# mmp/pbrt-v3

Hardware: NVIDIA H100
Metric: Msamples/sec (higher is better)
Workload: dtype f32

## Files before the change

### include/pb2.h

```cpp
#ifndef PB2_H
#define PB2_H

#include <stddef.h>
#include <stdint.h>

#ifdef __cplusplus
extern "C" {
#endif

#define PB2_ABI_VERSION 10

typedef enum pb2_status {
    PB2_OK = 0,
    PB2_ERR_NO_DEVICE = 1,
    PB2_ERR_CUDA = 2,
    PB2_ERR_INVALID = 3,
    PB2_ERR_UNSUPPORTED = 4,
    PB2_ERR_NCCL = 5
} pb2_status;


typedef struct pb2_bvh_node {
    float bmin[3];
    float bmax[3];
    int32_t offset;
    uint16_t n_prims;
    uint8_t axis;
    uint8_t pad;
} pb2_bvh_node;

enum { PB2_PRIM_TRIANGLE = 0, PB2_PRIM_SPHERE = 1, PB2_PRIM_INSTANCE = 2 };
enum { PB2_MAT_NONE = 0, PB2_MAT_MATTE = 1, PB2_MAT_PLASTIC = 2, PB2_MAT_MIRROR = 3, PB2_MAT_GLASS = 4, PB2_MAT_SUBSTRATE = 5, PB2_MAT_METAL = 6,
       PB2_MAT_UBER = 7 };
enum { PB2_LIGHTDIST_UNIFORM = 0, PB2_LIGHTDIST_POWER = 1, PB2_LIGHTDIST_SPATIAL = 2 };
enum { PB2_FILTER_BOX = 0, PB2_FILTER_GAUSSIAN = 1, PB2_FILTER_MITCHELL = 2, PB2_FILTER_SINC = 3, PB2_FILTER_TRIANGLE = 4 };

typedef struct pb2_mesh {
    int32_t first_tri, n_tris;
    int32_t first_vertex, n_vertices;
    int32_t has_n, has_uv, has_s;
    int32_t reverse_orientation;
    int32_t transform_swaps_handedness;
    int32_t alpha_tex, shadow_alpha_tex;
    int32_t pad;
} pb2_mesh;

enum { PB2_WRAP_REPEAT = 0, PB2_WRAP_BLACK = 1, PB2_WRAP_CLAMP = 2 };
typedef struct pb2_texture {
    int32_t channels;
    int32_t width, height;
    int32_t wrap;
    int32_t do_trilinear;
    float max_anisotropy;
    float su, sv, du, dv;
    int32_t kind;
    int32_t pad;
    const float *texels;
    int32_t child[3];
    float value[3];
} pb2_texture;
enum { PB2_TEXKIND_IMAGE = 0, PB2_TEXKIND_CONSTANT = 1, PB2_TEXKIND_SCALE = 2, PB2_TEXKIND_MIX = 3, PB2_TEXKIND_CHECKERBOARD = 4,
       PB2_TEXKIND_UV = 5 };

enum { PB2_TEX_KD = 0, PB2_TEX_KS = 1, PB2_TEX_KR = 2, PB2_TEX_KT = 3, PB2_TEX_OPACITY = 4, PB2_TEX_SIGMA = 5, PB2_TEX_ROUGHNESS = 6,
       PB2_TEX_UROUGHNESS = 7, PB2_TEX_VROUGHNESS = 8, PB2_TEX_ETA = 9, PB2_TEX_METAL_ETA = 10, PB2_TEX_METAL_K = 11,
       PB2_TEX_BUMP = 12, PB2_TEX_SLOTS = 13 };

typedef struct pb2_sphere {
    float object_to_world[16];
    float world_to_object[16];
    float radius, z_min, z_max, theta_min, theta_max, phi_max;
    int32_t reverse_orientation;
    int32_t transform_swaps_handedness;
} pb2_sphere;

typedef struct pb2_material {
    int32_t type;
    float kd[3];
    float sigma;
    float ks[3];
    float roughness;
    int32_t remap_roughness;
    int32_t pad[2];
    float kr[3];
    float kt[3];
    float eta;
    float uroughness, vroughness;
    float opacity[3];
    float metal_eta[3];
    float metal_k[3];
    int32_t pad3[2];
    int32_t tex[16];
} pb2_material;

enum { PB2_LIGHT_AREA = 0, PB2_LIGHT_POINT = 1, PB2_LIGHT_SPOT = 2, PB2_LIGHT_DISTANT = 3, PB2_LIGHT_INFINITE = 4 };
typedef struct pb2_light {
    int32_t prim;
    float L[3];
    int32_t two_sided;
    float area;
    int32_t type;
    int32_t pad;
} pb2_light;

typedef struct pb2_delta_light {
    float p[3];
    float total_width_deg;
    float falloff_start_deg;
    float world_radius;
    float world_to_light[9];
    float pad;
    float light_to_world[9];
    int32_t env_tex;
    float pad2[2];
} pb2_delta_light;

typedef struct pb2_bvh {
    int64_t node_offset, n_nodes;
    int64_t prim_offset, n_prims;
} pb2_bvh;

typedef struct pb2_instance {
    float instance_to_world[16];
    float world_to_instance[16];
    int32_t bvh;
    int32_t lone_prim;
    int32_t pad[2];
} pb2_instance;

typedef struct pb2_scene_desc {
    int64_t n_vertices;
    const float *P;
    const float *N;
    const float *UV;
    const float *S;
    int64_t n_tris;
    const int32_t *tri_index;
    const int32_t *tri_mesh;
    int32_t n_meshes;
    const pb2_mesh *meshes;
    int32_t n_spheres;
    const pb2_sphere *spheres;

    int64_t n_prims;
    const uint8_t *prim_type;
    const int32_t *prim_index;
    const int32_t *prim_material;
    const int32_t *prim_light;

    int64_t n_nodes;
    const pb2_bvh_node *nodes;
    const int32_t *bvh_prims;

    int32_t n_materials;
    const pb2_material *materials;
    int32_t n_lights;
    const pb2_light *lights;

    int32_t light_strategy;
    int32_t spatial_max_voxels;

    int32_t n_instances;
    int32_t n_bvhs;
    const pb2_instance *instances;
    const pb2_bvh *bvhs;
    int64_t n_bvh_prims;
    const pb2_delta_light *delta_lights;
    int32_t n_textures;
    int32_t pad_textures;
    const pb2_texture *textures;
} pb2_scene_desc;

typedef struct pb2_camera {
    float camera_to_world[16];
    float world_to_camera[16];
    float screen_window[4];
    float fov;
    float lens_radius, focal_distance;
    float shutter_open, shutter_close;
    float raster_to_camera[16];
    float dx_camera[3], dy_camera[3];
} pb2_camera;

typedef struct pb2_film_desc {
    int32_t full_resolution[2];
    int32_t cropped_pixel_bounds[4];
    float filter_radius[2];
    float max_sample_luminance;
    float scale;
    int32_t filter_type;
    float filter_param[2];
    int32_t pad;
} pb2_film_desc;

typedef struct pb2_path_params {
    int32_t samples_per_pixel;
    int32_t sample_at_pixel_center;
    int32_t max_depth;
    float rr_threshold;
    int32_t pixel_bounds[4];
    int32_t tile_rank, tile_count;
    int32_t flags;
    int32_t sampler;
} pb2_path_params;

enum { PB2_SAMPLER_HALTON = 0, PB2_SAMPLER_SOBOL = 1 };

#define PB2_FLAG_COUNT_TRAVERSAL 1
#define PB2_FLAG_LINEAR_NODES 2
#define PB2_FLAG_WIDE4 4
#define PB2_FLAG_PLAIN_TRACE 8
#define PB2_FLAG_SMALL_STACK 16
#define PB2_FLAG_LD128 32
#define PB2_FLAG_LEAF_TMA 64
#define PB2_FLAG_POOL 128
#define PB2_FLAG_CHAIN 256

typedef struct pb2_ray {
    float o[3];
    float d[3];
    float t_max;
} pb2_ray;

typedef struct pb2_hit {
    int32_t prim;
    float t;
    float b[3];
    float p[3];
    float p_error[3];
    float n[3];
    float ns[3];
    float dpdu[3];
    float uv[2];
} pb2_hit;

typedef struct pb2_stats {
    uint64_t camera_rays;
    uint64_t regular_rays;
    uint64_t shadow_rays;
    uint64_t node_visits;
    uint64_t prim_tests;
    uint64_t kernel_launches;
    double render_ms;
    double h2d_ms, d2h_ms;
    double trace_ms;
} pb2_stats;

typedef struct pb2_scene pb2_scene;


int pb2_abi_version(void);
const char *pb2_last_error(void);

int pb2_init(int device_id);
int pb2_init_devices(int n_devices, const int *device_ids);
int pb2_device_count(void);
int pb2_shutdown(void);

#define PB2_DIST_ID_BYTES 128
int pb2_dist_unique_id(void *id);
int pb2_dist_init(int rank, int world, const void *id);
int pb2_dist_info(int *rank, int *world);
int pb2_dist_shutdown(void);

int pb2_work_items(const pb2_film_desc *film, const pb2_path_params *params, int64_t first, int64_t n, int32_t *out,
                   int64_t *n_items);

int pb2_host_alloc(size_t bytes, void **out);
int pb2_host_free(void *p);

int pb2_scene_create(const pb2_scene_desc *desc, pb2_scene **out);
int pb2_scene_destroy(pb2_scene *scene);
int pb2_shade_class(const pb2_scene_desc *desc, int32_t *out);

int pb2_intersect(pb2_scene *scene, const pb2_ray *rays, int64_t n, pb2_hit *hits);
int pb2_intersect_p(pb2_scene *scene, const pb2_ray *rays, int64_t n, uint8_t *occluded);

int pb2_render_path(pb2_scene *scene, const pb2_camera *camera, const pb2_film_desc *film,
                    const pb2_path_params *params, float *film_rgbw, pb2_stats *stats);

int pb2_render_path_device(pb2_scene *scene, const pb2_camera *camera, const pb2_film_desc *film,
                           const pb2_path_params *params, float *film_rgbw_device, int clear,
                           void *stream, pb2_stats *stats);

typedef struct pb2_wf_hit {
    int32_t found;
    int32_t leaf;
    int32_t prim;
    float t;
    float b[3];
    int32_t listed;
} pb2_wf_hit;
int pb2_trace_wavefront(pb2_scene *scene, const pb2_ray *rays, const uint8_t *any_hit, int64_t n, int32_t flags,
                        pb2_wf_hit *out);

int pb2_li_samples(pb2_scene *scene, const pb2_camera *camera, const pb2_film_desc *film,
                   const pb2_path_params *params, const int32_t *pixel_xy, const int64_t *sample_num,
                   int64_t n, float *out_rgb, float *out_pfilm);

int pb2_halton_samples(const pb2_film_desc *film, const pb2_path_params *params,
                       const int32_t *pixel_xy, const int64_t *sample_num, const int32_t *dim,
                       int64_t n, float *out);

int pb2_sobol_samples_host(const pb2_film_desc *film, const pb2_path_params *params, const int32_t *pixel_xy,
                           const int64_t *sample_num, const int32_t *dim, int64_t n, float *out, uint64_t *tables);

int pb2_light_distribution(pb2_scene *scene, const float *points_xyz, int64_t n, float *out);

int pb2_texture_pyramid(const pb2_texture *texture, int32_t level, int32_t *n_levels, int32_t *w, int32_t *h, float *out);

int pb2_texture_eval_host(const pb2_texture *textures, int32_t n_textures, int32_t id, int64_t n, const float *uv, const float *duv,
                          float *out);

int pb2_bsdf_eval_host(const pb2_material *material, int64_t n, const float *in, float *out);

int pb2_camera_differentials_host(const pb2_camera *camera, const pb2_film_desc *film, const pb2_path_params *params, int64_t n,
                                  const float *in, float *out);
int pb2_uv_differentials_host(int64_t n, const float *in, float *out);

int pb2_env_distribution(const pb2_texture *texture, int32_t *nu, int32_t *nv, float *out);

int pb2_texture_lookup(const pb2_texture *texture, int64_t n, const float *st, const float *dst, float *out);

typedef struct pb2_build_node {
    float bmin[3], bmax[3];
    int32_t child[2];
    int32_t split_axis;
    int32_t first_prim_offset;
    int32_t n_primitives;
} pb2_build_node;
int pb2_hlbvh_treelets(const float *prim_bounds, int64_t n, int32_t max_prims_in_node, pb2_build_node *pool,
                       int32_t *ordered_prims, int32_t *treelet_roots, int32_t *n_treelets, double *device_ms);

int pb2_hlbvh_build(const float *prim_bounds, int64_t n, int32_t max_prims_in_node, pb2_bvh_node *nodes, int64_t *n_nodes,
                    int32_t *ordered_prims, double *device_ms);

#ifdef __cplusplus
}
#endif
#endif
```

### pbrt_v3_b200/__init__.py

```python
import ctypes as C
import os

import numpy as np

_HERE = os.path.dirname(os.path.abspath(__file__))
LIB_PATH = os.environ.get("PB2_LIB") or os.path.join(_HERE, "lib", "libpb2.so")

c_float_p = C.POINTER(C.c_float)
c_int32_p = C.POINTER(C.c_int32)
c_int64_p = C.POINTER(C.c_int64)
c_uint8_p = C.POINTER(C.c_uint8)

PB2_OK, PB2_ERR_NO_DEVICE, PB2_ERR_CUDA, PB2_ERR_INVALID, PB2_ERR_UNSUPPORTED, PB2_ERR_NCCL = range(6)
PB2_PRIM_TRIANGLE, PB2_PRIM_SPHERE, PB2_PRIM_INSTANCE = 0, 1, 2
PB2_FILTER_BOX, PB2_FILTER_GAUSSIAN, PB2_FILTER_MITCHELL, PB2_FILTER_SINC, PB2_FILTER_TRIANGLE = 0, 1, 2, 3, 4
PB2_MAT_NONE, PB2_MAT_MATTE, PB2_MAT_PLASTIC, PB2_MAT_MIRROR, PB2_MAT_GLASS, PB2_MAT_SUBSTRATE, PB2_MAT_METAL, PB2_MAT_UBER = range(8)
PB2_ABI_VERSION = 10
PB2_LIGHTDIST_UNIFORM, PB2_LIGHTDIST_POWER, PB2_LIGHTDIST_SPATIAL = 0, 1, 2
PB2_LIGHT_AREA, PB2_LIGHT_POINT, PB2_LIGHT_SPOT, PB2_LIGHT_DISTANT, PB2_LIGHT_INFINITE = 0, 1, 2, 3, 4


class BvhNode(C.Structure):
    _fields_ = [("bmin", C.c_float * 3), ("bmax", C.c_float * 3), ("offset", C.c_int32),
                ("n_prims", C.c_uint16), ("axis", C.c_uint8), ("pad", C.c_uint8)]


class Mesh(C.Structure):
    _fields_ = [("first_tri", C.c_int32), ("n_tris", C.c_int32), ("first_vertex", C.c_int32),
                ("n_vertices", C.c_int32), ("has_n", C.c_int32), ("has_uv", C.c_int32), ("has_s", C.c_int32),
                ("reverse_orientation", C.c_int32), ("transform_swaps_handedness", C.c_int32),
                ("alpha_tex", C.c_int32), ("shadow_alpha_tex", C.c_int32), ("pad", C.c_int32)]


class Sphere(C.Structure):
    _fields_ = [("object_to_world", C.c_float * 16), ("world_to_object", C.c_float * 16),
                ("radius", C.c_float), ("z_min", C.c_float), ("z_max", C.c_float), ("theta_min", C.c_float),
                ("theta_max", C.c_float), ("phi_max", C.c_float), ("reverse_orientation", C.c_int32),
                ("transform_swaps_handedness", C.c_int32)]


class Material(C.Structure):
    _fields_ = [("type", C.c_int32), ("kd", C.c_float * 3), ("sigma", C.c_float), ("ks", C.c_float * 3),
                ("roughness", C.c_float), ("remap_roughness", C.c_int32), ("pad", C.c_int32 * 2),
                ("kr", C.c_float * 3), ("kt", C.c_float * 3), ("eta", C.c_float), ("uroughness", C.c_float),
                ("vroughness", C.c_float), ("opacity", C.c_float * 3), ("metal_eta", C.c_float * 3),
                ("metal_k", C.c_float * 3), ("pad3", C.c_int32 * 2), ("tex", C.c_int32 * 16)]


PB2_WRAP_REPEAT, PB2_WRAP_BLACK, PB2_WRAP_CLAMP = 0, 1, 2
PB2_SAMPLER_HALTON, PB2_SAMPLER_SOBOL = 0, 1
(PB2_TEX_KD, PB2_TEX_KS, PB2_TEX_KR, PB2_TEX_KT, PB2_TEX_OPACITY, PB2_TEX_SIGMA, PB2_TEX_ROUGHNESS, PB2_TEX_UROUGHNESS,
 PB2_TEX_VROUGHNESS, PB2_TEX_ETA, PB2_TEX_METAL_ETA, PB2_TEX_METAL_K, PB2_TEX_BUMP) = range(13)


class Texture(C.Structure):
    _fields_ = [("channels", C.c_int32), ("width", C.c_int32), ("height", C.c_int32), ("wrap", C.c_int32),
                ("do_trilinear", C.c_int32), ("max_anisotropy", C.c_float), ("su", C.c_float), ("sv", C.c_float),
                ("du", C.c_float), ("dv", C.c_float), ("kind", C.c_int32), ("pad", C.c_int32), ("texels", c_float_p),
                ("child", C.c_int32 * 3), ("value", C.c_float * 3)]


PB2_TEXKIND_IMAGE, PB2_TEXKIND_CONSTANT, PB2_TEXKIND_SCALE, PB2_TEXKIND_MIX, PB2_TEXKIND_CHECKERBOARD, PB2_TEXKIND_UV = 0, 1, 2, 3, 4, 5


class Light(C.Structure):
    _fields_ = [("prim", C.c_int32), ("L", C.c_float * 3), ("two_sided", C.c_int32), ("area", C.c_float),
                ("type", C.c_int32), ("pad", C.c_int32)]


class DeltaLight(C.Structure):
    _fields_ = [("p", C.c_float * 3), ("total_width_deg", C.c_float), ("falloff_start_deg", C.c_float),
                ("world_radius", C.c_float), ("world_to_light", C.c_float * 9), ("pad", C.c_float),
                ("light_to_world", C.c_float * 9), ("env_tex", C.c_int32), ("pad2", C.c_float * 2)]


class Bvh(C.Structure):
    _fields_ = [("node_offset", C.c_int64), ("n_nodes", C.c_int64), ("prim_offset", C.c_int64), ("n_prims", C.c_int64)]


class Instance(C.Structure):
    _fields_ = [("instance_to_world", C.c_float * 16), ("world_to_instance", C.c_float * 16), ("bvh", C.c_int32),
                ("lone_prim", C.c_int32), ("pad", C.c_int32 * 2)]


class SceneDesc(C.Structure):
    _fields_ = [("n_vertices", C.c_int64), ("P", c_float_p), ("N", c_float_p), ("UV", c_float_p), ("S", c_float_p),
                ("n_tris", C.c_int64), ("tri_index", c_int32_p), ("tri_mesh", c_int32_p),
                ("n_meshes", C.c_int32), ("meshes", C.POINTER(Mesh)),
                ("n_spheres", C.c_int32), ("spheres", C.POINTER(Sphere)),
                ("n_prims", C.c_int64), ("prim_type", c_uint8_p), ("prim_index", c_int32_p),
                ("prim_material", c_int32_p), ("prim_light", c_int32_p),
                ("n_nodes", C.c_int64), ("nodes", C.POINTER(BvhNode)), ("bvh_prims", c_int32_p),
                ("n_materials", C.c_int32), ("materials", C.POINTER(Material)),
                ("n_lights", C.c_int32), ("lights", C.POINTER(Light)),
                ("light_strategy", C.c_int32), ("spatial_max_voxels", C.c_int32),
                ("n_instances", C.c_int32), ("n_bvhs", C.c_int32), ("instances", C.POINTER(Instance)),
                ("bvhs", C.POINTER(Bvh)), ("n_bvh_prims", C.c_int64), ("delta_lights", C.POINTER(DeltaLight)),
                ("n_textures", C.c_int32), ("pad_textures", C.c_int32), ("textures", C.POINTER(Texture))]


class Camera(C.Structure):
    _fields_ = [("camera_to_world", C.c_float * 16), ("world_to_camera", C.c_float * 16),
                ("screen_window", C.c_float * 4), ("fov", C.c_float), ("lens_radius", C.c_float),
                ("focal_distance", C.c_float), ("shutter_open", C.c_float), ("shutter_close", C.c_float),
                ("raster_to_camera", C.c_float * 16), ("dx_camera", C.c_float * 3), ("dy_camera", C.c_float * 3)]


class FilmDesc(C.Structure):
    _fields_ = [("full_resolution", C.c_int32 * 2), ("cropped_pixel_bounds", C.c_int32 * 4),
                ("filter_radius", C.c_float * 2), ("max_sample_luminance", C.c_float), ("scale", C.c_float),
                ("filter_type", C.c_int32), ("filter_param", C.c_float * 2), ("pad", C.c_int32)]


class PathParams(C.Structure):
    _fields_ = [("samples_per_pixel", C.c_int32), ("sample_at_pixel_center", C.c_int32), ("max_depth", C.c_int32),
                ("rr_threshold", C.c_float), ("pixel_bounds", C.c_int32 * 4), ("tile_rank", C.c_int32),
                ("tile_count", C.c_int32), ("flags", C.c_int32), ("sampler", C.c_int32)]


class Ray(C.Structure):
    _fields_ = [("o", C.c_float * 3), ("d", C.c_float * 3), ("t_max", C.c_float)]


class Hit(C.Structure):
    _fields_ = [("prim", C.c_int32), ("t", C.c_float), ("b", C.c_float * 3), ("p", C.c_float * 3),
                ("p_error", C.c_float * 3), ("n", C.c_float * 3), ("ns", C.c_float * 3), ("dpdu", C.c_float * 3),
                ("uv", C.c_float * 2)]


class WfHit(C.Structure):
    _fields_ = [("found", C.c_int32), ("leaf", C.c_int32), ("prim", C.c_int32), ("t", C.c_float), ("b", C.c_float * 3),
                ("listed", C.c_int32)]


class Stats(C.Structure):
    _fields_ = [("camera_rays", C.c_uint64), ("regular_rays", C.c_uint64), ("shadow_rays", C.c_uint64),
                ("node_visits", C.c_uint64), ("prim_tests", C.c_uint64), ("kernel_launches", C.c_uint64),
                ("render_ms", C.c_double), ("h2d_ms", C.c_double), ("d2h_ms", C.c_double), ("trace_ms", C.c_double)]


RAY_DTYPE = np.dtype([("o", np.float32, 3), ("d", np.float32, 3), ("t_max", np.float32)])
HIT_DTYPE = np.dtype([("prim", np.int32), ("t", np.float32), ("b", np.float32, 3), ("p", np.float32, 3),
                      ("p_error", np.float32, 3), ("n", np.float32, 3), ("ns", np.float32, 3),
                      ("dpdu", np.float32, 3), ("uv", np.float32, 2)])
WFHIT_DTYPE = np.dtype([("found", np.int32), ("leaf", np.int32), ("prim", np.int32), ("t", np.float32), ("b", np.float32, 3),
                        ("listed", np.int32)])
PB2_FLAG_COUNT_TRAVERSAL, PB2_FLAG_LINEAR_NODES, PB2_FLAG_WIDE4, PB2_FLAG_PLAIN_TRACE, PB2_FLAG_SMALL_STACK, PB2_FLAG_LD128, PB2_FLAG_LEAF_TMA, PB2_FLAG_POOL = 1, 2, 4, 8, 16, 32, 64, 128
PB2_FLAG_CHAIN = 256
NODE_DTYPE = np.dtype([("bmin", np.float32, 3), ("bmax", np.float32, 3), ("offset", np.int32),
                       ("n_prims", np.uint16), ("axis", np.uint8), ("pad", np.uint8)])
assert WFHIT_DTYPE.itemsize == C.sizeof(WfHit)
assert RAY_DTYPE.itemsize == C.sizeof(Ray) and HIT_DTYPE.itemsize == C.sizeof(Hit) and NODE_DTYPE.itemsize == 32


class Pb2Error(RuntimeError):
    def __init__(self, code, message):
        super().__init__("pb2 status %d: %s" % (code, message))
        self.code = code


_lib = None


def lib():
    global _lib
    if _lib is not None:
        return _lib
    if not os.path.exists(LIB_PATH):
        raise ImportError("%s is missing: run `python -c 'import __graft_entry__ as g; g.build()'` "
                          "(the CUDA extension is required; there is no fallback)" % LIB_PATH)
    L = C.CDLL(LIB_PATH)
    vp = C.c_void_p
    L.pb2_last_error.restype = C.c_char_p
    L.pb2_scene_create.argtypes = [C.POINTER(SceneDesc), C.POINTER(vp)]
    L.pb2_scene_destroy.argtypes = [vp]
    L.pb2_intersect.argtypes = [vp, vp, C.c_int64, vp]
    L.pb2_intersect_p.argtypes = [vp, vp, C.c_int64, vp]
    L.pb2_trace_wavefront.argtypes = [vp, vp, vp, C.c_int64, C.c_int32, vp]
    L.pb2_work_items.argtypes = [C.POINTER(FilmDesc), C.POINTER(PathParams), C.c_int64, C.c_int64, vp, C.POINTER(C.c_int64)]
    L.pb2_init_devices.argtypes = [C.c_int, C.POINTER(C.c_int)]
    L.pb2_dist_unique_id.argtypes = [vp]
    L.pb2_dist_init.argtypes = [C.c_int, C.c_int, vp]
    L.pb2_dist_info.argtypes = [C.POINTER(C.c_int), C.POINTER(C.c_int)]
    L.pb2_host_alloc.argtypes = [C.c_size_t, C.POINTER(vp)]
    L.pb2_host_free.argtypes = [vp]
    L.pb2_render_path.argtypes = [vp, C.POINTER(Camera), C.POINTER(FilmDesc), C.POINTER(PathParams), vp, C.POINTER(Stats)]
    L.pb2_render_path_device.argtypes = [vp, C.POINTER(Camera), C.POINTER(FilmDesc), C.POINTER(PathParams), vp,
                                         C.c_int, vp, C.POINTER(Stats)]
    L.pb2_li_samples.argtypes = [vp, C.POINTER(Camera), C.POINTER(FilmDesc), C.POINTER(PathParams), vp, vp, C.c_int64, vp, vp]
    L.pb2_halton_samples.argtypes = [C.POINTER(FilmDesc), C.POINTER(PathParams), vp, vp, vp, C.c_int64, vp]
    L.pb2_light_distribution.argtypes = [vp, vp, C.c_int64, vp]
    L.pb2_sobol_samples_host.argtypes = [C.POINTER(FilmDesc), C.POINTER(PathParams), vp, vp, vp, C.c_int64, vp, vp]
    L.pb2_texture_pyramid.argtypes = [C.POINTER(Texture), C.c_int32, C.POINTER(C.c_int32), C.POINTER(C.c_int32), C.POINTER(C.c_int32), vp]
    L.pb2_texture_lookup.argtypes = [C.POINTER(Texture), C.c_int64, vp, vp, vp]
    L.pb2_env_distribution.argtypes = [C.POINTER(Texture), C.POINTER(C.c_int32), C.POINTER(C.c_int32), vp]
    L.pb2_texture_eval_host.argtypes = [C.POINTER(Texture), C.c_int32, C.c_int32, C.c_int64, vp, vp, vp]
    L.pb2_bsdf_eval_host.argtypes = [C.POINTER(Material), C.c_int64, vp, vp]
    L.pb2_camera_differentials_host.argtypes = [C.POINTER(Camera), C.POINTER(FilmDesc), C.POINTER(PathParams), C.c_int64, vp, vp]
    L.pb2_uv_differentials_host.argtypes = [C.c_int64, vp, vp]
    L.pb2h_parse_file.argtypes = [C.c_char_p, C.c_char_p]
    L.pb2h_parse_string.argtypes = [C.c_char_p]
    L.pb2h_synth_soup.argtypes = [C.c_int64, C.c_uint64, C.c_float, C.c_int, C.c_int, C.c_int, C.c_int, C.c_char_p]
    L.pb2h_synth_instanced.argtypes = [C.c_int64, C.c_int, C.c_uint64, C.c_uint64, C.c_float, C.c_int, C.c_int, C.c_int, C.c_int]
    L.pb2h_scene_desc.restype = C.POINTER(SceneDesc)
    L.pb2h_camera.restype = C.POINTER(Camera)
    L.pb2h_film.restype = C.POINTER(FilmDesc)
    L.pb2h_path_params.restype = C.POINTER(PathParams)
    L.pb2h_render.argtypes = [C.c_int, C.POINTER(Stats)]
    L.pb2h_image.restype = c_float_p
    L.pb2h_image.argtypes = [C.POINTER(C.c_int), C.POINTER(C.c_int)]
    L.pb2h_resolve_film.argtypes = [vp, vp]
    L.pb2h_device_scene.restype = vp
    L.pb2h_write_pfm.argtypes = [C.c_char_p, vp, C.c_int, C.c_int]
    L.pb2h_write_image.argtypes = [C.c_char_p, vp] + [C.c_int] * 6
    L.pb2h_read_image.argtypes = [C.c_char_p, vp, C.POINTER(C.c_int), C.POINTER(C.c_int)]
    L.pb2h_loop_subdivide.argtypes = [C.c_int, C.c_int, vp, C.c_int, vp, C.POINTER(C.c_int), C.POINTER(C.c_int), vp, vp, vp]
    L.pb2h_set_light_strategy.argtypes = [C.c_int]
    L.pb2h_scene_intersect.argtypes = [vp, vp, vp]
    _lib = L
    return L


def check(code):
    if code != PB2_OK:
        raise Pb2Error(code, lib().pb2_last_error().decode("utf-8", "replace"))


def ptr(a):
    return a.ctypes.data_as(C.c_void_p) if a is not None else None


_initialised_device = None


def init(device=None):
    global _initialised_device
    if device is None:
        device = int(os.environ.get("LOCAL_RANK", os.environ.get("PB2_DEVICE", "0")))
    if _initialised_device == device:
        return
    check(lib().pb2_init(device))
    _initialised_device = device


def sobol_samples_host(film, params, pixel_xy, sample_num, dim, tables=False):
    pixel_xy = np.ascontiguousarray(pixel_xy, np.int32)
    sample_num = np.ascontiguousarray(sample_num, np.int64)
    dim = np.ascontiguousarray(dim, np.int32)
    out = np.zeros(len(dim), np.float32)
    tab = np.zeros(104, np.uint64)
    check(lib().pb2_sobol_samples_host(film, params, ptr(pixel_xy), ptr(sample_num), ptr(dim), len(dim), ptr(out), ptr(tab)))
    return (out, tab) if tables else out


def texture_pyramid(texture, fn=None):
    fn = fn or lib().pb2_texture_pyramid
    nl, w, h = C.c_int32(), C.c_int32(), C.c_int32()
    check(fn(C.byref(texture), 0, C.byref(nl), C.byref(w), C.byref(h), None))
    levels = []
    for lv in range(nl.value):
        check(fn(C.byref(texture), lv, C.byref(nl), C.byref(w), C.byref(h), None))
        a = np.zeros((h.value, w.value, texture.channels), np.float32)
        check(fn(C.byref(texture), lv, C.byref(nl), C.byref(w), C.byref(h), ptr(a)))
        levels.append(a)
    return levels


def bsdf_eval_host(material, frames, fn=None):
    fn = fn or lib().pb2_bsdf_eval_host
    frames = np.ascontiguousarray(frames, np.float32)
    out = np.zeros((len(frames), 19), np.float32)
    check(fn(C.byref(material), len(frames), ptr(frames), ptr(out)))
    return out


def texture_eval_host(textures, n_textures, tex_id, uv, duv, fn=None):
    fn = fn or lib().pb2_texture_eval_host
    uv = np.ascontiguousarray(uv, np.float32)
    duv = np.ascontiguousarray(duv, np.float32)
    out = np.zeros((len(uv), 3), np.float32)
    check(fn(textures, n_textures, tex_id, len(uv), ptr(uv), ptr(duv), ptr(out)))
    return out


def env_distribution(texture, fn=None):
    fn = fn or lib().pb2_env_distribution
    nu, nv = C.c_int32(), C.c_int32()
    check(fn(C.byref(texture), C.byref(nu), C.byref(nv), None))
    table = np.zeros(nv.value * (2 * nu.value + 2) + 2 * nv.value + 2, np.float32)
    check(fn(C.byref(texture), C.byref(nu), C.byref(nv), ptr(table)))
    return nu.value, nv.value, table


def read_image(path):
    w, h = C.c_int(), C.c_int()
    if lib().pb2h_read_image(path.encode(), None, C.byref(w), C.byref(h)) != 0:
        raise RuntimeError("cannot read %s" % path)
    out = np.zeros((h.value, w.value, 3), np.float32)
    lib().pb2h_read_image(path.encode(), ptr(out), C.byref(w), C.byref(h))
    return out


def texture_lookup(texture, st, dst):
    init()
    st = np.ascontiguousarray(st, np.float32)
    dst = np.ascontiguousarray(dst, np.float32)
    out = np.zeros((len(st), 3), np.float32)
    check(lib().pb2_texture_lookup(C.byref(texture), len(st), ptr(st), ptr(dst), ptr(out)))
    return out


class HostScene:

    _generation = 0

    def __init__(self):
        self.L = lib()
        HostScene._generation += 1
        self._gen = HostScene._generation

    def _current(self):
        if self._gen != HostScene._generation:
            raise RuntimeError("this HostScene was replaced by a later HostScene (the host front end holds one scene at a time)")

    @classmethod
    def from_file(cls, path, outfile=None):
        s = cls()
        if s.L.pb2h_parse_file(path.encode(), outfile.encode() if outfile else None) != 0:
            raise RuntimeError("could not parse %s" % path)
        return s

# ... 176 lines not shown
```

### pbrt_v3_b200/csrc/pb2_cuda.cu

```cuda
#include <cuda_runtime.h>
#include <cub/device/device_radix_sort.cuh>
#include <dlfcn.h>
#include <nccl.h>

#include <algorithm>
#include <mutex>
#include <chrono>
#include <cstddef>
#include <cstdio>
#include <cstdlib>
#include <cstring>
#include <string>
#include <thread>
#include <vector>

#include "device/pb2_path.cuh"
#include "device/pb2_wide4.cuh"
#include "host/core.h"
#include "pb2.h"

using namespace pb2;

static thread_local std::string g_lastError;
static int setError(int code, const std::string &msg) {
// ... 425 lines not shown
        out.prim = it.prim;
        out.b[0] = h.b0; out.b[1] = h.b1; out.b[2] = h.b2;
        out.p[0] = it.p.x; out.p[1] = it.p.y; out.p[2] = it.p.z;
        out.p_error[0] = it.pError.x; out.p_error[1] = it.pError.y; out.p_error[2] = it.pError.z;
        out.n[0] = it.n.x; out.n[1] = it.n.y; out.n[2] = it.n.z;
        out.ns[0] = it.ns.x; out.ns[1] = it.ns.y; out.ns[2] = it.ns.z;
        out.dpdu[0] = it.dpdus.x; out.dpdu[1] = it.dpdus.y; out.dpdu[2] = it.dpdus.z;
        out.uv[0] = it.uv.x; out.uv[1] = it.uv.y;
    }
    hits[i] = out;
}

__global__ void k_intersect_p(DScene sc, const pb2_ray *rays, int64_t n, uint8_t *occluded) {
    int64_t i = blockIdx.x * (int64_t)blockDim.x + threadIdx.x;
    if (i >= n) return;
    DRay r;
    r.o = mk3(rays[i].o[0], rays[i].o[1], rays[i].o[2]);
    r.d = mk3(rays[i].d[0], rays[i].d[1], rays[i].d[2]);
    r.tMax = rays[i].t_max;
    DHit h;
    h.leaf = -1;
    h.inst = -1;
    float tMax = r.tMax;
    occluded[i] = traverse<true>(sc, r, &tMax, &h, nullptr) ? 1 : 0;
}

struct DRenderParams {
    DCamera cam;
    DHalton halton;
    DPathParams path;
    int sbx0, sby0, sbx1, sby1;
    int pbx0, pby0, pbx1, pby1;
    int cx0, cy0, cx1, cy1;
    float filterRadiusX, filterRadiusY;
    float invFilterRadiusX, invFilterRadiusY;
    const float *filterTable;
    float maxSampleLuminance;
    int nTilesX, nTilesY;
    int tileRank, tileCount;
    long long nOwnedTiles;
    long long nWorkItems;
    int spp;
    float diffScale;
};

enum { CTR_WORK = 0, CTR_CAMERA = 1, CTR_REGULAR = 2, CTR_SHADOW = 3, CTR_NODES = 4, CTR_PRIMS = 5, CTR_COUNT = 8 };

PB2_HD int compact1by1(unsigned x) {
    x &= 0x55555555u;
    x = (x ^ (x >> 1)) & 0x33333333u;
    x = (x ^ (x >> 2)) & 0x0f0f0f0fu;
    x = (x ^ (x >> 4)) & 0x00ff00ffu;
    return (int)x;
}

PB2_HD bool decodeWork(const DRenderParams &rp, long long item, int *px, int *py, int *sample) {
    long long perTile = 256LL * rp.spp;
    long long owned = item / perTile;
    int r = (int)(item - owned * perTile);
    long long tile = (long long)rp.tileRank + owned * rp.tileCount;
    int ty = (int)(tile / rp.nTilesX), tx = (int)(tile - (long long)ty * rp.nTilesX);
    int s = r >> 8, m = r & 255;
    int x = rp.sbx0 + tx * 16 + compact1by1((unsigned)m);
    int y = rp.sby0 + ty * 16 + compact1by1((unsigned)m >> 1);
    *px = x;
    *py = y;
    *sample = s;
    if (x >= rp.sbx1 || y >= rp.sby1) return false;
    return x >= rp.pbx0 && x < rp.pbx1 && y >= rp.pby0 && y < rp.pby1;
}

__device__ __noinline__ void addSampleFiltered(const DRenderParams &rp, float4 *film, V2 pFilm, V3 L) {
    float dx = pFilm.x - 0.5f, dy = pFilm.y - 0.5f;
    int p0x = (int)ceilf(dx - rp.filterRadiusX), p0y = (int)ceilf(dy - rp.filterRadiusY);
    int p1x = (int)floorf(dx + rp.filterRadiusX) + 1, p1y = (int)floorf(dy + rp.filterRadiusY) + 1;
    p0x = max(p0x, rp.cx0);
    p0y = max(p0y, rp.cy0);
    p1x = min(p1x, rp.cx1);
    p1y = min(p1y, rp.cy1);
    int width = rp.cx1 - rp.cx0;
    for (int yy = p0y; yy < p1y; ++yy) {
        float fy = fabsf(((float)yy - dy) * rp.invFilterRadiusY * 16.f);
        int ify = min((int)floorf(fy), 15);
        for (int xx = p0x; xx < p1x; ++xx) {
            float fx = fabsf(((float)xx - dx) * rp.invFilterRadiusX * 16.f);
            int ifx = min((int)floorf(fx), 15);
            float w = rp.filterTable[ify * 16 + ifx];
            float4 *px = film + ((size_t)(yy - rp.cy0) * width + (xx - rp.cx0));
            atomicAdd(px, make_float4(L.x * w, L.y * w, L.z * w, w));
        }
    }
}

__device__ __forceinline__ void addSample(const DRenderParams &rp, float4 *film, V2 pFilm, V3 L) {
    float y = luminance(L);
    if (y > rp.maxSampleLuminance) L = L * (rp.maxSampleLuminance / y);
    if (rp.filterTable) {
        addSampleFiltered(rp, film, pFilm, L);
        return;
    }
    float dx = pFilm.x - 0.5f, dy = pFilm.y - 0.5f;
    int p0x = (int)ceilf(dx - rp.filterRadiusX), p0y = (int)ceilf(dy - rp.filterRadiusY);
    int p1x = (int)floorf(dx + rp.filterRadiusX) + 1, p1y = (int)floorf(dy + rp.filterRadiusY) + 1;
    p0x = max(p0x, rp.cx0);
    p0y = max(p0y, rp.cy0);
    p1x = min(p1x, rp.cx1);
    p1y = min(p1y, rp.cy1);
    int width = rp.cx1 - rp.cx0;
    for (int yy = p0y; yy < p1y; ++yy)
        for (int xx = p0x; xx < p1x; ++xx) {
            float4 *px = film + ((size_t)(yy - rp.cy0) * width + (xx - rp.cx0));
            atomicAdd(px, make_float4(L.x, L.y, L.z, 1.f));
        }
}

#include "pb2_wavefront.cuh"

__global__ void k_li_samples(DScene sc, DRenderParams rp, const int32_t *pixelXY, const int64_t *sampleNum, int64_t n,
                             float *outRGB, float *outPFilm, int *deferred) {
    int64_t i = blockIdx.x * (int64_t)blockDim.x + threadIdx.x;
    if (i >= n) return;
    int px = pixelXY[2 * i], py = pixelXY[2 * i + 1];
    DSampler smp;
    smp.index = sampleIndex<true>(rp.halton, px, py, sampleNum[i]);
    smp.dim = 0;
    V2 pFilm;
    DRay ray = generateCameraRay<true>(rp.cam, rp.halton, smp, px, py, &pFilm);
    DLane ln;
    laneStartPath(ln, ray, smp);
    while (ln.state != LS_IDLE) {
        DHit hit;
        float tMax;
        bool found = traceLane(sc, ln, &tMax, &hit, nullptr);
        DTexCtx tc;
        tc.cam = &rp.cam;
        tc.pFilm = pFilm;
        tc.diffScale = rp.diffScale;
        laneAdvance<SHADE_FULL>(sc, rp.halton, rp.path, ln, found, hit, tMax, &tc);
        if (ln.state == LS_DEFER) {
            atomicAdd(deferred, 1);
            return;
        }
    }
    V3 L = guardRadiance(ln.L);
    outRGB[3 * i] = L.x;
    outRGB[3 * i + 1] = L.y;
    outRGB[3 * i + 2] = L.z;
    if (outPFilm) {
        outPFilm[2 * i] = pFilm.x;
        outPFilm[2 * i + 1] = pFilm.y;
    }
}

__global__ void k_wf_debug_fill(WfPool pool, const pb2_ray *rays, const uint8_t *anyHit, int n) {
    int i = blockIdx.x * blockDim.x + threadIdx.x;
    if (i == 0) {
        for (int q = 0; q < WQ_COUNT; ++q) pool.counts[q] = 0;
        pool.counts[WQ_TRACE0] = (unsigned)n;
    }
    if (i >= n) return;
    WfCtx &cx = pool.ctx[i];
    cx.ln.state = (anyHit && anyHit[i]) ? LS_SHADOW : LS_PATH;
    cx.ln.ray.o = mk3(rays[i].o[0], rays[i].o[1], rays[i].o[2]);
    cx.ln.ray.d = mk3(rays[i].d[0], rays[i].d[1], rays[i].d[2]);
    cx.ln.ray.tMax = rays[i].t_max;
    cx.hit = make_float4(__int_as_float(-1), 0.f, 0.f, 0.f);
    cx.tHit = 0.f;
    cx.found = -1;
    pool.queue[WQ_TRACE0][i] = i;
}
__global__ void k_wf_debug_read(DScene sc, WfPool pool, int n, pb2_wf_hit *out) {
    int i = blockIdx.x * blockDim.x + threadIdx.x;
    if (i >= n) return;
    const WfCtx &cx = pool.ctx[i];
    pb2_wf_hit h;
    h.found = cx.found;
    h.t = cx.tHit;
    h.leaf = __float_as_int(cx.hit.x);
    h.b[0] = cx.hit.y; h.b[1] = cx.hit.z; h.b[2] = cx.hit.w;
    h.prim = (cx.found > 0 && h.leaf >= 0) ? asInt(ldg4(&sc.leafPrims[3 * (size_t)h.leaf]).w) : -1;
    h.listed = 0;
    out[i] = h;
}
__global__ void k_wf_debug_lists(WfPool pool, pb2_wf_hit *out) {
    unsigned ns = pool.counts[WQ_SHADE], nl = pool.counts[WQ_LIGHT];
    for (unsigned i = blockIdx.x * blockDim.x + threadIdx.x; i < ns + nl; i += gridDim.x * blockDim.x) {
        int c = i < ns ? pool.queue[WQ_SHADE][i] : pool.queue[WQ_LIGHT][i - ns];
        atomicAdd(&out[c].listed, i < ns ? 1 : 2);
    }
}

__global__ void k_halton_samples(DHalton h, const int32_t *pixelXY, const int64_t *sampleNum, const int32_t *dim, int64_t n,
                                 float *out) {
    int64_t i = blockIdx.x * (int64_t)blockDim.x + threadIdx.x;
    if (i >= n) return;
    const int px = pixelXY[2 * i], py = pixelXY[2 * i + 1];
    int64_t index = sampleIndex<true>(h, px, py, sampleNum[i]);
    if (h.sobol && dim[i] < 2) out[i] = sobolPixelSample(h, index, dim[i], dim[i] == 0 ? px : py);
    else out[i] = sampleDimension<true>(h, index, dim[i]);
}

__global__ void k_halton_batch(DHalton h, const int32_t *pixelXY, const int64_t *sampleNum, const int32_t *dim0, int64_t n, float *out) {
    int64_t i = blockIdx.x * (int64_t)blockDim.x + threadIdx.x;
    if (i >= n) return;
    const int64_t index = sampleIndex<true>(h, pixelXY[2 * i], pixelXY[2 * i + 1], sampleNum[i]);
    float u[kSampleBatch];
    haltonSampleBatch<true>(h, index, dim0[i], kSampleBatch, u);
#pragma unroll
    for (int k = 0; k < kSampleBatch; ++k) out[kSampleBatch * i + k] = u[k];
}

__global__ void k_light_distribution(DScene sc, const float *points, int64_t n, float *out) {
    int64_t i = blockIdx.x * (int64_t)blockDim.x + threadIdx.x;
    if (i >= n) return;
    const float *rec = lightDistLookup(sc.lightDist, mk3(points[3 * i], points[3 * i + 1], points[3 * i + 2]));
    if (!rec) return;
    int stride = 2 * sc.nLights + 1;
    for (int k = 0; k < stride; ++k) out[i * stride + k] = rec[k];
}

static DHalton haltonTablesOnly() {
    DHalton h;
    memset(&h, 0, sizeof(h));
    h.primes = cur().primes;
    h.primeSums = cur().primeSums;
    h.perms = cur().perms;
    h.dimRecs = cur().dimRecs;
    h.dimTabs = cur().dimTabs;
    h.digitTab = cur().digitTab;
    return h;
}

static void launchLightDistBuild(const pb2_scene *scene, cudaStream_t stream) {
    k_lightdist_build<<<g_numSMs * 4, 128, 0, stream>>>(scene->d, haltonTablesOnly());
    k_lightdist_done<<<1, 32, 0, stream>>>(scene->d);
}
static int lightDistOverflowed(pb2_scene *scene, cudaStream_t stream, bool *overflowed) {
    *overflowed = false;
    if (!scene->lazyLightDist) return PB2_OK;
    CUDA_TRY(cudaMemcpyAsync(scene->ldHostCounters, scene->d.lightDist.counters, 4 * sizeof(int), cudaMemcpyDeviceToHost, stream));
    CUDA_TRY(cudaStreamSynchronize(stream));
    *overflowed = scene->ldHostCounters[2] != 0;
    return PB2_OK;
}
static int lightDistOverflowError() {
    return setError(PB2_ERR_UNSUPPORTED, "the on-demand pool of spatial light distributions is exhausted (very many lights x very many voxels touched): "
                                         "raise PB2_LIGHTDIST_POOL_MB or use lightsamplestrategy \"power\" / \"uniform\"");
}

static int requireDevice() {
    if (!g_initialised) return setError(PB2_ERR_NO_DEVICE, "pb2_init() has not succeeded: no CUDA device is bound (there is no CPU fallback)");
    return PB2_OK;
}

static bool computeFilterTable(const pb2_film_desc *f, float table[256]) {
    const float rx = f->filter_radius[0], ry = f->filter_radius[1];
    const float p0 = f->filter_param[0], p1 = f->filter_param[1];
    auto eval = [&](float x, float y) -> float {
        switch (f->filter_type) {
        case PB2_FILTER_GAUSSIAN: {
            const float alpha = p0, expX = std::exp(-alpha * rx * rx), expY = std::exp(-alpha * ry * ry);
            auto g = [&](float d, float expv) { return std::max((float)0, float(std::exp(-alpha * d * d) - expv)); };
            return g(x, expX) * g(y, expY);
        }
        case PB2_FILTER_MITCHELL: {
            const float B = p0, C = p1;
            auto m1 = [&](float v) {
                v = std::abs(2 * v);
                if (v > 1)
                    return ((-B - 6 * C) * v * v * v + (6 * B + 30 * C) * v * v + (-12 * B - 48 * C) * v + (8 * B + 24 * C)) * (1.f / 6.f);
                return ((12 - 9 * B - 6 * C) * v * v * v + (-18 + 12 * B + 6 * C) * v * v + (6 - 2 * B)) * (1.f / 6.f);
            };
            const float invRx = 1 / rx, invRy = 1 / ry;
            return m1(x * invRx) * m1(y * invRy);
        }
        case PB2_FILTER_SINC: {
            const float tau = p0, Pi = 3.14159265358979323846f;
            auto sinc = [&](float v) -> float {
                v = std::abs(v);
                if (v < 1e-5) return 1;
                return std::sin(Pi * v) / (Pi * v);
            };
            auto ws = [&](float v, float radius) -> float {
                v = std::abs(v);
                if (v > radius) return 0;
                float lanczos = sinc(v / tau);
                return sinc(v) * lanczos;
            };
            return ws(x, rx) * ws(y, ry);
        }
        case PB2_FILTER_TRIANGLE:
            return std::max((float)0, rx - std::abs(x)) * std::max((float)0, ry - std::abs(y));
        default:
            return 1.f;
        }
    };
    int offset = 0;
    for (int y = 0; y < 16; ++y)
        for (int x = 0; x < 16; ++x, ++offset) table[offset] = eval((x + 0.5f) * rx / 16, (y + 0.5f) * ry / 16);
    return f->filter_type != PB2_FILTER_BOX;
}

static DRenderParams makeRenderParams(const pb2_camera *cam, const pb2_film_desc *film, const pb2_path_params *pp) {
    DRenderParams rp;
    memset(&rp, 0, sizeof(rp));
    memcpy(rp.cam.rasterToCamera.m, cam->raster_to_camera, sizeof(float) * 16);
    memcpy(rp.cam.cameraToWorld.m, cam->camera_to_world, sizeof(float) * 16);
    rp.cam.lensRadius = cam->lens_radius;
    rp.cam.focalDistance = cam->focal_distance;
    rp.cam.dxCamera = mk3(cam->dx_camera[0], cam->dx_camera[1], cam->dx_camera[2]);
    rp.cam.dyCamera = mk3(cam->dy_camera[0], cam->dy_camera[1], cam->dy_camera[2]);
    rp.diffScale = 1 / std::sqrt((float)pp->samples_per_pixel);
    rp.halton = makeHalton(film, pp);
    rp.path.maxDepth = pp->max_depth;
    rp.path.rrThreshold = pp->rr_threshold;
    SampleBounds sb = filmSampleBounds(film);
    rp.sbx0 = sb.x0; rp.sby0 = sb.y0; rp.sbx1 = sb.x1; rp.sby1 = sb.y1;
    rp.pbx0 = pp->pixel_bounds[0]; rp.pby0 = pp->pixel_bounds[1]; rp.pbx1 = pp->pixel_bounds[2]; rp.pby1 = pp->pixel_bounds[3];
    rp.cx0 = film->cropped_pixel_bounds[0]; rp.cy0 = film->cropped_pixel_bounds[1];
    rp.cx1 = film->cropped_pixel_bounds[2]; rp.cy1 = film->cropped_pixel_bounds[3];
    rp.filterRadiusX = film->filter_radius[0];
    rp.filterRadiusY = film->filter_radius[1];
    rp.invFilterRadiusX = 1.f / film->filter_radius[0];
    rp.invFilterRadiusY = 1.f / film->filter_radius[1];
    rp.filterTable = nullptr;
    rp.maxSampleLuminance = film->max_sample_luminance;
    rp.nTilesX = (sb.x1 - sb.x0 + 15) / 16;
    rp.nTilesY = (sb.y1 - sb.y0 + 15) / 16;
    rp.tileCount = std::max(1, pp->tile_count);
    rp.tileRank = pp->tile_rank;
    long long nTiles = (long long)std::max(0, rp.nTilesX) * std::max(0, rp.nTilesY);
    rp.nOwnedTiles = nTiles > rp.tileRank ? (nTiles - rp.tileRank + rp.tileCount - 1) / rp.tileCount : 0;
    rp.spp = pp->samples_per_pixel;
    rp.nWorkItems = rp.nOwnedTiles * 256LL * rp.spp;
    return rp;
}

static int validateRenderArgs(const pb2_scene *scene, const pb2_camera *cam, const pb2_film_desc *film, const pb2_path_params *pp) {
    if (!scene || !cam || !film || !pp) return setError(PB2_ERR_INVALID, "null argument");
    if (pp->samples_per_pixel <= 0 || pp->max_depth < 0) return setError(PB2_ERR_INVALID, "bad samples_per_pixel / max_depth");
    if (5 + 8 * ((long long)pp->max_depth + 1) > kMaxHaltonDims)
        return setError(PB2_ERR_UNSUPPORTED, "maxdepth above 123: HaltonSampler can only sample 1000 dimensions");
    if (pp->tile_count < 0 || pp->tile_rank < 0 || (pp->tile_count > 0 && pp->tile_rank >= pp->tile_count))
        return setError(PB2_ERR_INVALID, "bad tile_rank / tile_count");
    if (pp->sampler != PB2_SAMPLER_HALTON && pp->sampler != PB2_SAMPLER_SOBOL) return setError(PB2_ERR_INVALID, "unknown sampler");
    if (pp->sampler == PB2_SAMPLER_SOBOL && (pp->samples_per_pixel & (pp->samples_per_pixel - 1)))
        return setError(PB2_ERR_INVALID, "SobolSampler: samples_per_pixel must be the power of two its constructor rounds up to (sobol.h:52)");
    if (film->cropped_pixel_bounds[2] < film->cropped_pixel_bounds[0] || film->cropped_pixel_bounds[3] < film->cropped_pixel_bounds[1])
        return setError(PB2_ERR_INVALID, "bad cropped pixel bounds");
    if (!(film->filter_radius[0] > 0) || !(film->filter_radius[1] > 0)) return setError(PB2_ERR_INVALID, "bad filter radius");
    if (film->filter_type < PB2_FILTER_BOX || film->filter_type > PB2_FILTER_TRIANGLE) return setError(PB2_ERR_INVALID, "unknown filter type");
    return PB2_OK;
}

enum { kMaxPipes = 4 };
typedef void (*TraceKernel)(DScene, WfPool, int, WfChain);
typedef void (*AdvanceKernel)(const DScene *, const DRenderParams *, WfPool, int, int, int, float4 *, unsigned long long *);

struct TraceLaunch {
    TraceKernel fn = nullptr;
    int block = 128;
    size_t smem = 0;
    int grid = 0;
    bool chain = false;
    const char *name = "";
};

enum TraceKernelForm { TK_COUNT, TK_PLAIN, TK_POOL, TK_WIDE2, TK_WIDE4, TK_LINEAR };
struct TraceKernelEntry {
    TraceKernelForm form;
    int features;
    TraceKernel fn;
    const char *name;
    size_t smem;
};
template <int WIDTH, int T>
static TraceKernelEntry wideTrace() {
    const char *name = WIDTH == 4              ? "k_wf_trace_w<4>"
                       : (T & TRACE_ALPHA) ? "k_wf_trace_w<2,alpha>"
                       : (T & TRACE_CHAIN) ? "k_wf_trace_w<2,chain>"
                                           : "k_wf_trace_w<2>";
    return {WIDTH == 4 ? TK_WIDE4 : TK_WIDE2, T, k_wf_trace_w<WIDTH, T>, name, 0};
}
template <int T>
static TraceKernelEntry linearTrace() { return {TK_LINEAR, T, k_wf_trace<T>, "k_wf_trace", 0}; }

struct TraceKey {
    TraceKernelForm form;
    int features;
};
static TraceKey chooseTraceKernel(const pb2_scene *scene, int flags, bool render) {
    const bool instanced = scene->d.instances != nullptr;
    const bool records = scene->d.wide4 != nullptr && !(flags & PB2_FLAG_LINEAR_NODES);
    const bool linearFits = !instanced || scene->bvhDepth + 3 + scene->instDepth <= 64;
    int sceneBits = scene->d.spheres ? TRACE_SPHERES : 0;
    if (instanced) sceneBits |= TRACE_SPHERES | TRACE_INST;
    if (flags & PB2_FLAG_COUNT_TRAVERSAL) return {TK_COUNT, 0};
    if ((flags & PB2_FLAG_PLAIN_TRACE) || (!records && !linearFits)) return {TK_PLAIN, 0};
    if (scene->d.hasAlpha) return records ? TraceKey{TK_WIDE2, sceneBits | TRACE_ALPHA} : TraceKey{TK_PLAIN, 0};
    if (!records) return {TK_LINEAR, sceneBits | (sceneBits || scene->bvhDepth > 32 ? TRACE_DEEP : 0)};
    if ((flags & PB2_FLAG_POOL) && !sceneBits) return {TK_POOL, 0};
    const bool ld128 = (flags & PB2_FLAG_LD128) != 0;
    int features = sceneBits | (ld128 ? TRACE_LD128 : 0) | ((flags & PB2_FLAG_SMALL_STACK) ? TRACE_SMALL_STACK : 0);
    if (flags & PB2_FLAG_WIDE4) return {TK_WIDE4, features};
    if (!ld128 && (flags & PB2_FLAG_LEAF_TMA) && !sceneBits) features = TRACE_LEAF_TMA;
    if (!ld128 && render && (flags & PB2_FLAG_CHAIN) && !(flags & (PB2_FLAG_SMALL_STACK | PB2_FLAG_LEAF_TMA))) features |= TRACE_CHAIN;
    return {TK_WIDE2, features};
}

static int selectTraceKernel(pb2_scene *scene, int flags, TraceLaunch *out, bool render = false, const char *steps = "") {
    static const TraceKernelEntry kernels[] = {
        {TK_COUNT, 0, k_wf_trace_plain<true>, "k_wf_trace_plain<count>", 0},
        {TK_PLAIN, 0, k_wf_trace_plain<false>, "k_wf_trace_plain", 0},
        {TK_POOL, 0, k_wf_trace_pool, "k_wf_trace_pool", 4 * sizeof(PoolWarp)},
        wideTrace<2, 0>(), wideTrace<2, TRACE_SMALL_STACK>(),
        wideTrace<2, TRACE_LD128>(), wideTrace<2, TRACE_LD128 | TRACE_SMALL_STACK>(),
        wideTrace<2, TRACE_SPHERES>(), wideTrace<2, TRACE_SPHERES | TRACE_SMALL_STACK>(),
        wideTrace<2, TRACE_SPHERES | TRACE_LD128>(), wideTrace<2, TRACE_SPHERES | TRACE_LD128 | TRACE_SMALL_STACK>(),
        wideTrace<2, TRACE_SPHERES | TRACE_INST>(), wideTrace<2, TRACE_SPHERES | TRACE_INST | TRACE_SMALL_STACK>(),
        wideTrace<2, TRACE_SPHERES | TRACE_INST | TRACE_LD128>(), wideTrace<2, TRACE_SPHERES | TRACE_INST | TRACE_LD128 | TRACE_SMALL_STACK>(),
        wideTrace<2, TRACE_LEAF_TMA>(),
        wideTrace<2, TRACE_CHAIN>(), wideTrace<2, TRACE_SPHERES | TRACE_CHAIN>(), wideTrace<2, TRACE_SPHERES | TRACE_INST | TRACE_CHAIN>(),
        wideTrace<2, TRACE_ALPHA>(), wideTrace<2, TRACE_SPHERES | TRACE_ALPHA>(), wideTrace<2, TRACE_SPHERES | TRACE_INST | TRACE_ALPHA>(),
        wideTrace<4, 0>(), wideTrace<4, TRACE_SMALL_STACK>(),
        wideTrace<4, TRACE_LD128>(), wideTrace<4, TRACE_LD128 | TRACE_SMALL_STACK>(),
        wideTrace<4, TRACE_SPHERES>(), wideTrace<4, TRACE_SPHERES | TRACE_SMALL_STACK>(),
        wideTrace<4, TRACE_SPHERES | TRACE_LD128>(), wideTrace<4, TRACE_SPHERES | TRACE_LD128 | TRACE_SMALL_STACK>(),
        wideTrace<4, TRACE_SPHERES | TRACE_INST>(), wideTrace<4, TRACE_SPHERES | TRACE_INST | TRACE_SMALL_STACK>(),
        wideTrace<4, TRACE_SPHERES | TRACE_INST | TRACE_LD128>(), wideTrace<4, TRACE_SPHERES | TRACE_INST | TRACE_LD128 | TRACE_SMALL_STACK>(),
        linearTrace<0>(), linearTrace<TRACE_DEEP>(),
        linearTrace<TRACE_SPHERES | TRACE_DEEP>(), linearTrace<TRACE_SPHERES | TRACE_INST | TRACE_DEEP>(),
    };
    const TraceKey want = chooseTraceKernel(scene, flags, render);
    const TraceKernelEntry *k = nullptr;
    for (const TraceKernelEntry &e : kernels)
        if (e.form == want.form && e.features == want.features) k = &e;
    if (!k)
        return setError(PB2_ERR_CUDA, "no trace kernel of form " + std::to_string(want.form) + " is compiled for the trace features " +
                                          std::to_string(want.features));
    TraceLaunch t;
    t.fn = k->fn;
    t.smem = k->smem;
    t.chain = (k->features & TRACE_CHAIN) != 0;
    t.name = k->name;
    if (k->form == TK_POOL && !scene->wfSpill)
        CUDA_TRY(cudaMalloc((void **)&scene->wfSpill, (size_t)kMaxPipes * g_numSMs * 8 * 4 * PL_R * PL_SPILL * sizeof(int2)));
    if (t.smem) CUDA_TRY(cudaFuncSetAttribute(t.fn, cudaFuncAttributeMaxDynamicSharedMemorySize, (int)t.smem));
    int blocksPerSM = 1;
    CUDA_TRY(cudaOccupancyMaxActiveBlocksPerMultiprocessor(&blocksPerSM, t.fn, t.block, t.smem));
    blocksPerSM = std::max(1, std::min(blocksPerSM, 8));
    cudaFuncAttributes fa;
    CUDA_TRY(cudaFuncGetAttributes(&fa, t.fn));
    size_t need = (size_t)blocksPerSM * (fa.sharedSizeBytes + t.smem + 1024);
    int pct = (int)std::min<size_t>(100, (need * 100 + 233471) / 233472);
    CUDA_TRY(cudaFuncSetAttribute(t.fn, cudaFuncAttributePreferredSharedMemoryCarveout, pct));
    static const int verbose = envInt("PB2_VERBOSE", 0);
    if (verbose)
        fprintf(stderr, "pb2: trace kernel %s: %d regs, %zu B smem, %d blocks/SM, carve-out %d %%, BVH depth %d%s\n", t.name, fa.numRegs,
                fa.sharedSizeBytes + t.smem, blocksPerSM, pct, scene->bvhDepth, steps);
    t.grid = g_numSMs * blocksPerSM;
    *out = t;
    return PB2_OK;
}

static int ensurePool(pb2_scene *scene, int capacity) {
    if (scene->wfCapacity < capacity) {
        if (scene->wfCtx) cudaFree(scene->wfCtx);
        if (scene->wfQueues) cudaFree(scene->wfQueues);
        scene->wfCtx = nullptr;
        scene->wfQueues = nullptr;
        scene->wfCapacity = 0;
        CUDA_TRY(cudaMalloc(&scene->wfCtx, (size_t)capacity * sizeof(WfCtx)));
        CUDA_TRY(cudaMalloc((void **)&scene->wfQueues, (size_t)capacity * WQ_COUNT * sizeof(int)));
        scene->wfCapacity = capacity;
    }
    if (!scene->wfCounts) CUDA_TRY(cudaMalloc((void **)&scene->wfCounts, kMaxPipes * WQ_COUNT * sizeof(unsigned)));
    if (!scene->wfHostCounts) CUDA_TRY(cudaMallocHost((void **)&scene->wfHostCounts, (kMaxPipes * WQ_COUNT + 2) * sizeof(unsigned long long)));
    return PB2_OK;
}

static WfPool poolOf(const pb2_scene *scene, int capacity, int pipe = 0, int nPipes = 1) {
    WfPool pool;
    const int cap = capacity / nPipes;
    pool.capacity = cap;
    pool.ctx = (WfCtx *)scene->wfCtx + (size_t)pipe * cap;
    for (int q = 0; q < WQ_COUNT; ++q) pool.queue[q] = scene->wfQueues + ((size_t)pipe * WQ_COUNT + q) * cap;
    pool.counts = scene->wfCounts + (size_t)pipe * WQ_COUNT;
    pool.ctr = scene->counters;
    pool.spill = scene->wfSpill ? scene->wfSpill + (size_t)pipe * g_numSMs * 8 * 4 * PL_R * PL_SPILL : nullptr;
    return pool;
}

constexpr int kShadeLambertAreaMinBlocks = 4;

typedef void (*GenKernel)(const DRenderParams *, WfPool, int, int);
typedef void (*FinishKernel)(const DScene *, const DRenderParams *, WfPool, int, unsigned, float4 *);

template <typename K>
struct StepKernel {
    int features;
    K fn;
};
template <bool SHADE, int MINB, int F>
static StepKernel<AdvanceKernel> advanceStep() { return {F, k_wf_advance<SHADE, MINB, F>}; }

template <typename K, size_t N>
static const StepKernel<K> &stepKernel(const StepKernel<K> (&table)[N], int frame) {
    int reads = 0;
    for (const StepKernel<K> &k : table) reads |= k.features;
    const StepKernel<K> *best = nullptr;
    for (const StepKernel<K> &k : table)
        if (!(frame & reads & ~k.features) && (!best || __builtin_popcount(k.features) < __builtin_popcount(best->features))) best = &k;
    return *best;
}

static int frameShadeFeatures(const pb2_scene *scene, const DRenderParams &rp) {
    int f = scene->shadeFeatures;
    if (scene->d.spheres) f |= SHADE_SPHERES;
    if (scene->lazyLightDist) f |= SHADE_LAZY;
    if (scene->d.nTextures > 0) f |= SHADE_TEXTURES;
    if (rp.halton.sobol) f |= SHADE_SOBOL;
    return f;
}

static int renderWavefront(pb2_scene *scene, const DRenderParams &rp, float4 *film, cudaStream_t stream, int flags,
                           bool timeTrace, unsigned long long *launches, double *traceMs) {
    const bool lazyLights = scene->lazyLightDist;
    static const int maxCapacity = envInt("PB2_POOL", 1 << 22);
    long long want = std::min<long long>(maxCapacity, std::max<long long>(rp.nWorkItems, 1024));
    int capacity = (int)((want + 255) / 256 * 256);
    int rc = ensurePool(scene, capacity);
    if (rc) return rc;
    static const StepKernel<GenKernel> genSteps[] = {{0, k_wf_gen<0>}, {SHADE_SOBOL, k_wf_gen<SHADE_SOBOL>}};
    static const StepKernel<AdvanceKernel> lightSteps[] = {
        advanceStep<false, 7, SHADE_LAMBERT_AREA>(),
        advanceStep<false, 7, SHADE_GENERAL>(),
        advanceStep<false, 7, SHADE_GENERAL | SHADE_SPHERES>(),
    };
    static const StepKernel<AdvanceKernel> shadeSteps[] = {
        advanceStep<true, kShadeLambertAreaMinBlocks, SHADE_LAMBERT_AREA>(),
        advanceStep<true, 4, SHADE_GENERAL>(),
        advanceStep<true, 4, SHADE_GENERAL | SHADE_SPHERES>(),
        advanceStep<true, 4, SHADE_GENERAL | SHADE_SPECULAR>(),
        advanceStep<true, 4, SHADE_GENERAL | SHADE_SPHERES | SHADE_SPECULAR>(),
        advanceStep<true, 4, SHADE_GENERAL | SHADE_LAZY>(),
        advanceStep<true, 4, SHADE_GENERAL | SHADE_SPHERES | SHADE_LAZY>(),
        advanceStep<true, 4, SHADE_GENERAL | SHADE_SPECULAR | SHADE_LAZY>(),
        advanceStep<true, 4, SHADE_GENERAL | SHADE_SPHERES | SHADE_SPECULAR | SHADE_LAZY>(),
        advanceStep<true, 3, SHADE_FULL>(),
    };
    static const StepKernel<FinishKernel> finishSteps[] = {
        {SHADE_LAMBERT_AREA, k_wf_finish<SHADE_LAMBERT_AREA>},
        {SHADE_GENERAL, k_wf_finish<SHADE_GENERAL>},
        {SHADE_GENERAL | SHADE_SPHERES, k_wf_finish<SHADE_GENERAL | SHADE_SPHERES>},
        {SHADE_GENERAL | SHADE_SPECULAR, k_wf_finish<SHADE_GENERAL | SHADE_SPECULAR>},
        {SHADE_GENERAL | SHADE_SPHERES | SHADE_SPECULAR, k_wf_finish<SHADE_GENERAL | SHADE_SPHERES | SHADE_SPECULAR>},
    };
    const int features = frameShadeFeatures(scene, rp);
    const StepKernel<GenKernel> &gen = stepKernel(genSteps, features);
    const StepKernel<AdvanceKernel> &advLight = stepKernel(lightSteps, features), &advShade = stepKernel(shadeSteps, features);
    const StepKernel<FinishKernel> &finish = stepKernel(finishSteps, features);
    char steps[96];
    snprintf(steps, sizeof(steps), "; shade features %d: gen %d, light %d, shade %d, tail %d", features, gen.features,
             advLight.features, advShade.features, finish.features);
    TraceLaunch trace;
    if ((rc = selectTraceKernel(scene, flags, &trace, true, steps))) return rc;
    if (!scene->paramBuf) CUDA_TRY(cudaMalloc(&scene->paramBuf, sizeof(DScene) + sizeof(DRenderParams)));
    const DScene *dSc = reinterpret_cast<const DScene *>(scene->paramBuf);
    const DRenderParams *dRp = reinterpret_cast<const DRenderParams *>((char *)scene->paramBuf + sizeof(DScene));
    CUDA_TRY(cudaMemcpyAsync((void *)dSc, &scene->d, sizeof(DScene), cudaMemcpyHostToDevice, stream));
    CUDA_TRY(cudaMemcpyAsync((void *)dRp, &rp, sizeof(DRenderParams), cudaMemcpyHostToDevice, stream));
    WfChain chain;
    memset(&chain, 0, sizeof(chain));
    if (trace.chain) {
        chain.sc = dSc;
        chain.rp = dRp;
        chain.film = film;
    }
    static const int finishPerSM = envInt("PB2_FINISH", 256);
    const bool textured = (features & (SHADE_TEXTURES | SHADE_SOBOL)) != 0;
    const unsigned finishThreshold = ((flags & PB2_FLAG_COUNT_TRAVERSAL) || lazyLights || textured) ? 0u : (unsigned)(g_numSMs * std::max(0, finishPerSM));
    const int finishBlocks = std::max(1, (int)((finishThreshold + 127) / 128));
    static const int syncEvery = std::max(1, envInt("PB2_SYNC_EVERY", 8));
    static const int pipesEnv = envInt("PB2_PIPES", 0);
    const int pipesWanted = std::min((int)kMaxPipes, pipesEnv > 0 ? pipesEnv : 2);
    const int nPipes = (lazyLights || capacity < 65536) ? 1 : pipesWanted;
    cudaStream_t streams[kMaxPipes] = {stream, stream, stream, stream};
    if (nPipes > 1) {
        if (!scene->forkEvent) CUDA_TRY(cudaEventCreateWithFlags(&scene->forkEvent, cudaEventDisableTiming));
        CUDA_TRY(cudaEventRecord(scene->forkEvent, stream));
        for (int p = 1; p < nPipes; ++p) {
            if (!scene->pipeStreams[p]) CUDA_TRY(cudaStreamCreateWithFlags(&scene->pipeStreams[p], cudaStreamNonBlocking));
            if (!scene->joinEvents[p]) CUDA_TRY(cudaEventCreateWithFlags(&scene->joinEvents[p], cudaEventDisableTiming));
            streams[p] = scene->pipeStreams[p];
            CUDA_TRY(cudaStreamWaitEvent(streams[p], scene->forkEvent, 0));
        }
    }
    WfPool pools[kMaxPipes];
    for (int p = 0; p < nPipes; ++p) pools[p] = poolOf(scene, capacity / nPipes * nPipes, p, nPipes);
    const int capP = pools[0].capacity;
    const int blocks128 = std::min((capP + 127) / 128, g_numSMs * 32);
    for (int p = 0; p < nPipes; ++p) k_wf_init<<<(capP + 255) / 256, 256, 0, streams[p]>>>(pools[p]);
    unsigned long long nLaunch = nPipes;
    size_t nEvents = 0;
    int cur = 0;
    volatile unsigned *hc = scene->wfHostCounts;
    unsigned long long *hWork = reinterpret_cast<unsigned long long *>(scene->wfHostCounts + kMaxPipes * WQ_COUNT);
    for (long long round = 0;; ++round) {
        int next = 1 - cur;
        for (int p = 0; p < nPipes; ++p) {
            const WfPool &pool = pools[p];
            cudaStream_t st = streams[p];
            gen.fn<<<blocks128, 128, 0, st>>>(dRp, pool, WQ_FREE0 + cur, WQ_TRACE0 + cur);
            if (timeTrace) {
                if (scene->traceEvents.size() < nEvents + 2) {
                    cudaEvent_t e0, e1;
                    CUDA_TRY(cudaEventCreate(&e0));
                    CUDA_TRY(cudaEventCreate(&e1));
                    scene->traceEvents.push_back(e0);
                    scene->traceEvents.push_back(e1);
                }
                CUDA_TRY(cudaEventRecord(scene->traceEvents[nEvents], st));
            }
            chain.freeQ = WQ_FREE0 + next;
            trace.fn<<<trace.grid, trace.block, trace.smem, st>>>(scene->d, pool, WQ_TRACE0 + cur, chain);
            if (timeTrace) {
                CUDA_TRY(cudaEventRecord(scene->traceEvents[nEvents + 1], st));
                nEvents += 2;
            }
            if (!trace.chain) advLight.fn<<<blocks128, 128, 0, st>>>(dSc, dRp, pool, WQ_LIGHT, WQ_TRACE0 + next, WQ_FREE0 + next, film, scene->counters);
            else --nLaunch;
            advShade.fn<<<blocks128, 128, 0, st>>>(dSc, dRp, pool, WQ_SHADE, WQ_TRACE0 + next, WQ_FREE0 + next, film, scene->counters);
            if (lazyLights) {
                launchLightDistBuild(scene, st);
                advShade.fn<<<blocks128, 128, 0, st>>>(dSc, dRp, pool, WQ_RETRY, WQ_TRACE0 + next, WQ_FREE0 + next, film, scene->counters);
                nLaunch += 3;
            }
            if (finishThreshold) finish.fn<<<finishBlocks, 128, 0, st>>>(dSc, dRp, pool, WQ_TRACE0 + next, finishThreshold, film);
            k_wf_reset<<<1, 32, 0, st>>>(pool, WQ_FREE0 + cur, WQ_TRACE0 + cur, WQ_TRACE0 + next, finishThreshold);
            nLaunch += finishThreshold ? 6 : 5;
        }
        cur = next;
        if ((round + 1) % syncEvery != 0) continue;
        for (int p = 0; p < nPipes; ++p)
            CUDA_TRY(cudaMemcpyAsync((void *)(scene->wfHostCounts + p * WQ_COUNT), pools[p].counts, WQ_COUNT * sizeof(unsigned), cudaMemcpyDeviceToHost, streams[p]));
        for (int p = 1; p < nPipes; ++p) CUDA_TRY(cudaStreamSynchronize(streams[p]));
        CUDA_TRY(cudaMemcpyAsync(hWork, &scene->counters[CTR_WORK], sizeof(unsigned long long), cudaMemcpyDeviceToHost, stream));
        CUDA_TRY(cudaStreamSynchronize(stream));
        bool overflowed = false;
        if ((rc = lightDistOverflowed(scene, stream, &overflowed))) return rc;
        if (overflowed) return lightDistOverflowError();
        const bool workLeft = (long long)*hWork < rp.nWorkItems;
        bool done = true;
        for (int p = 0; p < nPipes; ++p) {
            const unsigned traceNext = hc[p * WQ_COUNT + WQ_TRACE0 + cur], freeNext = hc[p * WQ_COUNT + WQ_FREE0 + cur];
            if (!(traceNext == 0 && !(workLeft && freeNext > 0))) done = false;
        }
        if (done) break;
        if (round > 100000000LL) return setError(PB2_ERR_CUDA, "wavefront did not terminate");
    }
    if (nPipes > 1) {
        for (int p = 1; p < nPipes; ++p) {
            CUDA_TRY(cudaEventRecord(scene->joinEvents[p], streams[p]));
            CUDA_TRY(cudaStreamWaitEvent(stream, scene->joinEvents[p], 0));
        }
    }
    CUDA_TRY(cudaGetLastError());
    *launches = nLaunch;
    *traceMs = 0;
    for (size_t e = 0; e + 1 < nEvents; e += 2) {
        float ms = 0;
        CUDA_TRY(cudaEventElapsedTime(&ms, scene->traceEvents[e], scene->traceEvents[e + 1]));
        *traceMs += ms;
    }
    return PB2_OK;
}

extern "C" {

int pb2_abi_version(void) { return PB2_ABI_VERSION; }
const char *pb2_last_error(void) { return g_lastError.c_str(); }

static void freeDeviceTables() {
    for (DeviceState &d : g_devs) {
        cudaSetDevice(d.id);
        cudaFree(d.primes);
        cudaFree(d.primeSums);
        cudaFree(d.perms);
        cudaFree(d.dimRecs);
        cudaFree(d.dimTabs);
        cudaFree(d.digitTab);
        cudaFree(d.sobol);
        cudaFree(d.sobolVdc);
    }
    g_devs.clear();
    g_initialised = false;
}

int pb2_init_devices(int n, const int *device_ids) {
    int count = 0;
    cudaError_t e = cudaGetDeviceCount(&count);
    if (e != cudaSuccess || count == 0) {
        cudaGetLastError();
        return setError(PB2_ERR_NO_DEVICE, std::string("no CUDA device available (") +
                                               (e != cudaSuccess ? cudaGetErrorString(e) : "device count is 0") +
                                               "); the path-tracing hot path has no CPU fallback");
    }
    std::vector<int> ids;
    if (n <= 0) for (int i = 0; i < count; ++i) ids.push_back(i);
    else {
        if (!device_ids) return setError(PB2_ERR_INVALID, "null device list");
        ids.assign(device_ids, device_ids + n);
    }
    for (size_t i = 0; i < ids.size(); ++i) {
        if (ids[i] < 0 || ids[i] >= count) return setError(PB2_ERR_INVALID, "device id out of range");
        for (size_t j = 0; j < i; ++j)
            if (ids[j] == ids[i]) return setError(PB2_ERR_INVALID, "device listed twice");
    }
    if (g_initialised && g_devs.size() == ids.size()) {
        bool same = true;
        for (size_t i = 0; i < ids.size(); ++i) same &= g_devs[i].id == ids[i];
        if (same) return PB2_OK;
    }
    if (g_dist.comm) return setError(PB2_ERR_INVALID, "pb2_init: shut the communicator down (pb2_dist_shutdown) before rebinding devices");
    freeDeviceTables();
    buildHaltonHostTables();
    t_dev = 0;
    for (int id : ids) {
        CUDA_TRY(cudaSetDevice(id));
        cudaDeviceProp prop;
        CUDA_TRY(cudaGetDeviceProperties(&prop, id));
        if (prop.major != 9 || prop.minor != 0) {
            freeDeviceTables();
            return setError(PB2_ERR_NO_DEVICE, std::string("device \"") + prop.name + "\" is not sm_90 (Hopper); this library is built for sm_90a only");
        }
        g_devs.emplace_back();
        DeviceState &d = g_devs.back();
        d.id = id;
        d.numSMs = prop.multiProcessorCount;
        CUDA_TRY(cudaMalloc((void **)&d.primes, g_halton.hPrimes.size() * sizeof(int32_t)));
        CUDA_TRY(cudaMalloc((void **)&d.primeSums, g_halton.hPrimeSums.size() * sizeof(int32_t)));
        CUDA_TRY(cudaMalloc((void **)&d.perms, g_halton.hPerms.size() * sizeof(uint16_t)));
        CUDA_TRY(cudaMalloc((void **)&d.dimRecs, g_halton.hDimRecs.size() * sizeof(ulonglong2)));
        CUDA_TRY(cudaMemcpy(d.dimRecs, g_halton.hDimRecs.data(), g_halton.hDimRecs.size() * sizeof(ulonglong2), cudaMemcpyHostToDevice));
        CUDA_TRY(cudaMemcpy(d.primes, g_halton.hPrimes.data(), g_halton.hPrimes.size() * sizeof(int32_t), cudaMemcpyHostToDevice));
        CUDA_TRY(cudaMemcpy(d.primeSums, g_halton.hPrimeSums.data(), g_halton.hPrimeSums.size() * sizeof(int32_t), cudaMemcpyHostToDevice));
        CUDA_TRY(cudaMemcpy(d.perms, g_halton.hPerms.data(), g_halton.hPerms.size() * sizeof(uint16_t), cudaMemcpyHostToDevice));
        CUDA_TRY(cudaMalloc((void **)&d.dimTabs, g_halton.hDimTabs.size() * sizeof(HaltonDimTab)));
        CUDA_TRY(cudaMalloc((void **)&d.digitTab, g_halton.hDigitTab.size() * sizeof(uint16_t)));
        CUDA_TRY(cudaMemcpy(d.dimTabs, g_halton.hDimTabs.data(), g_halton.hDimTabs.size() * sizeof(HaltonDimTab), cudaMemcpyHostToDevice));
        CUDA_TRY(cudaMemcpy(d.digitTab, g_halton.hDigitTab.data(), g_halton.hDigitTab.size() * sizeof(uint16_t), cudaMemcpyHostToDevice));
    }
    CUDA_TRY(cudaSetDevice(g_devs[0].id));
    for (size_t i = 1; i < g_devs.size(); ++i) {
        int can = 0;
        if (cudaDeviceCanAccessPeer(&can, g_devs[0].id, g_devs[i].id) == cudaSuccess && can) {
            cudaError_t pe = cudaDeviceEnablePeerAccess(g_devs[i].id, 0);
            g_devs[i].peerOfPrimary = pe == cudaSuccess || pe == cudaErrorPeerAccessAlreadyEnabled;
        }
        cudaGetLastError();
    }
    g_initialised = true;
    return PB2_OK;
}

int pb2_init(int device_id) { return pb2_init_devices(1, &device_id); }

int pb2_device_count(void) { return g_initialised ? (int)g_devs.size() : 0; }

int pb2_shutdown(void) {
    if (!g_initialised) return PB2_OK;
    pb2_dist_shutdown();
    freeDeviceTables();
    return PB2_OK;
}

int pb2_debug_radical_inverse_tables(const uint32_t *index, const int32_t *dim, int64_t n, float *out_loop, float *out_tab) {
    if (!index || !dim || !out_loop || !out_tab) return setError(PB2_ERR_INVALID, "null argument");
    buildHaltonHostTables();
    for (int64_t i = 0; i < n; ++i) {
        if (dim[i] < 2 || dim[i] >= kMaxHaltonDims) return setError(PB2_ERR_INVALID, "dimension out of range");
        const uint32_t base = (uint32_t)g_halton.hPrimes[dim[i]];
        const uint16_t *perm = g_halton.hPerms.data() + g_halton.hPrimeSums[dim[i]];
        const uint64_t magic = g_halton.hDimRecs[dim[i]].x;
        out_loop[i] = scrambledRadicalInverse32(base, magic, index[i], perm);
        out_tab[i] = scrambledRadicalInverseTab(g_halton.hDimTabs[dim[i]], g_halton.hDigitTab.data(), base, magic, index[i], perm);
    }
    return PB2_OK;
}

int pb2_debug_halton_batch(const pb2_film_desc *film, const pb2_path_params *pp, const uint32_t *index, const int32_t *dim0, int64_t n,
                           float *out_batch, float *out_tab) {
    if (!film || !pp || !index || !dim0 || !out_batch || !out_tab) return setError(PB2_ERR_INVALID, "null argument");
    buildHaltonHostTables();
    DHalton h = makeHalton(film, pp);
    h.perms = g_halton.hPerms.data();
    h.primes = g_halton.hPrimes.data();
    h.primeSums = g_halton.hPrimeSums.data();
    h.dimRecs = g_halton.hDimRecs.data();
    h.dimTabs = g_halton.hDimTabs.data();
    h.digitTab = g_halton.hDigitTab.data();
    for (int64_t i = 0; i < n; ++i) {
        if (dim0[i] < 2 || dim0[i] + kSampleBatch > kMaxHaltonDims) return setError(PB2_ERR_INVALID, "dimension out of range");
        haltonSampleBatch(h, (int64_t)index[i], dim0[i], kSampleBatch, out_batch + kSampleBatch * i);
        for (int k = 0; k < kSampleBatch; ++k) {
            const int d = dim0[i] + k;
            const uint32_t base = (uint32_t)g_halton.hPrimes[d];
            const uint16_t *perm = g_halton.hPerms.data() + g_halton.hPrimeSums[d];
// ... 796 lines not shown
        std::vector<int32_t> lightPrims(d->n_lights);
        for (int i = 0; i < d->n_lights; ++i) {
            if (d->lights[i].type != PB2_LIGHT_AREA) {
                lightPrims[i] = 0;
                continue;
            }
            if (d->lights[i].prim < 0 || d->lights[i].prim >= d->n_prims) return setError(PB2_ERR_INVALID, "light primitive out of range");
            lightPrims[i] = d->lights[i].prim;
        }
        const int32_t *dLightPrims;
        if ((rc = upload(s, lightPrims.data(), lightPrims.size(), &dLightPrims))) return rc;
        float4 *lrec;
        if ((rc = allocate(s, 3 * (size_t)d->n_lights, &lrec))) return rc;
        k_build_leaf_records<<<(unsigned)((d->n_lights + 255) / 256), 256>>>(sc, dLightPrims, d->n_lights, lrec);
        CUDA_TRY(cudaGetLastError());
        sc.lightRecs = lrec;
    }

    DLightDist &ld = sc.lightDist;
    memset(&ld, 0, sizeof(ld));
    int nl = d->n_lights;
    ld.stride = 2 * nl + 2;
    ld.strategy = (nl <= 1) ? PB2_LIGHTDIST_UNIFORM : d->light_strategy;
    ld.boundsMin = mk3(d->nodes[0].bmin[0], d->nodes[0].bmin[1], d->nodes[0].bmin[2]);
    ld.boundsMax = mk3(d->nodes[0].bmax[0], d->nodes[0].bmax[1], d->nodes[0].bmax[2]);
    if (nl > 0 && ld.strategy != PB2_LIGHTDIST_SPATIAL) {
        std::vector<float> rec(ld.stride);
        for (int i = 0; i < nl; ++i) {
            if (ld.strategy == PB2_LIGHTDIST_UNIFORM)
                rec[i] = 1.f;
            else {
                const pb2_light &l = d->lights[i];
                const float Pi = 3.14159265358979323846f;
                float s2 = l.two_sided ? 2.f : 1.f;
                float p[3];
                for (int c = 0; c < 3; ++c) {
                    if (l.type == PB2_LIGHT_POINT)
                        p[c] = l.L[c] * (4 * Pi);
                    else if (l.type == PB2_LIGHT_SPOT)
                        p[c] = ((l.L[c] * 2) * Pi) * (1 - .5f * (deltaLights[i].cosFalloffStart + deltaLights[i].cosTotalWidth));
                    else if (l.type == PB2_LIGHT_DISTANT)
                        p[c] = ((l.L[c] * Pi) * deltaLights[i].worldRadius) * deltaLights[i].worldRadius;
                    else if (l.type == PB2_LIGHT_INFINITE)
                        p[c] = ((Pi * deltaLights[i].worldRadius) * deltaLights[i].worldRadius) * (deltaLights[i].envTex ? deltaLights[i].dist[c] : l.L[c]);
                    else
                        p[c] = ((s2 * l.L[c]) * l.area) * Pi;
                }
                rec[i] = 0.212671f * p[0] + 0.715160f * p[1] + 0.072169f * p[2];
            }
        }
        float *cdf = rec.data() + nl;
        cdf[0] = 0;
        for (int i = 1; i < nl + 1; ++i) cdf[i] = cdf[i - 1] + rec[i - 1] / nl;
        float funcInt = cdf[nl];
        if (funcInt == 0) {
            for (int i = 1; i < nl + 1; ++i) cdf[i] = float(i) / float(nl);
        } else {
            for (int i = 1; i < nl + 1; ++i) cdf[i] /= funcInt;
        }
        rec[2 * nl + 1] = funcInt;
        if ((rc = upload(s, rec.data(), rec.size(), &ld.table))) return rc;
    } else if (nl > 0) {
        float diag[3] = {ld.boundsMax.x - ld.boundsMin.x, ld.boundsMax.y - ld.boundsMin.y, ld.boundsMax.z - ld.boundsMin.z};
        int maxExtent = (diag[0] > diag[1] && diag[0] > diag[2]) ? 0 : (diag[1] > diag[2] ? 1 : 2);
        float bmax = diag[maxExtent];
        int maxVoxels = d->spatial_max_voxels > 0 ? d->spatial_max_voxels : 64;
        for (int i = 0; i < 3; ++i) ld.nVoxels[i] = std::max(1, int(std::round(diag[i] / bmax * maxVoxels)));
        size_t nVox = (size_t)ld.nVoxels[0] * ld.nVoxels[1] * ld.nVoxels[2];
        const size_t recordBytes = (size_t)ld.stride * sizeof(float);
        const size_t eagerLimit = (size_t)std::max(1, envInt("PB2_LIGHTDIST_EAGER_MB", 256)) << 20;
        const bool lazy = envInt("PB2_LIGHTDIST_LAZY", 0) != 0 || nVox * recordBytes > eagerLimit;
        if (!lazy) {
            float *table;
            if ((rc = allocate(s, nVox * ld.stride, &table))) return rc;
            ld.table = table;
            int threads = 128;
            k_spatial_light_dist<<<(unsigned)((nVox + threads - 1) / threads), threads>>>(sc, haltonTablesOnly(), table);
            CUDA_TRY(cudaGetLastError());
        } else {
            const size_t poolLimit = (size_t)std::max(1, envInt("PB2_LIGHTDIST_POOL_MB", 2048)) << 20;
            const size_t records = std::max<size_t>(1, std::min(nVox, poolLimit / recordBytes));
            float *table;
            if ((rc = allocate(s, records * ld.stride, &table))) return rc;
            ld.table = table;
            ld.poolRecords = (int)records;
            if ((rc = allocate(s, nVox, &ld.slots))) return rc;
            if ((rc = allocate(s, nVox, &ld.requests))) return rc;
            if ((rc = allocate(s, (size_t)4, &ld.counters))) return rc;
            CUDA_TRY(cudaMemset(ld.slots, 0xff, nVox * sizeof(int)));
            CUDA_TRY(cudaMemset(ld.counters, 0, 4 * sizeof(int)));
            CUDA_TRY(cudaMallocHost((void **)&s->ldHostCounters, 4 * sizeof(int)));
            s->lazyLightDist = true;
        }
    }
    if ((rc = allocate(s, (size_t)CTR_COUNT, &s->counters))) return rc;
    CUDA_TRY(cudaDeviceSynchronize());
    guard.s = nullptr;
    *out = s;
    return PB2_OK;
}

int pb2_intersect(pb2_scene *scene, const pb2_ray *rays, int64_t n, pb2_hit *hits) {
    int rc = requireDevice();
    if (rc) return rc;
    if (!scene || (n > 0 && (!rays || !hits))) return setError(PB2_ERR_INVALID, "null argument");
    if (n <= 0) return PB2_OK;
    pb2_ray *dRays = nullptr;
    pb2_hit *dHits = nullptr;
    CUDA_TRY(cudaMalloc((void **)&dRays, n * sizeof(pb2_ray)));
    cudaError_t e = cudaMalloc((void **)&dHits, n * sizeof(pb2_hit));
    if (e != cudaSuccess) { cudaFree(dRays); return setError(PB2_ERR_CUDA, cudaGetErrorString(e)); }
    e = cudaMemcpy(dRays, rays, n * sizeof(pb2_ray), cudaMemcpyHostToDevice);
    if (e == cudaSuccess) {
        k_intersect<<<(unsigned)((n + 127) / 128), 128>>>(scene->d, dRays, n, dHits);
        e = cudaGetLastError();
    }
    if (e == cudaSuccess) e = cudaMemcpy(hits, dHits, n * sizeof(pb2_hit), cudaMemcpyDeviceToHost);
    cudaFree(dRays);
    cudaFree(dHits);
    if (e != cudaSuccess) return setError(PB2_ERR_CUDA, std::string("pb2_intersect: ") + cudaGetErrorString(e));
    return PB2_OK;
}

int pb2_intersect_p(pb2_scene *scene, const pb2_ray *rays, int64_t n, uint8_t *occluded) {
    int rc = requireDevice();
    if (rc) return rc;
    if (!scene || (n > 0 && (!rays || !occluded))) return setError(PB2_ERR_INVALID, "null argument");
    if (n <= 0) return PB2_OK;
    pb2_ray *dRays = nullptr;
    uint8_t *dOcc = nullptr;
    CUDA_TRY(cudaMalloc((void **)&dRays, n * sizeof(pb2_ray)));
    cudaError_t e = cudaMalloc((void **)&dOcc, n);
    if (e != cudaSuccess) { cudaFree(dRays); return setError(PB2_ERR_CUDA, cudaGetErrorString(e)); }
    e = cudaMemcpy(dRays, rays, n * sizeof(pb2_ray), cudaMemcpyHostToDevice);
    if (e == cudaSuccess) {
        k_intersect_p<<<(unsigned)((n + 127) / 128), 128>>>(scene->d, dRays, n, dOcc);
        e = cudaGetLastError();
    }
    if (e == cudaSuccess) e = cudaMemcpy(occluded, dOcc, n, cudaMemcpyDeviceToHost);
    cudaFree(dRays);
    cudaFree(dOcc);
    if (e != cudaSuccess) return setError(PB2_ERR_CUDA, std::string("pb2_intersect_p: ") + cudaGetErrorString(e));
    return PB2_OK;
}

int pb2_trace_wavefront(pb2_scene *scene, const pb2_ray *rays, const uint8_t *any_hit, int64_t n, int32_t flags, pb2_wf_hit *out) {
    int rc = requireDevice();
    if (rc) return rc;
    if (!scene || (n > 0 && (!rays || !out))) return setError(PB2_ERR_INVALID, "null argument");
    if (n <= 0) return PB2_OK;
    if (n > (1 << 24)) return setError(PB2_ERR_INVALID, "at most 2^24 rays per call");
    const int N = (int)n;
    if ((rc = ensurePool(scene, (N + 255) / 256 * 256))) return rc;
    TraceLaunch trace;
    if ((rc = selectTraceKernel(scene, flags, &trace))) return rc;
    WfPool pool = poolOf(scene, scene->wfCapacity);
    pb2_ray *dRays = nullptr;
    uint8_t *dAny = nullptr;
    pb2_wf_hit *dOut = nullptr;
    cudaError_t e = cudaMalloc((void **)&dRays, n * sizeof(pb2_ray));
    if (e == cudaSuccess) e = cudaMalloc((void **)&dOut, n * sizeof(pb2_wf_hit));
    if (e == cudaSuccess && any_hit) e = cudaMalloc((void **)&dAny, n);
    if (e == cudaSuccess) e = cudaMemcpy(dRays, rays, n * sizeof(pb2_ray), cudaMemcpyHostToDevice);
    if (e == cudaSuccess && any_hit) e = cudaMemcpy(dAny, any_hit, n, cudaMemcpyHostToDevice);
    if (e == cudaSuccess) {
        const int blocks = (N + 127) / 128;
        k_wf_debug_fill<<<blocks, 128>>>(pool, dRays, dAny, N);
        WfChain noChain;
        memset(&noChain, 0, sizeof(noChain));
        trace.fn<<<trace.grid, trace.block, trace.smem>>>(scene->d, pool, WQ_TRACE0, noChain);
        k_wf_debug_read<<<blocks, 128>>>(scene->d, pool, N, dOut);
        k_wf_debug_lists<<<std::min(blocks, g_numSMs * 8), 128>>>(pool, dOut);
        e = cudaGetLastError();
    }
    if (e == cudaSuccess) e = cudaMemcpy(out, dOut, n * sizeof(pb2_wf_hit), cudaMemcpyDeviceToHost);
    cudaFree(dRays);
    cudaFree(dAny);
    cudaFree(dOut);
    if (e != cudaSuccess) return setError(PB2_ERR_CUDA, std::string("pb2_trace_wavefront: ") + cudaGetErrorString(e));
    return PB2_OK;
}

__global__ void k_film_sum_peers(float4 *film, const float4 *p0, const float4 *p1, const float4 *p2, const float4 *p3, const float4 *p4,
                                 const float4 *p5, const float4 *p6, int nPeers, size_t nPixels) {
    const float4 *peers[7] = {p0, p1, p2, p3, p4, p5, p6};
    for (size_t i = blockIdx.x * (size_t)blockDim.x + threadIdx.x; i < nPixels; i += (size_t)gridDim.x * blockDim.x) {
        float4 a = film[i];
        for (int k = 0; k < nPeers; ++k) {
            const float4 b = peers[k][i];
            a.x += b.x; a.y += b.y; a.z += b.z; a.w += b.w;
        }
        film[i] = a;
    }
}

static int ensureFilm(pb2_scene *scene, size_t nFloats) {
    if (scene->filmFloats < nFloats) {
        if (scene->film) cudaFree(scene->film);
        scene->film = nullptr;
        scene->filmFloats = 0;
        CUDA_TRY(cudaMalloc((void **)&scene->film, nFloats * sizeof(float)));
        scene->filmFloats = nFloats;
    }
    return PB2_OK;
}

static int renderPathDeviceOne(pb2_scene *scene, const pb2_camera *cam, const pb2_film_desc *film, const pb2_path_params *pp,
                               float *film_rgbw_device, int clear, void *stream_, pb2_stats *stats);

static int renderPathDeviceGroup(pb2_scene *scene, const pb2_camera *cam, const pb2_film_desc *film, const pb2_path_params *pp,
                                 float *film_rgbw_device, int clear, cudaStream_t stream, pb2_stats *stats) {
    const int n = (int)g_devs.size();
    if (n > 8) return setError(PB2_ERR_UNSUPPORTED, "at most 8 local devices");
    if ((int)scene->replicas.size() != n - 1) return setError(PB2_ERR_INVALID, "the scene was created before pb2_init_devices bound this device group");
    const size_t nPixels = (size_t)(film->cropped_pixel_bounds[2] - film->cropped_pixel_bounds[0]) *
                           (size_t)(film->cropped_pixel_bounds[3] - film->cropped_pixel_bounds[1]);
    std::vector<int> rcs((size_t)n, PB2_OK);
    std::vector<std::string> errs((size_t)n);
    std::vector<pb2_stats> sts((size_t)n);
    std::vector<std::thread> workers;
    CUDA_TRY(cudaStreamSynchronize(stream));
    for (int i = 0; i < n; ++i)
        workers.emplace_back([&, i] {
            t_dev = i;
            pb2_scene *rep = i == 0 ? scene : scene->replicas[(size_t)i - 1];
            int rc = cudaSetDevice(g_devs[(size_t)i].id) == cudaSuccess ? PB2_OK : setError(PB2_ERR_CUDA, "cudaSetDevice failed");
            float *target = film_rgbw_device;
            if (rc == PB2_OK && i > 0) {
                rc = ensureFilm(rep, nPixels * 4);
                target = rep->film;
            }
            pb2_path_params p = *pp;
            p.tile_rank = i;
            p.tile_count = n;
            memset(&sts[(size_t)i], 0, sizeof(pb2_stats));
            if (rc == PB2_OK) rc = renderPathDeviceOne(rep, cam, film, &p, target, i == 0 ? clear : 1, nullptr, &sts[(size_t)i]);
            if (rc == PB2_OK && cudaDeviceSynchronize() != cudaSuccess) rc = setError(PB2_ERR_CUDA, "device synchronisation failed after the render");
            rcs[(size_t)i] = rc;
            errs[(size_t)i] = g_lastError;
        });
    for (std::thread &w : workers) w.join();
    t_dev = 0;
    CUDA_TRY(cudaSetDevice(g_devs[0].id));
    for (int i = 0; i < n; ++i)
        if (rcs[(size_t)i]) return setError(rcs[(size_t)i], "device " + std::to_string(g_devs[(size_t)i].id) + ": " + errs[(size_t)i]);
    const float4 *peers[7] = {nullptr, nullptr, nullptr, nullptr, nullptr, nullptr, nullptr};
    std::vector<float *> staged;
    for (int i = 1; i < n; ++i) {
        pb2_scene *rep = scene->replicas[(size_t)i - 1];
        if (g_devs[(size_t)i].peerOfPrimary) peers[i - 1] = reinterpret_cast<const float4 *>(rep->film);
        else {
            float *tmp = nullptr;
            CUDA_TRY(cudaMalloc((void **)&tmp, nPixels * 16));
            staged.push_back(tmp);
            CUDA_TRY(cudaMemcpyPeerAsync(tmp, g_devs[0].id, rep->film, g_devs[(size_t)i].id, nPixels * 16, stream));
            peers[i - 1] = reinterpret_cast<const float4 *>(tmp);
        }
    }
    const int blocks = (int)std::min<size_t>((nPixels + 255) / 256, (size_t)g_numSMs * 8);
    k_film_sum_peers<<<blocks, 256, 0, stream>>>(reinterpret_cast<float4 *>(film_rgbw_device), peers[0], peers[1], peers[2], peers[3], peers[4],
                                                 peers[5], peers[6], n - 1, nPixels);
    CUDA_TRY(cudaGetLastError());
    CUDA_TRY(cudaStreamSynchronize(stream));
    for (float *t : staged) cudaFree(t);
    if (stats) {
        memset(stats, 0, sizeof(*stats));
        for (const pb2_stats &st : sts) {
            stats->camera_rays += st.camera_rays;
            stats->regular_rays += st.regular_rays;
            stats->shadow_rays += st.shadow_rays;
            stats->node_visits += st.node_visits;
            stats->prim_tests += st.prim_tests;
            stats->kernel_launches += st.kernel_launches;
            stats->render_ms = std::max(stats->render_ms, st.render_ms);
            stats->trace_ms = std::max(stats->trace_ms, st.trace_ms);
        }
        stats->kernel_launches += 1;
    }
    return PB2_OK;
}

int pb2_render_path_device(pb2_scene *scene, const pb2_camera *cam, const pb2_film_desc *film, const pb2_path_params *pp,
                           float *film_rgbw_device, int clear, void *stream_, pb2_stats *stats) {
    int rc = requireDevice();
    if (rc) return rc;
    if ((rc = validateRenderArgs(scene, cam, film, pp))) return rc;
    if (!film_rgbw_device) return setError(PB2_ERR_INVALID, "null film pointer");
    if (pp->tile_count == 0 && g_devs.size() > 1) return renderPathDeviceGroup(scene, cam, film, pp, film_rgbw_device, clear, (cudaStream_t)stream_, stats);
    return renderPathDeviceOne(scene, cam, film, pp, film_rgbw_device, clear, stream_, stats);
}

static int renderPathDeviceOne(pb2_scene *scene, const pb2_camera *cam, const pb2_film_desc *film, const pb2_path_params *pp,
                               float *film_rgbw_device, int clear, void *stream_, pb2_stats *stats) {
    int rc = PB2_OK;
    cudaStream_t stream = (cudaStream_t)stream_;
    const bool distributed = pp->tile_count == 0 && g_dist.world > 1;
    pb2_path_params ppLocal = *pp;
    if (distributed) {
        ppLocal.tile_rank = g_dist.rank;
        ppLocal.tile_count = g_dist.world;
        pp = &ppLocal;
    }
    DRenderParams rp = makeRenderParams(cam, film, pp);
    if (pp->sampler == PB2_SAMPLER_SOBOL && (rc = attachSobol(&rp.halton, film))) return rc;
    {
        float table[256];
        if (computeFilterTable(film, table)) {
            if (!scene->filterTable) CUDA_TRY(cudaMalloc((void **)&scene->filterTable, sizeof(table)));
            CUDA_TRY(cudaMemcpyAsync(scene->filterTable, table, sizeof(table), cudaMemcpyHostToDevice, stream));
            CUDA_TRY(cudaStreamSynchronize(stream));
            rp.filterTable = scene->filterTable;
        }
    }
    size_t nPixels = (size_t)(rp.cx1 - rp.cx0) * (size_t)(rp.cy1 - rp.cy0);
    if (clear) CUDA_TRY(cudaMemsetAsync(film_rgbw_device, 0, nPixels * 4 * sizeof(float), stream));
    CUDA_TRY(cudaMemsetAsync(scene->counters, 0, CTR_COUNT * sizeof(unsigned long long), stream));
    cudaEvent_t e0 = nullptr, e1 = nullptr;
    if (stats) {
        CUDA_TRY(cudaEventCreate(&e0));
        CUDA_TRY(cudaEventCreate(&e1));
        CUDA_TRY(cudaEventRecord(e0, stream));
    }
    unsigned long long launches = 0;
    double traceMs = 0;
    if (rp.nWorkItems > 0) {
        rc = renderWavefront(scene, rp, (float4 *)film_rgbw_device, stream, pp->flags, stats != nullptr, &launches, &traceMs);
        if (rc) {
            if (e0) cudaEventDestroy(e0);
            if (e1) cudaEventDestroy(e1);
            return rc;
        }
    }
// ... 796 lines not shown
```

### pbrt_v3_b200/csrc/pb2_wavefront.cuh

```cuda
#ifndef PB2_WAVEFRONT_CUH
#define PB2_WAVEFRONT_CUH

struct alignas(32) WfCtx {
    DLane ln;
    alignas(16) float4 hit;
    float tHit;
    int found;
    V2 pFilm;
};
static_assert(offsetof(WfCtx, ln) == 0 && offsetof(DLane, state) == 0 && offsetof(DLane, ray) == 4 && sizeof(DRay) == 28,
              "the trace kernels read the first 32 bytes of a context as {state, o, d, tMax}");
static_assert(offsetof(WfCtx, tHit) % 8 == 0 && offsetof(WfCtx, found) == offsetof(WfCtx, tHit) + 4, "tHit/found are stored as one float2");
static_assert(sizeof(DLane) == 192 && offsetof(WfCtx, hit) == 192 && offsetof(WfCtx, tHit) == 208 && offsetof(WfCtx, pFilm) == 216 &&
                  sizeof(WfCtx) == 224 && sizeof(WfCtx) % 32 == 0,
              "a context is seven whole 32-byte sectors: the lane (six), then hit, tHit / found and pFilm (one)");

struct WfSlot {
    DLane ln;
    float hit[4];
    float tHit;
    int found;
    V2 pFilm;
    int pad[2];
};
static_assert(offsetof(WfSlot, hit) == offsetof(WfCtx, hit) && offsetof(WfSlot, tHit) == offsetof(WfCtx, tHit) &&
                  offsetof(WfSlot, found) == offsetof(WfCtx, found) && offsetof(WfSlot, pFilm) == offsetof(WfCtx, pFilm) &&
                  sizeof(WfSlot) == 232 && alignof(WfSlot) == 8,
              "a slot holds a context's bytes at the context's offsets, 8-byte aligned, 58 words apart");

enum { WF_OUT_START = 96, WF_OUT_LIGHT = 128, WF_OUT_SHADE = (int)sizeof(DLane) };
static_assert(offsetof(DLane, lightNum) == 88 && offsetof(DLane, pick) == 92 && offsetof(DLane, ldSum) == 96 && offsetof(DLane, ldLight) == 108 &&
                  offsetof(DLane, bounces) < 96 && offsetof(DLane, misTerm) == 120,
              "the written-back prefixes above cover the fields their kernels change");

__device__ __forceinline__ int wfLaneId() {
    int lane;
    asm volatile("mov.u32 %0, %%laneid;" : "=r"(lane));
    return lane;
}

enum { WF_IN_ALL = 0x7f, WF_IN_SHADE = 0x47 };
static_assert(offsetof(DLane, etaScale) + sizeof(float) <= 96 && offsetof(DLane, smp) + sizeof(DSampler) <= 96 &&
                  offsetof(DLane, ldSum) == 96 && offsetof(DLane, betaNext) + sizeof(V3) <= 192 && offsetof(WfCtx, hit) == 192 &&
                  offsetof(WfCtx, pFilm) + sizeof(V2) <= 224,
              "WF_IN_SHADE: the fields shadeVertex reads on entry lie in sectors 0-2 and 6, the dead ones in sectors 3-5");

template <unsigned SECTORS>
__device__ __forceinline__ int wfStagedChunk(int kk) {
    if (SECTORS == WF_IN_ALL) return kk;
    const int n = kk >> 1;
    int s = 0, seen = 0;
#pragma unroll
    for (int t = 0; t < 7; ++t)
        if ((SECTORS >> t) & 1u) {
            s = n == seen ? t : s;
            ++seen;
        }
    return 2 * s + (kk & 1);
}

template <unsigned SECTORS = WF_IN_ALL>
__device__ __forceinline__ void wfStageIn(const WfCtx *ctx, WfSlot *warpSlots, int c) {
    constexpr int NSECT = ((SECTORS >> 0) & 1) + ((SECTORS >> 1) & 1) + ((SECTORS >> 2) & 1) + ((SECTORS >> 3) & 1) +
                          ((SECTORS >> 4) & 1) + ((SECTORS >> 5) & 1) + ((SECTORS >> 6) & 1);
    static_assert(SECTORS <= WF_IN_ALL && NSECT > 0, "sectors of a 224-byte context");
    constexpr int CHUNKS = 2 * NSECT, BATCH = NSECT;
    const int lane = wfLaneId();
    __syncwarp();
#pragma unroll
    for (int b = 0; b < 2; ++b) {
        uint4 v[BATCH];
        int cs[BATCH];
#pragma unroll
        for (int it = 0; it < BATCH; ++it) {
            const int q = (b * BATCH + it) * 32 + lane, j = q / CHUNKS, kk = q % CHUNKS;
            const int k = wfStagedChunk<SECTORS>(kk);
            cs[it] = __shfl_sync(0xffffffffu, c, j);
            if (cs[it] >= 0) v[it] = __ldcs(reinterpret_cast<const uint4 *>(ctx + cs[it]) + k);
        }
#pragma unroll
        for (int it = 0; it < BATCH; ++it) {
            const int q = (b * BATCH + it) * 32 + lane, j = q / CHUNKS, kk = q % CHUNKS;
            const int k = wfStagedChunk<SECTORS>(kk);
            if (cs[it] >= 0) {
                uint2 *s = reinterpret_cast<uint2 *>(reinterpret_cast<char *>(&warpSlots[j]) + 16 * k);
                s[0] = make_uint2(v[it].x, v[it].y);
                s[1] = make_uint2(v[it].z, v[it].w);
            }
        }
    }
    __syncwarp();
}

template <int BYTES>
__device__ __forceinline__ void wfStageOut(WfCtx *ctx, const WfSlot *warpSlots, int c) {
    static_assert(BYTES % 32 == 0 && BYTES <= (int)sizeof(DLane), "whole sectors of the lane");
    constexpr int CHUNKS = BYTES / 16;
    const int lane = wfLaneId();
    __syncwarp();
#pragma unroll
    for (int it = 0; it < CHUNKS; ++it) {
        const int q = it * 32 + lane, j = q / CHUNKS, k = q % CHUNKS;
        const int cj = __shfl_sync(0xffffffffu, c, j);
        if (cj >= 0) {
            const uint2 *s = reinterpret_cast<const uint2 *>(reinterpret_cast<const char *>(&warpSlots[j]) + 16 * k);
            const uint2 lo = s[0], hi = s[1];
            __stcs(reinterpret_cast<uint4 *>(ctx + cj) + k, make_uint4(lo.x, lo.y, hi.x, hi.y));
        }
    }
    __syncwarp();
}

enum { WQ_TRACE0 = 0, WQ_TRACE1 = 1, WQ_SHADE = 2, WQ_LIGHT = 3, WQ_FREE0 = 4, WQ_FREE1 = 5, WQ_CURSOR = 6, WQ_RETRY = 7, WQ_COUNT = 8 };
enum { WQ_FINISH = WQ_RETRY, WF_FINISH_WAIT = 1, WF_FINISH_GO = 2 };

struct WfPool {
    int capacity;
    WfCtx *ctx;
    int *queue[WQ_COUNT];
    unsigned *counts;
    unsigned long long *ctr;
    int2 *spill;
};

__device__ __forceinline__ int *wfQueue(const WfPool &pool, int q) {
    int *list = pool.queue[0];
#pragma unroll
    for (int k = 1; k < WQ_COUNT; ++k) {
        int *entry = pool.queue[k];
        asm("" : "+l"(entry));
        list = q == k ? entry : list;
    }
    return list;
}

__device__ __forceinline__ void wfPush(int *queue, unsigned *counter, int value, bool participate) {
    unsigned mask = __ballot_sync(0xffffffffu, participate);
    if (!mask) return;
    int lane = threadIdx.x & 31;
    int leader = __ffs(mask) - 1;
    unsigned base = 0;
    if (lane == leader) base = atomicAdd(counter, (unsigned)__popc(mask));
    base = __shfl_sync(0xffffffffu, base, leader);
    if (participate) queue[base + __popc(mask & ((1u << lane) - 1u))] = value;
}

__device__ __forceinline__ void wfCountRays(unsigned long long *counters, unsigned regular, unsigned shadow) {
    for (int o = 16; o > 0; o >>= 1) {
        regular += __shfl_down_sync(0xffffffffu, regular, o);
        shadow += __shfl_down_sync(0xffffffffu, shadow, o);
    }
    if ((threadIdx.x & 31) == 0) {
        if (regular) atomicAdd(&counters[CTR_REGULAR], (unsigned long long)regular);
        if (shadow) atomicAdd(&counters[CTR_SHADOW], (unsigned long long)shadow);
    }
}

struct WfChain {
    const DScene *sc;
    const DRenderParams *rp;
    float4 *film;
    int freeQ;
    int pad;
};

template <int F>
__device__ __noinline__ int wfChainLight(const WfChain &ch, WfCtx *cx, bool found) {
    DLane &ln = cx->ln;
    const float4 h4 = cx->hit;
    const int foundCode = cx->found;
    DHit hit;
    hit.leaf = __float_as_int(h4.x);
    hit.b0 = h4.y;
    hit.b1 = h4.z;
    hit.b2 = h4.w;
    hit.inst = foundCode >= 2 ? foundCode - 2 : -1;
    lightAdvance<F>(*ch.sc, ln, found, hit, cx->tHit);
    if (ln.state == LS_IDLE) addSample(*ch.rp, ch.film, cx->pFilm, guardRadiance(ln.L));
    return ln.state;
}

template <bool GENERAL>
__device__ __forceinline__ bool wfStartSample(const DRenderParams &rp, const WfPool &pool, WfSlot &slot, bool want, unsigned *cameraRays) {
    bool started = false;
    while (__any_sync(0xffffffffu, want && !started)) {
        const bool draw = want && !started;
        const unsigned mask = __ballot_sync(0xffffffffu, draw);
        const int lane = threadIdx.x & 31, leader = __ffs(mask) - 1;
        unsigned long long w0 = 0;
        if (lane == leader) w0 = atomicAdd(&pool.ctr[CTR_WORK], (unsigned long long)__popc(mask));
        w0 = __shfl_sync(0xffffffffu, w0, leader);
        if (draw) {
            const long long item = (long long)w0 + __popc(mask & ((1u << lane) - 1u));
            if (item >= rp.nWorkItems) {
                want = false;
            } else {
                int px, py, sample;
                if (decodeWork(rp, item, &px, &py, &sample)) {
                    DSampler smp;
                    smp.index = sampleIndex<GENERAL>(rp.halton, px, py, sample);
                    smp.dim = 0;
                    V2 pFilm;
                    DRay ray = generateCameraRay<GENERAL>(rp.cam, rp.halton, smp, px, py, &pFilm);
                    laneStartPath(slot.ln, ray, smp);
                    slot.pFilm = pFilm;
                    ++*cameraRays;
                    started = true;
                }
            }
        }
    }
    return started;
}

template <int F>
__global__ void __launch_bounds__(128) k_wf_gen(const DRenderParams *__restrict__ rpp, WfPool pool, int freeQ, int traceQ) {
    __shared__ WfSlot stage[128];
    WfSlot &slot = stage[threadIdx.x];
    WfSlot *warpSlots = stage + (threadIdx.x & ~31u);
    const DRenderParams &rp = *rpp;
    const int *freeList = wfQueue(pool, freeQ);
    int *traceList = wfQueue(pool, traceQ);
    const unsigned n = pool.counts[freeQ];
    unsigned stride = gridDim.x * blockDim.x;
    unsigned cameraRays = 0;
    for (unsigned base = blockIdx.x * blockDim.x; base < n; base += stride) {
        unsigned i = base + threadIdx.x;
        const bool have = i < n;
        const int c = have ? freeList[i] : -1;
        const bool started = wfStartSample<(F & SHADE_SOBOL) != 0>(rp, pool, slot, have, &cameraRays);
        if (started) {
            slot.ln.lightNum = 0;
            slot.ln.pick = 0;
            __stcs(reinterpret_cast<float2 *>(&pool.ctx[c].pFilm), make_float2(slot.pFilm.x, slot.pFilm.y));
        }
        wfStageOut<WF_OUT_START>(pool.ctx, warpSlots, started ? c : -1);
        wfPush(traceList, &pool.counts[traceQ], c, started);
    }
    for (int o = 16; o > 0; o >>= 1) cameraRays += __shfl_down_sync(0xffffffffu, cameraRays, o);
    if ((threadIdx.x & 31) == 0 && cameraRays) {
        atomicAdd(&pool.ctr[CTR_CAMERA], (unsigned long long)cameraRays);
        atomicAdd(&pool.ctr[CTR_REGULAR], (unsigned long long)cameraRays);
    }
}

enum {
    TRACE_SPHERES = 1,
    TRACE_INST = 2,
    TRACE_ALPHA = 4,
    TRACE_LD128 = 8,
    TRACE_SMALL_STACK = 16,
    TRACE_LEAF_TMA = 32,
    TRACE_CHAIN = 64,
    TRACE_DEEP = 128,
};

template <bool COUNT>
__global__ void __launch_bounds__(128) k_wf_trace_plain(DScene sc, WfPool pool, int traceQ, WfChain) {
    unsigned long long *counters = pool.ctr;
    unsigned n = pool.counts[traceQ];
    unsigned stride = gridDim.x * blockDim.x;
    DCounters ctr;
    ctr.nodes = ctr.prims = 0;
    for (unsigned base = blockIdx.x * blockDim.x; base < n; base += stride) {
        unsigned i = base + threadIdx.x;
        bool have = i < n;
        int c = have ? pool.queue[traceQ][i] : 0;
        int state = LS_IDLE;
        if (have) {
            const float4 *p = reinterpret_cast<const float4 *>(&pool.ctx[c]);
            float4 a = p[0], b = p[1];
            state = __float_as_int(a.x);
            DRay ray;
            ray.o = mk3(a.y, a.z, a.w);
            ray.d = mk3(b.x, b.y, b.z);
            ray.tMax = b.w;
            float tMax = ray.tMax;
            DHit hit;
            hit.leaf = -1;
            hit.b0 = hit.b1 = hit.b2 = 0;
            hit.inst = -1;
            bool found = traverseAnyOrClosest(sc, ray, state == LS_SHADOW, &tMax, &hit, COUNT ? &ctr : nullptr);
            WfCtx &cx = pool.ctx[c];
            cx.hit = make_float4(__int_as_float(hit.leaf), hit.b0, hit.b1, hit.b2);
            cx.tHit = tMax;
            cx.found = found ? (state != LS_SHADOW && hit.inst >= 0 ? 2 + hit.inst : 1) : 0;
        }
        wfPush(pool.queue[WQ_SHADE], &pool.counts[WQ_SHADE], c, have && state == LS_PATH);
        wfPush(pool.queue[WQ_LIGHT], &pool.counts[WQ_LIGHT], c, have && state != LS_PATH);
    }
    if (COUNT) {
        unsigned long long n0 = ctr.nodes, n1 = ctr.prims;
        for (int o = 16; o > 0; o >>= 1) {
            n0 += __shfl_down_sync(0xffffffffu, n0, o);
            n1 += __shfl_down_sync(0xffffffffu, n1, o);
        }
        if ((threadIdx.x & 31) == 0) {
            atomicAdd(&counters[CTR_NODES], n0);
            atomicAdd(&counters[CTR_PRIMS], n1);
        }
    }
}

template <int T>
__global__ void __launch_bounds__(128, (T & TRACE_SPHERES) ? 6 : 8) k_wf_trace(DScene sc, WfPool pool, int traceQ, WfChain) {
    static constexpr bool SPHERES = (T & TRACE_SPHERES) != 0, INST = (T & TRACE_INST) != 0, DEEP = (T & TRACE_DEEP) != 0;
    static constexpr int LEAF_T = SPHERES ? 8 : 12, FETCH_T = 8, NSUB = SPHERES ? 2 : 4, SDEPTH = 32;
    __shared__ int sstack[SDEPTH][128];
    int lstack[DEEP ? 64 - SDEPTH : 1];
    const unsigned FULL = 0xffffffffu;
    const int tid = threadIdx.x;
    const int lane = tid & 31;
    const unsigned n = pool.counts[traceQ];
    enum { M_FETCH = 0, M_NODE = 1, M_LEAF = 2 };
    enum { F_ANY = 1, F_FOUND = 2, F_EXHAUSTED = 4, F_EXIT = 8, F_HITIN = 16 };
    int inst = -1, hitInst = -1, instBase = 0;
    int mode = M_FETCH;
    int c = -1;
    int flags = 0;
    DRaySetup rs;
    rs.o = rs.invDir = mk3(0, 0, 0);
    rs.neg0 = rs.neg1 = rs.neg2 = 0;
    rs.kx = rs.ky = rs.kz = 0;
    rs.Sx = rs.Sy = rs.Sz = 0;
    float tMax = 0;
    int cur = 0, sp = 0, leafFirst = 0, leafN = 0;
    auto stackGet = [&](int slot) -> int { return (!DEEP || slot < SDEPTH) ? sstack[slot][tid] : lstack[DEEP ? slot - SDEPTH : 0]; };
    auto stackPut = [&](int slot, int v) {
        if (!DEEP || slot < SDEPTH) sstack[slot][tid] = v;
        else lstack[DEEP ? slot - SDEPTH : 0] = v;
    };
    while (true) {
        unsigned mNode = __ballot_sync(FULL, mode == M_NODE);
        unsigned mLeaf = __ballot_sync(FULL, mode == M_LEAF);
        unsigned mFetch = __ballot_sync(FULL, mode == M_FETCH && !((flags & F_EXHAUSTED) && c < 0));
        int nNode = __popc(mNode), nLeaf = __popc(mLeaf), nFetch = __popc(mFetch);
        int step;
        if (nFetch >= FETCH_T || (nFetch > 0 && nNode == 0 && nLeaf == 0)) step = M_FETCH;
        else if (nLeaf >= LEAF_T || (nLeaf > 0 && nNode == 0)) step = M_LEAF;
        else if (nNode > 0) step = M_NODE;
        else break;

        if (step == M_NODE) {
#pragma unroll
            for (int sub = 0; sub < NSUB; ++sub) {
                if (mode == M_NODE) {
                    float4 n0 = ldg4(&sc.nodes[2 * (size_t)cur]);
                    float4 n1 = ldg4(&sc.nodes[2 * (size_t)cur + 1]);
                    bool pass = slabTest(n0, n1, rs, tMax);
                    uint32_t meta = floatBits(n1.w);
                    int nPrims = (int)(meta & 0xffffu);
                    int axis = (int)((meta >> 16) & 0xffu);
                    int isNeg = axis == 0 ? rs.neg0 : (axis == 1 ? rs.neg1 : rs.neg2);
                    int second = asInt(n1.z);
                    bool interior = pass && nPrims == 0;
                    bool leaf = pass && nPrims > 0;
                    int far = isNeg ? cur + 1 : second;
                    int near = isNeg ? second : cur + 1;
                    int slot = interior ? sp : (sp > 0 ? sp - 1 : 0);
                    int top = stackGet(slot);
                    if (interior) stackPut(slot, far);
                    if (interior) {
                        cur = near;
                        ++sp;
                    } else if (leaf) {
                        leafFirst = second;
                        leafN = nPrims;
                        mode = M_LEAF;
                    } else if (sp == instBase) {
                        if (INST && inst >= 0) {
                            mode = M_LEAF;
                            flags |= F_EXIT;
                            leafN = 0;
                        } else
                            mode = M_FETCH;
                    } else {
                        cur = top;
                        --sp;
                    }
                }
            }
        } else if (step == M_LEAF) {
            if (mode == M_LEAF) {
                if (INST && (flags & F_EXIT)) {
                    flags &= ~F_EXIT;
                    sp -= 3;
                    float saved = __int_as_float(stackGet(sp));
                    leafFirst = stackGet(sp + 1);
                    leafN = stackGet(sp + 2);
                    if (!(flags & F_HITIN)) tMax = saved;
                    const float4 *p = reinterpret_cast<const float4 *>(&pool.ctx[c]);
                    float4 ra = p[0], rb = p[1];
                    rs = setupRay(mk3(ra.y, ra.z, ra.w), mk3(rb.x, rb.y, rb.z));
                    inst = -1;
                    instBase = 0;
                }
                bool finished = false, entered = false;
                const bool any = (flags & F_ANY) != 0;
                while (leafN > 0) {
                    const int idx = leafFirst;
                    ++leafFirst;
                    --leafN;
                    const float4 *rec = &sc.leafPrims[3 * (size_t)idx];
                    float4 a = ldg4(rec), b = ldg4(rec + 1), c4 = ldg4(rec + 2);
                    uint32_t pf = floatBits(b.w);
                    if (INST && (pf & LEAF_INSTANCE)) {
                        const int id = asInt(c4.w);
                        const DInstance &in = sc.instances[id];
                        const float4 *p = reinterpret_cast<const float4 *>(&pool.ctx[c]);
                        float4 ra = p[0], rb = p[1];
                        DRay ray;
                        ray.o = mk3(ra.y, ra.z, ra.w);
                        ray.d = mk3(rb.x, rb.y, rb.z);
                        ray.tMax = rb.w;
                        DRay r2 = xfRay(in.w2i, ray, tMax);
                        stackPut(sp, __float_as_int(tMax));
                        stackPut(sp + 1, leafFirst);
                        stackPut(sp + 2, leafN);
                        sp += 3;
                        instBase = sp;
                        inst = id;
                        flags &= ~F_HITIN;
                        rs = setupRay(r2.o, r2.d);
                        tMax = r2.tMax;
                        if (in.root >= 0) {
                            cur = in.root;
                            mode = M_NODE;
                            leafN = 0;
                            entered = true;
                            break;
                        }
                        leafFirst = in.lone;
                        leafN = 1;
                        continue;
                    }
                    if (SPHERES && (pf & LEAF_SPHERE)) {
                        const float4 *p = reinterpret_cast<const float4 *>(&pool.ctx[c]);
                        float4 ra = p[0], rb = p[1];
                        DRay ray;
                        ray.o = mk3(ra.y, ra.z, ra.w);
                        ray.d = mk3(rb.x, rb.y, rb.z);
                        ray.tMax = rb.w;
                        if (INST && inst >= 0) ray = xfRay(sc.instances[inst].w2i, ray, tMax);
                        float t, phi;
                        if (sphereLeafTest(sc, asInt(c4.w), ray, tMax, &t, &phi)) {
                            flags |= F_FOUND;
                            if (any) { finished = true; break; }
                            tMax = t;
                            if (INST) {
                                hitInst = inst;
                                if (inst >= 0) flags |= F_HITIN;
                            }
                            __stcs(reinterpret_cast<float4 *>(&pool.ctx[c].hit), make_float4(__int_as_float(idx), phi, 0.f, 0.f));
                        }
                        continue;
                    }
                    float t, b0, b1, b2;
                    if (triangleTest(mk3(a.x, a.y, a.z), mk3(b.x, b.y, b.z), mk3(c4.x, c4.y, c4.z), rs, tMax, &t, &b0, &b1, &b2)) {
                        if (any) { flags |= F_FOUND; finished = true; break; }
                        if (pf & LEAF_DEGENERATE) continue;
                        flags |= F_FOUND;
                        tMax = t;
                        if (INST) {
                            hitInst = inst;
                            if (inst >= 0) flags |= F_HITIN;
                        }
                        __stcs(reinterpret_cast<float4 *>(&pool.ctx[c].hit), make_float4(__int_as_float(idx), b0, b1, b2));
                    }
                }
                if (!entered) {
                    leafN = 0;
                    if (finished) mode = M_FETCH;
                    else if (sp == instBase) {
                        if (INST && inst >= 0) flags |= F_EXIT;
                        else mode = M_FETCH;
                    } else {
                        --sp;
                        cur = stackGet(sp);
                        mode = M_NODE;
                    }
                }
            }
        } else {
            bool flush = mode == M_FETCH && c >= 0;
            int state = LS_IDLE;
            if (flush) {
                WfCtx &cx = pool.ctx[c];
                state = (flags & F_ANY) ? LS_SHADOW : __ldcs(&cx.ln.state);
                const int foundCode = (flags & F_FOUND) ? ((INST && !(flags & F_ANY) && hitInst >= 0) ? 2 + hitInst : 1) : 0;
                __stcs(reinterpret_cast<float2 *>(&cx.tHit), make_float2(tMax, __int_as_float(foundCode)));
            }
            wfPush(pool.queue[WQ_SHADE], &pool.counts[WQ_SHADE], c, flush && state == LS_PATH);
            wfPush(pool.queue[WQ_LIGHT], &pool.counts[WQ_LIGHT], c, flush && state != LS_PATH);
            if (flush) c = -1;
            bool want = mode == M_FETCH && !(flags & F_EXHAUSTED);
            unsigned wantMask = __ballot_sync(FULL, want);
            if (wantMask) {
                int leader = __ffs(wantMask) - 1;
                unsigned base = 0;
                if (lane == leader) base = atomicAdd(&pool.counts[WQ_CURSOR], (unsigned)__popc(wantMask));
                base = __shfl_sync(FULL, base, leader);
                if (want) {
                    unsigned i = base + __popc(wantMask & ((1u << lane) - 1u));
                    if (i >= n)
                        flags |= F_EXHAUSTED;
                    else {
                        c = pool.queue[traceQ][i];
                        const float4 *p = reinterpret_cast<const float4 *>(&pool.ctx[c]);
                        float4 ra = __ldcs(p), rb = __ldcs(p + 1);
                        flags = (__float_as_int(ra.x) == LS_SHADOW) ? F_ANY : 0;
                        rs = setupRay(mk3(ra.y, ra.z, ra.w), mk3(rb.x, rb.y, rb.z));
                        tMax = rb.w;
                        cur = 0;
                        sp = 0;
                        leafN = 0;
                        mode = M_NODE;
                        if (INST) {
                            inst = hitInst = -1;
                            instBase = 0;
                        }
                    }
                }
            }
        }
    }
}

constexpr int traceMinBlocks(int width, int t) {
    if (width == 4) return (t & TRACE_SPHERES) ? 5 : 7;
    if (t & TRACE_LEAF_TMA) return 5;
    return (t & (TRACE_SPHERES | TRACE_ALPHA)) ? 6 : 9;
}
template <int WIDTH, int T>
__global__ void __launch_bounds__(128, traceMinBlocks(WIDTH, T)) k_wf_trace_w(DScene sc, WfPool pool, int traceQ, WfChain chain) {
    static_assert(WIDTH == 2 || WIDTH == 4, "two- or four-child records");
    static constexpr bool SPHERES = (T & TRACE_SPHERES) != 0, INST = (T & TRACE_INST) != 0, ALPHA = (T & TRACE_ALPHA) != 0;
    static constexpr bool LD128 = (T & TRACE_LD128) != 0, LEAFTMA = (T & TRACE_LEAF_TMA) != 0, CHAIN = (T & TRACE_CHAIN) != 0;
    static_assert(!LEAFTMA || (!SPHERES && !INST), "the staging experiment covers triangle scenes");
    static constexpr int LEAF_T = 1, FETCH_T = 8, NSUB = 4, SDEPTH = (T & TRACE_SMALL_STACK) ? 4 : 16;
    constexpr int STAGED = 4;
    __shared__ alignas(16) float4 sleaf[LEAFTMA ? 128 * 3 * STAGED : 1];
    __shared__ alignas(8) unsigned long long sbar[LEAFTMA ? 4 : 1];
    unsigned barPhase = 0;
    if (LEAFTMA) {
        if ((threadIdx.x & 31) == 0) {
            const unsigned bar = (unsigned)__cvta_generic_to_shared(&sbar[threadIdx.x >> 5]);
            asm volatile("mbarrier.init.shared::cta.b64 [%0], 1;" ::"r"(bar));
            asm volatile("fence.mbarrier_init.release.cluster;" ::: "memory");
        }
        __syncwarp();
    }
    constexpr int BLOCK = 128;
    __shared__ int2 sstack[SDEPTH * BLOCK];
    __shared__ unsigned sCount[2];
    if (CHAIN) {
        if (threadIdx.x < 2) sCount[threadIdx.x] = 0;
        __syncthreads();
    }
    int2 lstack[(WIDTH == 4 ? 100 : 66) - SDEPTH];
    const unsigned FULL = 0xffffffffu;
    const int tid = threadIdx.x;
    const int lane = tid & 31;
    const unsigned n = pool.counts[traceQ];
    enum { M_FETCH = 0, M_NODE = 1, M_LEAF = 2 };
    enum { F_ANY = 1, F_FOUND = 2, F_EXHAUSTED = 4, F_EXIT = 8, F_HITIN = 16 };
    int inst = -1, hitInst = -1, instBase = 0;
    auto stGet = [&](int i) -> int2 { return i < SDEPTH ? sstack[i * BLOCK + tid] : lstack[i - SDEPTH]; };
    auto stPut = [&](int i, int2 e) {
        if (i < SDEPTH) sstack[i * BLOCK + tid] = e;
        else lstack[i - SDEPTH] = e;
    };
    int mode = M_FETCH;
    int c = -1;
    int flags = 0;
    DRaySetup rs;
    rs.o = rs.invDir = mk3(0, 0, 0);
    rs.neg0 = rs.neg1 = rs.neg2 = 0;
    rs.kx = rs.ky = rs.kz = 0;
    rs.Sx = rs.Sy = rs.Sz = 0;
    rs.slow = 0;
    float tMax = 0;
    int cur = 0, sp = 0, leafFirst = 0, leafN = 0;
    while (true) {
        unsigned mNode = __ballot_sync(FULL, mode == M_NODE);
        unsigned mLeaf = __ballot_sync(FULL, mode == M_LEAF);
        unsigned mFetch = __ballot_sync(FULL, mode == M_FETCH && !((flags & F_EXHAUSTED) && c < 0));
        int nNode = __popc(mNode), nLeaf = __popc(mLeaf), nFetch = __popc(mFetch);
        int step;
        if (nFetch >= FETCH_T || (nFetch > 0 && nNode == 0 && nLeaf == 0)) step = M_FETCH;
        else if (nLeaf >= LEAF_T || (nLeaf > 0 && nNode == 0)) step = M_LEAF;
        else if (nNode > 0) step = M_NODE;
        else break;

        if (step == M_NODE) {
            const bool warpSlow = __any_sync(FULL, rs.slow != 0);
#pragma unroll
            for (int sub = 0; sub < NSUB; ++sub) {
                {
                    const bool need = (mode == M_NODE) & (cur < 0);
                    const bool empty = need & (sp == instBase);
                    const bool pop = need & !empty;
                    const int slot = pop ? sp - 1 : 0;
                    const int2 e = slot < SDEPTH ? sstack[slot * BLOCK + tid] : lstack[slot - SDEPTH];
                    sp = pop ? sp - 1 : sp;
                    const bool take = pop & (__int_as_float(e.y) < tMax);
                    const bool leafRef = take & (e.x < 0);
                    leafFirst = leafRef ? (e.x & (int)WIDE_LEAF_OFFSET_MASK) : leafFirst;
                    leafN = leafRef ? (((e.x >> WIDE_LEAF_COUNT_SHIFT) & 0xf) + 1) : leafN;
                    cur = (take & !leafRef) ? e.x : cur;
                    mode = leafRef ? (int)M_LEAF : mode;
                    if (empty) {
                        if (INST && inst >= 0) {
                            mode = M_LEAF;
                            flags |= F_EXIT;
                            leafN = 0;
                        } else
                            mode = M_FETCH;
                    }
                }
                if (WIDTH == 4) {
                    if (mode == M_NODE && cur >= 0) {
                        const float4 *w = &sc.wide4[8 * (size_t)cur];
                        float4 q0, q1, q2, q3, q4, q5, q6, q7;
                        if (!LD128) {
                            ldg256(w, q0, q1);
                            ldg256(w + 2, q2, q3);
                            ldg256(w + 4, q4, q5);
                            ldg256(w + 6, q6, q7);
                        } else {
                            q0 = ldg4(w); q1 = ldg4(w + 1); q2 = ldg4(w + 2); q3 = ldg4(w + 3); q4 = ldg4(w + 4); q5 = ldg4(w + 5);
                            q6 = ldg4(w + 6);
                            q7.x = __uint_as_float(__ldg(reinterpret_cast<const unsigned *>(w + 7)));
                        }
                        const uint32_t meta = floatBits(q7.x);
                        const Wide4Visit v = warpSlow ? wide4Visit<false>(q0, q1, q2, q3, q4, q5, q6, meta, rs, tMax)
                                                      : wide4Visit<true>(q0, q1, q2, q3, q4, q5, q6, meta, rs, tMax);
                        const int refs[4] = {asInt(q6.x), asInt(q6.y), asInt(q6.z), asInt(q6.w)};
                        const int last = v.nPass - 1;
                        int ref = -1;
#pragma unroll
                        for (int k = 0; k < 4; ++k) {
                            const bool first = v.pass[k] & (v.after[k] == last);
                            ref = first ? refs[k] : ref;
                            const bool deferred = v.pass[k] & !first;
                            const int slot = sp + v.after[k];
                            const int2 e = make_int2(refs[k], __float_as_int(v.tMin[k]));
                            if (deferred & (slot < SDEPTH)) sstack[slot * BLOCK + tid] = e;
                            if (deferred & (slot >= SDEPTH)) lstack[slot - SDEPTH] = e;
                        }
                        sp += last > 0 ? last : 0;
                        const bool have = v.nPass > 0;
                        const bool isLeaf = have & (ref < 0);
                        leafFirst = isLeaf ? (ref & (int)WIDE_LEAF_OFFSET_MASK) : leafFirst;
                        leafN = isLeaf ? (((ref >> WIDE_LEAF_COUNT_SHIFT) & 0xf) + 1) : leafN;
                        mode = isLeaf ? (int)M_LEAF : (int)M_NODE;
                        cur = (have & !isLeaf) ? ref : -1;
                    }
                } else if (mode == M_NODE && cur >= 0) {
                    const float4 *w = &sc.wide[4 * (size_t)cur];
                    float4 q0, q1, q2, q3;
                    if (!LD128) {
                        ldg256(w, q0, q1);
                        ldg256(w + 2, q2, q3);
                    } else {
                        q0 = ldg4(w); q1 = ldg4(w + 1); q2 = ldg4(w + 2); q3 = ldg4(w + 3);
                    }
                    float t0, t1;
                    bool p0, p1;
                    if (warpSlow) slabTestPair(q0, q1, q2, rs, tMax, &p0, &p1, &t0, &t1);
                    else slabTestPairFast(q0, q1, q2, rs, tMax, &p0, &p1, &t0, &t1);
                    const uint32_t meta = floatBits(q3.z);
                    if (meta & WIDE_SINGLE) p1 = false;
                    const int axis = (int)(meta & 3u);
                    const bool isNeg = (axis == 0 ? rs.neg0 : (axis == 1 ? rs.neg1 : rs.neg2)) != 0;
                    const int ref0 = asInt(q3.x), ref1 = asInt(q3.y);
                    const bool both = p0 & p1;
                    {
                        const int2 e = make_int2(isNeg ? ref0 : ref1, __float_as_int(isNeg ? t0 : t1));
                        if (both & (sp < SDEPTH)) sstack[sp * BLOCK + tid] = e;
                        if (both & (sp >= SDEPTH)) lstack[sp - SDEPTH] = e;
                        sp += both ? 1 : 0;
                    }
                    const int ref = (both ? isNeg : !p0) ? ref1 : ref0;
                    const bool have = p0 | p1;
                    const bool isLeaf = have & (ref < 0);
                    leafFirst = isLeaf ? (ref & (int)WIDE_LEAF_OFFSET_MASK) : leafFirst;
                    leafN = isLeaf ? (((ref >> WIDE_LEAF_COUNT_SHIFT) & 0xf) + 1) : leafN;
                    mode = isLeaf ? (int)M_LEAF : (int)M_NODE;
                    cur = (have & !isLeaf) ? ref : -1;
                }
            }
        } else if (step == M_LEAF) {
            int stagedN = 0;
            if (LEAFTMA) {
                const unsigned bar = (unsigned)__cvta_generic_to_shared(&sbar[tid >> 5]);
                stagedN = (mode == M_LEAF) ? min(leafN, STAGED) : 0;
                unsigned bytes = (unsigned)stagedN * 48u;
                for (int o = 16; o > 0; o >>= 1) bytes += __shfl_xor_sync(FULL, bytes, o);
                asm volatile("fence.proxy.async.shared::cta;" ::: "memory");
                if (lane == 0) asm volatile("mbarrier.arrive.expect_tx.shared::cta.b64 _, [%0], %1;" ::"r"(bar), "r"(bytes) : "memory");
                __syncwarp();
                if (stagedN > 0) {
                    const unsigned dst = (unsigned)__cvta_generic_to_shared(&sleaf[tid * STAGED * 3]);
                    const float4 *src = &sc.leafPrims[3 * (size_t)leafFirst];
                    asm volatile("cp.async.bulk.shared::cluster.global.mbarrier::complete_tx::bytes [%0], [%1], %2, [%3];" ::"r"(dst), "l"(src),
                                 "r"((unsigned)stagedN * 48u), "r"(bar)
                                 : "memory");
                }
                unsigned done = 0;
                while (!done)
                    asm volatile("{ .reg .pred p; mbarrier.try_wait.parity.shared::cta.b64 p, [%1], %2; selp.u32 %0, 1, 0, p; }"
                                 : "=r"(done)
                                 : "r"(bar), "r"(barPhase)
                                 : "memory");
                barPhase ^= 1u;
            }
            if (mode == M_LEAF) {
                if (INST && (flags & F_EXIT)) {
                    flags &= ~F_EXIT;
                    sp -= 2;
                    const int2 rest = stGet(sp), saved = stGet(sp + 1);
                    leafFirst = rest.x;
                    leafN = rest.y;
                    if (!(flags & F_HITIN)) tMax = __int_as_float(saved.x);
                    const float4 *p = reinterpret_cast<const float4 *>(&pool.ctx[c]);
                    float4 ra = p[0], rb = p[1];
                    rs = setupRay(mk3(ra.y, ra.z, ra.w), mk3(rb.x, rb.y, rb.z));
                    inst = -1;
                    instBase = 0;
                }
                bool finished = false, entered = false;
                const bool any = (flags & F_ANY) != 0;
                int staged = 0;
                while (leafN > 0) {
                    const int idx = leafFirst;
                    ++leafFirst;
                    --leafN;
                    const float4 *rec = &sc.leafPrims[3 * (size_t)idx];
                    float4 a, b, c4;
                    if (LEAFTMA && staged < stagedN) {
                        const float4 *sl = &sleaf[(tid * STAGED + staged) * 3];
                        a = sl[0]; b = sl[1]; c4 = sl[2];
                        ++staged;
                    } else {
                        a = ldg4(rec); b = ldg4(rec + 1); c4 = ldg4(rec + 2);
                    }
                    uint32_t pf = floatBits(b.w);
                    if (INST && (pf & LEAF_INSTANCE)) {
                        const int id = asInt(c4.w);
                        const DInstance &in = sc.instances[id];
                        const float4 *p = reinterpret_cast<const float4 *>(&pool.ctx[c]);
                        float4 ra = p[0], rb = p[1];
                        DRay ray;
                        ray.o = mk3(ra.y, ra.z, ra.w);
                        ray.d = mk3(rb.x, rb.y, rb.z);
                        ray.tMax = rb.w;
                        DRay r2 = xfRay(in.w2i, ray, tMax);
                        stPut(sp, make_int2(leafFirst, leafN));
                        stPut(sp + 1, make_int2(__float_as_int(tMax), 0));
                        sp += 2;
                        instBase = sp;
                        inst = id;
                        flags &= ~F_HITIN;
                        rs = setupRay(r2.o, r2.d);
                        tMax = r2.tMax;
                        if (in.wroot >= 0) {
                            cur = WIDTH == 4 ? in.wroot4 : in.wroot;
                            mode = M_NODE;
                            leafN = 0;
                            entered = true;
                            break;
                        }
                        leafFirst = in.lone;
                        leafN = 1;
                        continue;
                    }
                    if (SPHERES && (pf & LEAF_SPHERE)) {
                        const float4 *p = reinterpret_cast<const float4 *>(&pool.ctx[c]);
                        float4 ra = p[0], rb = p[1];
                        DRay ray;
                        ray.o = mk3(ra.y, ra.z, ra.w);
                        ray.d = mk3(rb.x, rb.y, rb.z);
                        ray.tMax = rb.w;
                        if (INST && inst >= 0) ray = xfRay(sc.instances[inst].w2i, ray, tMax);
                        float t, phi;
                        if (sphereLeafTest(sc, asInt(c4.w), ray, tMax, &t, &phi)) {
                            flags |= F_FOUND;
                            if (any) { finished = true; break; }
                            tMax = t;
                            if (INST) {
                                hitInst = inst;
                                if (inst >= 0) flags |= F_HITIN;
                            }
                            __stcs(reinterpret_cast<float4 *>(&pool.ctx[c].hit), make_float4(__int_as_float(idx), phi, 0.f, 0.f));
                        }
                        continue;
                    }
                    float t, b0, b1, b2;
                    if (triangleTest(mk3(a.x, a.y, a.z), mk3(b.x, b.y, b.z), mk3(c4.x, c4.y, c4.z), rs, tMax, &t, &b0, &b1, &b2)) {
                        if (ALPHA && (pf & LEAF_ALPHA) && alphaRejects(sc, asInt(a.w), b0, b1, b2, any)) continue;
                        if (any) { flags |= F_FOUND; finished = true; break; }
                        if (pf & LEAF_DEGENERATE) continue;
                        flags |= F_FOUND;
                        tMax = t;
                        if (INST) {
                            hitInst = inst;
                            if (inst >= 0) flags |= F_HITIN;
                        }
                        __stcs(reinterpret_cast<float4 *>(&pool.ctx[c].hit), make_float4(__int_as_float(idx), b0, b1, b2));
                    }
                }
                if (!entered) {
                    leafN = 0;
                    if (finished) mode = M_FETCH;
                    else if (sp == instBase) {
                        if (INST && inst >= 0) flags |= F_EXIT;
                        else mode = M_FETCH;
                    } else {
                        mode = M_NODE;
                        cur = -1;
                    }
                }
            }
        } else {
            bool flush = mode == M_FETCH && c >= 0;
            int state = LS_IDLE;
            if (flush) {
                WfCtx &cx = pool.ctx[c];
                state = (flags & F_ANY) ? LS_SHADOW : __ldcs(&cx.ln.state);
                const int foundCode = (flags & F_FOUND) ? ((INST && !(flags & F_ANY) && hitInst >= 0) ? 2 + hitInst : 1) : 0;
                __stcs(reinterpret_cast<float2 *>(&cx.tHit), make_float2(tMax, __int_as_float(foundCode)));
            }
            wfPush(pool.queue[WQ_SHADE], &pool.counts[WQ_SHADE], c, flush && state == LS_PATH);
            bool again = false;
            if (CHAIN) {
                int next = LS_PATH;
                if (flush && state != LS_PATH) {
                    next = wfChainLight<SHADE_GENERAL | (SPHERES ? SHADE_SPHERES : 0)>(chain, &pool.ctx[c], (flags & F_FOUND) != 0);
                    again = next != LS_IDLE;
                }
                const unsigned mShadow = __ballot_sync(FULL, again && next == LS_SHADOW), mRegular = __ballot_sync(FULL, again && next != LS_SHADOW);
                if (lane == 0) {
                    if (mShadow) atomicAdd(&sCount[1], (unsigned)__popc(mShadow));
                    if (mRegular) atomicAdd(&sCount[0], (unsigned)__popc(mRegular));
                }
                wfPush(pool.queue[chain.freeQ], &pool.counts[chain.freeQ], c, flush && state != LS_PATH && !again);
            } else
                wfPush(pool.queue[WQ_LIGHT], &pool.counts[WQ_LIGHT], c, flush && state != LS_PATH);
            if (again) {
                const float4 *p = reinterpret_cast<const float4 *>(&pool.ctx[c]);
                const float4 ra = p[0], rb = p[1];
                flags = (__float_as_int(ra.x) == LS_SHADOW) ? F_ANY : 0;
                rs = setupRay(mk3(ra.y, ra.z, ra.w), mk3(rb.x, rb.y, rb.z));
                tMax = rb.w;
                cur = 0;
                if (INST) {
                    inst = hitInst = -1;
                    instBase = 0;
                }
                sp = 0;
                leafN = 0;
                mode = M_NODE;
            } else if (flush)
                c = -1;
            bool want = mode == M_FETCH && !(flags & F_EXHAUSTED);
            unsigned wantMask = __ballot_sync(FULL, want);
            if (wantMask) {
                int leader = __ffs(wantMask) - 1;
                unsigned base = 0;
                if (lane == leader) base = atomicAdd(&pool.counts[WQ_CURSOR], (unsigned)__popc(wantMask));
                base = __shfl_sync(FULL, base, leader);
                if (want) {
                    unsigned i = base + __popc(wantMask & ((1u << lane) - 1u));
                    if (i >= n)
                        flags |= F_EXHAUSTED;
                    else {
                        c = pool.queue[traceQ][i];
                        const float4 *p = reinterpret_cast<const float4 *>(&pool.ctx[c]);
                        float4 ra = __ldcs(p), rb = __ldcs(p + 1);
                        flags = (__float_as_int(ra.x) == LS_SHADOW) ? F_ANY : 0;
                        rs = setupRay(mk3(ra.y, ra.z, ra.w), mk3(rb.x, rb.y, rb.z));
                        tMax = rb.w;
                        cur = 0;
                        if (INST) {
                            inst = hitInst = -1;
                            instBase = 0;
                        }
                        sp = 0;
                        leafN = 0;
                        mode = M_NODE;
                    }
                }
            }
        }
    }
    if (CHAIN) {
        __syncthreads();
        if (threadIdx.x == 0) {
            if (sCount[0]) atomicAdd(&pool.ctr[CTR_REGULAR], (unsigned long long)sCount[0]);
            if (sCount[1]) atomicAdd(&pool.ctr[CTR_SHADOW], (unsigned long long)sCount[1]);
        }
    }
}

enum { PL_EMPTY = 0, PL_NODE = 1, PL_LEAF = 2, PL_DONE = 3, PL_R = 64, PL_SPILL = 64 };
enum { PL_RAYS = 48, PL_SD = 8 };
struct PoolWarp {
    float f[10][PL_RAYS];
    int i[6][PL_RAYS];
    int2 stk[PL_SD][PL_RAYS];
    int list[PL_RAYS];
};

__global__ void __launch_bounds__(128, 8) k_wf_trace_pool(DScene sc, WfPool pool, int traceQ, WfChain) {
    static_assert(PL_RAYS > 32 && PL_RAYS <= PL_R, "a warp owns 33 .. 64 slots");
    static constexpr int NSUB = 4, LEAF_T = 16, FILL_T = 12;
    extern __shared__ unsigned char poolSmemRaw[];
    PoolWarp &pw = reinterpret_cast<PoolWarp *>(poolSmemRaw)[threadIdx.x >> 5];
    const bool second = (threadIdx.x & 31) + 32 < PL_RAYS;
    const unsigned FULL = 0xffffffffu;
    const int lane = threadIdx.x & 31;
    const unsigned ltMask = (1u << lane) - 1u;
    const unsigned n = pool.counts[traceQ];
    int2 *spill = pool.spill + ((size_t)(blockIdx.x * 4 + (threadIdx.x >> 5)) * PL_R) * PL_SPILL;
    pw.i[3][lane] = 0;
    if (second) pw.i[3][lane + 32] = 0;
    __syncwarp();
    bool exhausted = false;
    auto stGet = [&](int s, int d) -> int2 { return d < PL_SD ? pw.stk[d][s] : spill[(size_t)s * PL_SPILL + (d - PL_SD)]; };
    auto stPut = [&](int s, int d, int2 e) {
        if (d < PL_SD) pw.stk[d][s] = e;
        else spill[(size_t)s * PL_SPILL + (d - PL_SD)] = e;
    };
    while (true) {
        const int fl0 = pw.i[3][lane], fl1 = second ? pw.i[3][lane + 32] : -1;
        const int m0 = (fl0 >> 12) & 3, m1 = second ? ((fl1 >> 12) & 3) : -1;
        const unsigned bN0 = __ballot_sync(FULL, m0 == PL_NODE), bN1 = __ballot_sync(FULL, m1 == PL_NODE);
        const unsigned bL0 = __ballot_sync(FULL, m0 == PL_LEAF), bL1 = __ballot_sync(FULL, m1 == PL_LEAF);
        const unsigned bD0 = __ballot_sync(FULL, m0 == PL_DONE), bD1 = __ballot_sync(FULL, m1 == PL_DONE);
        const int nN = __popc(bN0) + __popc(bN1), nL = __popc(bL0) + __popc(bL1), nD = __popc(bD0) + __popc(bD1);
        const int nE = PL_RAYS - nN - nL - nD;
        int phase;
        if (nD + (exhausted ? 0 : nE) >= FILL_T || (nN == 0 && nL == 0 && (nD > 0 || (!exhausted && nE > 0)))) phase = PL_DONE;
        else if (nL >= LEAF_T || (nL > 0 && nN == 0)) phase = PL_LEAF;
        else if (nN > 0) phase = PL_NODE;
        else break;

        if (phase == PL_DONE) {
#pragma unroll 1
            for (int h = 0; h < 2; ++h) {
                const bool exists = h == 0 || second;
                const int s = exists ? lane + 32 * h : lane;
                const int fl = exists ? pw.i[3][s] : (PL_NODE << 12);
                const int mode = (fl >> 12) & 3;
                const bool flush = mode == PL_DONE;
                int c = flush ? pw.i[2][s] : -1;
                int state = LS_IDLE;
                if (flush) {
                    WfCtx &cx = pool.ctx[c];
                    state = (fl & 1) ? LS_SHADOW : __ldcs(&cx.ln.state);
                    __stcs(reinterpret_cast<float2 *>(&cx.tHit), make_float2(pw.f[6][s], __int_as_float((fl & 2) ? 1 : 0)));
                }
                wfPush(pool.queue[WQ_SHADE], &pool.counts[WQ_SHADE], c, flush && state == LS_PATH);
                wfPush(pool.queue[WQ_LIGHT], &pool.counts[WQ_LIGHT], c, flush && state != LS_PATH);
                bool want = (flush || mode == PL_EMPTY) && !exhausted;
                const unsigned wantMask = __ballot_sync(FULL, want);
                int newFlags = 0;
                if (wantMask) {
                    const int leader = __ffs(wantMask) - 1;
                    unsigned base = 0;
                    if (lane == leader) base = atomicAdd(&pool.counts[WQ_CURSOR], (unsigned)__popc(wantMask));
                    base = __shfl_sync(FULL, base, leader);
                    const unsigned idx = base + __popc(wantMask & ltMask);
                    if (want && idx < n) {
                        c = pool.queue[traceQ][idx];
                        const float4 *p = reinterpret_cast<const float4 *>(&pool.ctx[c]);
                        const float4 ra = __ldcs(p), rb = __ldcs(p + 1);
                        const DRaySetup rs = setupRay(mk3(ra.y, ra.z, ra.w), mk3(rb.x, rb.y, rb.z));
                        pw.f[0][s] = rs.o.x; pw.f[1][s] = rs.o.y; pw.f[2][s] = rs.o.z;
                        pw.f[3][s] = rs.invDir.x; pw.f[4][s] = rs.invDir.y; pw.f[5][s] = rs.invDir.z;
                        pw.f[6][s] = rb.w;
                        pw.f[7][s] = rs.Sx; pw.f[8][s] = rs.Sy; pw.f[9][s] = rs.Sz;
                        pw.i[0][s] = 0;
                        pw.i[1][s] = 0;
                        pw.i[2][s] = c;
                        newFlags = ((__float_as_int(ra.x) == LS_SHADOW) ? 1 : 0) | (rs.neg0 << 2) | (rs.neg1 << 3) | (rs.neg2 << 4) | (rs.kx << 5) |
                                   (rs.ky << 7) | (rs.kz << 9) | (rs.slow << 11) | (PL_NODE << 12);
                    }
                    if (__any_sync(FULL, want && idx >= n)) exhausted = true;
                }
                if (flush || want) pw.i[3][s] = newFlags;
            }
            __syncwarp();
            continue;
        }

        const unsigned b0 = phase == PL_NODE ? bN0 : bL0, b1 = phase == PL_NODE ? bN1 : bL1;
        const int c0 = __popc(b0);
        if (b0 & (1u << lane)) pw.list[__popc(b0 & ltMask)] = lane;
        if (b1 & (1u << lane)) pw.list[c0 + __popc(b1 & ltMask)] = lane + 32;
        __syncwarp();
        const int nSel = min(c0 + __popc(b1), 32);
        const bool active = lane < nSel;
        const int s = active ? pw.list[lane] : 0;
        __syncwarp();

        if (phase == PL_NODE) {
            DRaySetup rs;
            rs.o = mk3(pw.f[0][s], pw.f[1][s], pw.f[2][s]);
            rs.invDir = mk3(pw.f[3][s], pw.f[4][s], pw.f[5][s]);
            float tMax = pw.f[6][s];
            int cur = pw.i[0][s], sp = pw.i[1][s];
            int fl = pw.i[3][s];
            rs.neg0 = (fl >> 2) & 1; rs.neg1 = (fl >> 3) & 1; rs.neg2 = (fl >> 4) & 1;
            rs.kx = rs.ky = rs.kz = 0;
            rs.Sx = rs.Sy = rs.Sz = 0;
            rs.slow = (fl >> 11) & 1;
            int mode = active ? (int)PL_NODE : (int)PL_EMPTY;
            int leafFirst = 0, leafN = 0;
            const bool warpSlow = __any_sync(FULL, active && rs.slow != 0);
#pragma unroll
            for (int sub = 0; sub < NSUB; ++sub) {
                {
                    const bool need = (mode == PL_NODE) & (cur < 0);
                    const bool empty = need & (sp == 0);
                    const bool pop = need & !empty;
                    int2 e = make_int2(0, 0);
                    if (pop) e = stGet(s, sp - 1);
                    sp = pop ? sp - 1 : sp;
                    const bool take = pop & (__int_as_float(e.y) < tMax);
                    const bool leafRef = take & (e.x < 0);
                    leafFirst = leafRef ? (e.x & (int)WIDE_LEAF_OFFSET_MASK) : leafFirst;
                    leafN = leafRef ? (((e.x >> WIDE_LEAF_COUNT_SHIFT) & 0xf) + 1) : leafN;
                    cur = (take & !leafRef) ? e.x : cur;
                    mode = leafRef ? (int)PL_LEAF : mode;
                    if (empty) mode = PL_DONE;
                }
                if (mode == PL_NODE && cur >= 0) {
                    const float4 *w = &sc.wide[4 * (size_t)cur];
                    float4 q0, q1, q2, q3;
                    ldg256(w, q0, q1);
                    ldg256(w + 2, q2, q3);
                    float t0, t1;
                    bool p0, p1;
                    if (warpSlow) slabTestPair(q0, q1, q2, rs, tMax, &p0, &p1, &t0, &t1);
                    else slabTestPairFast(q0, q1, q2, rs, tMax, &p0, &p1, &t0, &t1);
                    const uint32_t meta = floatBits(q3.z);
                    if (meta & WIDE_SINGLE) p1 = false;
                    const int axis = (int)(meta & 3u);
                    const bool isNeg = (axis == 0 ? rs.neg0 : (axis == 1 ? rs.neg1 : rs.neg2)) != 0;
                    const int ref0 = asInt(q3.x), ref1 = asInt(q3.y);
                    const bool both = p0 & p1;
                    if (both) stPut(s, sp, make_int2(isNeg ? ref0 : ref1, __float_as_int(isNeg ? t0 : t1)));
                    sp += both ? 1 : 0;
                    const int ref = (both ? isNeg : !p0) ? ref1 : ref0;
                    const bool have = p0 | p1;
                    const bool isLeaf = have & (ref < 0);
                    leafFirst = isLeaf ? (ref & (int)WIDE_LEAF_OFFSET_MASK) : leafFirst;
                    leafN = isLeaf ? (((ref >> WIDE_LEAF_COUNT_SHIFT) & 0xf) + 1) : leafN;
                    mode = isLeaf ? (int)PL_LEAF : (int)PL_NODE;
                    cur = (have & !isLeaf) ? ref : -1;
                }
            }
            if (active) {
                pw.i[0][s] = cur;
                pw.i[1][s] = sp;
                pw.i[3][s] = (fl & 0xfff) | (mode << 12);
                pw.i[4][s] = leafFirst;
                pw.i[5][s] = leafN;
            }
        } else {
            if (active) {
                DRaySetup rs;
                rs.o = mk3(pw.f[0][s], pw.f[1][s], pw.f[2][s]);
                rs.invDir = mk3(0, 0, 0);
                float tMax = pw.f[6][s];
                rs.Sx = pw.f[7][s]; rs.Sy = pw.f[8][s]; rs.Sz = pw.f[9][s];
                int fl = pw.i[3][s];
                rs.neg0 = rs.neg1 = rs.neg2 = 0;
                rs.kx = (fl >> 5) & 3; rs.ky = (fl >> 7) & 3; rs.kz = (fl >> 9) & 3;
                rs.slow = 0;
                const int c = pw.i[2][s];
                int leafFirst = pw.i[4][s], leafN = pw.i[5][s];
                const bool any = (fl & 1) != 0;
                bool finished = false;
                while (leafN > 0) {
                    const int idx = leafFirst;
                    ++leafFirst;
                    --leafN;
                    const float4 *rec = &sc.leafPrims[3 * (size_t)idx];
                    const float4 a = ldg4(rec), b = ldg4(rec + 1), c4 = ldg4(rec + 2);
                    const uint32_t pf = floatBits(b.w);
                    float t, b0, b1, b2;
                    if (triangleTest(mk3(a.x, a.y, a.z), mk3(b.x, b.y, b.z), mk3(c4.x, c4.y, c4.z), rs, tMax, &t, &b0, &b1, &b2)) {
                        if (any) { fl |= 2; finished = true; break; }
                        if (pf & LEAF_DEGENERATE) continue;
                        fl |= 2;
                        tMax = t;
                        __stcs(reinterpret_cast<float4 *>(&pool.ctx[c].hit), make_float4(__int_as_float(idx), b0, b1, b2));
                    }
                }
                const int sp = pw.i[1][s];
                const int mode = (finished || sp == 0) ? (int)PL_DONE : (int)PL_NODE;
                pw.f[6][s] = tMax;
                pw.i[0][s] = -1;
                pw.i[3][s] = (fl & 0xfff) | (mode << 12);
            }
        }
        __syncwarp();
    }
}

template <bool SHADE, int MINB, int F>
__global__ void __launch_bounds__(128, MINB) k_wf_advance(const DScene *__restrict__ scp, const DRenderParams *__restrict__ rpp, WfPool pool,
                                                          int srcQ, int traceQ, int freeQ, float4 *film, unsigned long long *counters) {
    __shared__ WfSlot stage[128];
    __shared__ float sampleRows[SHADE ? 128 * (kSampleBatch + 1) : 1];
    WfSlot &slot = stage[threadIdx.x];
    WfSlot *warpSlots = stage + (threadIdx.x & ~31u);
    float *u = sampleRows + (SHADE ? threadIdx.x * (kSampleBatch + 1) : 0);
    const DScene &sc = *scp;
    const DRenderParams &rp = *rpp;
    const int *srcList = wfQueue(pool, srcQ);
    int *traceList = wfQueue(pool, traceQ), *freeList = wfQueue(pool, freeQ);
    unsigned n = pool.counts[srcQ];
    unsigned stride = gridDim.x * blockDim.x;
    unsigned regular = 0, shadow = 0;
    for (unsigned base = blockIdx.x * blockDim.x; base < n; base += stride) {
        unsigned i = base + threadIdx.x;
        bool have = i < n;
        int c = have ? srcList[i] : 0;
        bool ended = false, deferred = false;
        wfStageIn<SHADE ? WF_IN_SHADE : WF_IN_ALL>(pool.ctx, warpSlots, have ? c : -1);
        if (have) {
            DLane &ln = slot.ln;
            const int foundCode = slot.found;
            DHit hit;
            hit.leaf = __float_as_int(slot.hit[0]);
            hit.b0 = slot.hit[1];
            hit.b1 = slot.hit[2];
            hit.b2 = slot.hit[3];
            hit.inst = foundCode >= 2 ? foundCode - 2 : -1;
            bool found = foundCode != 0;
            float tHit = slot.tHit;
            if (SHADE && (F & SHADE_TEXTURES)) {
                DTexCtx tc;
                tc.cam = &rp.cam;
                tc.pFilm = slot.pFilm;
                tc.diffScale = rp.diffScale;
                shadeVertex<F>(sc, rp.halton, rp.path, ln, found, hit, tHit, u, &tc);
            } else if (SHADE) shadeVertex<F>(sc, rp.halton, rp.path, ln, found, hit, tHit, u);
            else lightAdvance<F>(sc, ln, found, hit, tHit);
            if (SHADE && (F & SHADE_LAZY) && ln.state == LS_DEFER) {
                ln.state = LS_PATH;
                deferred = true;
            } else {
                ended = ln.state == LS_IDLE;
                if (ended) addSample(rp, film, slot.pFilm, guardRadiance(ln.L));
                else if (ln.state == LS_SHADOW) shadow++;
                else regular++;
            }
        }
        wfStageOut<SHADE ? WF_OUT_SHADE : WF_OUT_LIGHT>(pool.ctx, warpSlots, have && !ended ? c : -1);
        if (SHADE && (F & SHADE_LAZY)) wfPush(pool.queue[WQ_RETRY], &pool.counts[WQ_RETRY], c, deferred);
        wfPush(traceList, &pool.counts[traceQ], c, have && !ended && !deferred);
        wfPush(freeList, &pool.counts[freeQ], c, have && ended);
    }
    wfCountRays(counters, regular, shadow);
}

__device__ __forceinline__ bool wfFinishNow(const DRenderParams &rp, const WfPool &pool, int traceQ, unsigned threshold) {
    const unsigned n = pool.counts[traceQ];
    return n > 0 && n <= threshold && (long long)pool.ctr[CTR_WORK] >= rp.nWorkItems;
}

template <int F>
__global__ void __launch_bounds__(128) k_wf_finish(const DScene *__restrict__ scp, const DRenderParams *__restrict__ rpp, WfPool pool, int traceQ,
                                                   unsigned threshold, float4 *film) {
    const DScene &sc = *scp;
    const DRenderParams &rp = *rpp;
    __shared__ bool sGo;
    if (threadIdx.x == 0) {
        const unsigned mine = wfFinishNow(rp, pool, traceQ, threshold) ? WF_FINISH_GO : WF_FINISH_WAIT;
        const unsigned first = atomicCAS(&pool.counts[WQ_FINISH], 0u, mine);
        sGo = (first ? first : mine) == WF_FINISH_GO;
    }
    __syncthreads();
    if (!sGo) return;
    const unsigned n = pool.counts[traceQ];
    const int *traceList = wfQueue(pool, traceQ);
    unsigned regular = 0, shadow = 0;
    for (unsigned i = blockIdx.x * blockDim.x + threadIdx.x; i < n; i += gridDim.x * blockDim.x) {
        WfCtx &cx = pool.ctx[traceList[i]];
        DLane &ln = cx.ln;
        while (ln.state != LS_IDLE) {
            DHit hit;
            float tMax;
            const bool found = traceLane(sc, ln, &tMax, &hit, nullptr);
            laneAdvance<F>(sc, rp.halton, rp.path, ln, found, hit, tMax);
            if (ln.state == LS_DEFER) break;
            if (ln.state == LS_SHADOW) shadow++;
            else if (ln.state != LS_IDLE) regular++;
        }
        addSample(rp, film, cx.pFilm, guardRadiance(ln.L));
    }
    wfCountRays(pool.ctr, regular, shadow);
}

__global__ void __launch_bounds__(128) k_lightdist_build(DScene sc, DHalton h) {
    const DLightDist &ld = sc.lightDist;
    const int nReq = ld.counters[0];
    __shared__ int sRecord;
    for (int r = blockIdx.x; r < nReq; r += gridDim.x) {
        const int voxel = ld.requests[r];
        if (threadIdx.x == 0) {
            int k = atomicAdd(&ld.counters[1], 1);
            if (k >= ld.poolRecords) {
                ld.counters[2] = 1;
                k = -1;
            }
            sRecord = k;
        }
        __syncthreads();
        const int k = sRecord;
        if (k >= 0) {
            float *rec = const_cast<float *>(ld.table) + (size_t)k * ld.stride;
            const int pz = voxel % ld.nVoxels[2], py = (voxel / ld.nVoxels[2]) % ld.nVoxels[1], px = voxel / (ld.nVoxels[2] * ld.nVoxels[1]);
            const DVoxelBounds vb = voxelBounds(ld, px, py, pz);
            for (int j = threadIdx.x; j < sc.nLights; j += blockDim.x) rec[j] = voxelLightContribution(sc, h, vb, j);
            __syncthreads();
            if (threadIdx.x == 0) {
                finishVoxelDistribution(sc.nLights, rec);
                __threadfence();
                ld.slots[voxel] = k;
            }
        }
        __syncthreads();
    }
}
__global__ void k_lightdist_done(DScene sc) {
    if (threadIdx.x == 0 && blockIdx.x == 0) sc.lightDist.counters[0] = 0;
}

__global__ void k_wf_init(WfPool pool) {
    unsigned i = blockIdx.x * blockDim.x + threadIdx.x;
    if (i < (unsigned)pool.capacity) pool.queue[WQ_FREE0][i] = (int)i;
    if (i < WQ_COUNT) pool.counts[i] = (i == WQ_FREE0) ? (unsigned)pool.capacity : 0u;
}

__global__ void k_wf_reset(WfPool pool, int a, int b, int traceNext, unsigned threshold) {
    if (threadIdx.x == 0) {
        if (threshold && pool.counts[WQ_FINISH] == WF_FINISH_GO) pool.counts[traceNext] = 0;
        pool.counts[WQ_RETRY] = 0;
        pool.counts[WQ_CURSOR] = 0;
        pool.counts[WQ_SHADE] = 0;
        pool.counts[WQ_LIGHT] = 0;
        pool.counts[a] = 0;
        pool.counts[b] = 0;
    }
}

#endif
```

Measured before the change: 222.8.

## Split wavefront trace queue into separate path and shadow lists with specialized kernels

Advance kernels now push rays into separate path and shadow trace queues, and the render loop launches a closest-hit trace kernel for path rays and an any-hit trace kernel for shadow rays. The aim is to remove per-ray branching between any-hit and closest-hit logic inside one kernel and to reduce warp divergence. Each specialization can also be compiled more tightly. The cost is an extra kernel launch per round, extra queue bookkeeping and cursors, and more compiled kernel variants.

```diff
diff --git a/include/pb2.h b/include/pb2.h
--- a/include/pb2.h
+++ b/include/pb2.h
@@ -8,7 +8,7 @@
 extern "C" {
 #endif
 
-#define PB2_ABI_VERSION 10
+#define PB2_ABI_VERSION 11
 
 typedef enum pb2_status {
     PB2_OK = 0,
@@ -294,6 +294,8 @@
 int pb2_trace_wavefront(pb2_scene *scene, const pb2_ray *rays, const uint8_t *any_hit, int64_t n, int32_t flags,
                         pb2_wf_hit *out);
 
+int pb2_wavefront_round(int32_t cur, int32_t split, int32_t tail, uint32_t *counts, int32_t *lists_out, int32_t *n_counts);
+
 int pb2_li_samples(pb2_scene *scene, const pb2_camera *camera, const pb2_film_desc *film,
                    const pb2_path_params *params, const int32_t *pixel_xy, const int64_t *sample_num,
                    int64_t n, float *out_rgb, float *out_pfilm);
diff --git a/pbrt_v3_b200/__init__.py b/pbrt_v3_b200/__init__.py
--- a/pbrt_v3_b200/__init__.py
+++ b/pbrt_v3_b200/__init__.py
@@ -15,7 +15,7 @@
 PB2_PRIM_TRIANGLE, PB2_PRIM_SPHERE, PB2_PRIM_INSTANCE = 0, 1, 2
 PB2_FILTER_BOX, PB2_FILTER_GAUSSIAN, PB2_FILTER_MITCHELL, PB2_FILTER_SINC, PB2_FILTER_TRIANGLE = 0, 1, 2, 3, 4
 PB2_MAT_NONE, PB2_MAT_MATTE, PB2_MAT_PLASTIC, PB2_MAT_MIRROR, PB2_MAT_GLASS, PB2_MAT_SUBSTRATE, PB2_MAT_METAL, PB2_MAT_UBER = range(8)
-PB2_ABI_VERSION = 10
+PB2_ABI_VERSION = 11
 PB2_LIGHTDIST_UNIFORM, PB2_LIGHTDIST_POWER, PB2_LIGHTDIST_SPATIAL = 0, 1, 2
 PB2_LIGHT_AREA, PB2_LIGHT_POINT, PB2_LIGHT_SPOT, PB2_LIGHT_DISTANT, PB2_LIGHT_INFINITE = 0, 1, 2, 3, 4
 
@@ -177,6 +177,7 @@
     L.pb2_intersect.argtypes = [vp, vp, C.c_int64, vp]
     L.pb2_intersect_p.argtypes = [vp, vp, C.c_int64, vp]
     L.pb2_trace_wavefront.argtypes = [vp, vp, vp, C.c_int64, C.c_int32, vp]
+    L.pb2_wavefront_round.argtypes = [C.c_int32, C.c_int32, C.c_int32, vp, vp, vp]
     L.pb2_work_items.argtypes = [C.POINTER(FilmDesc), C.POINTER(PathParams), C.c_int64, C.c_int64, vp, C.POINTER(C.c_int64)]
     L.pb2_init_devices.argtypes = [C.c_int, C.POINTER(C.c_int)]
     L.pb2_dist_unique_id.argtypes = [vp]
diff --git a/pbrt_v3_b200/csrc/pb2_cuda.cu b/pbrt_v3_b200/csrc/pb2_cuda.cu
--- a/pbrt_v3_b200/csrc/pb2_cuda.cu
+++ b/pbrt_v3_b200/csrc/pb2_cuda.cu
@@ -601,22 +601,26 @@
     }
 }
 
-__global__ void k_wf_debug_fill(WfPool pool, const pb2_ray *rays, const uint8_t *anyHit, int n) {
+__global__ void k_wf_debug_fill(WfPool pool, const pb2_ray *rays, const uint8_t *anyHit, int n, int shadowQ) {
     int i = blockIdx.x * blockDim.x + threadIdx.x;
-    if (i == 0) {
-        for (int q = 0; q < WQ_COUNT; ++q) pool.counts[q] = 0;
-        pool.counts[WQ_TRACE0] = (unsigned)n;
-    }
-    if (i >= n) return;
-    WfCtx &cx = pool.ctx[i];
-    cx.ln.state = (anyHit && anyHit[i]) ? LS_SHADOW : LS_PATH;
-    cx.ln.ray.o = mk3(rays[i].o[0], rays[i].o[1], rays[i].o[2]);
-    cx.ln.ray.d = mk3(rays[i].d[0], rays[i].d[1], rays[i].d[2]);
-    cx.ln.ray.tMax = rays[i].t_max;
-    cx.hit = make_float4(__int_as_float(-1), 0.f, 0.f, 0.f);
-    cx.tHit = 0.f;
-    cx.found = -1;
-    pool.queue[WQ_TRACE0][i] = i;
+    const bool have = i < n;
+    const int state = (have && anyHit && anyHit[i]) ? LS_SHADOW : LS_PATH;
+    if (have) {
+        WfCtx &cx = pool.ctx[i];
+        cx.ln.state = state;
+        cx.ln.ray.o = mk3(rays[i].o[0], rays[i].o[1], rays[i].o[2]);
+        cx.ln.ray.d = mk3(rays[i].d[0], rays[i].d[1], rays[i].d[2]);
+        cx.ln.ray.tMax = rays[i].t_max;
+        cx.hit = make_float4(__int_as_float(-1), 0.f, 0.f, 0.f);
+        cx.tHit = 0.f;
+        cx.found = -1;
+    }
+    if (shadowQ != WQ_TRACE0) {
+        wfPushTrace(pool, WQ_TRACE0, shadowQ, i, state, have);
+        return;
+    }
+    if (i == 0) pool.counts[WQ_TRACE0] = (unsigned)n;
+    if (have) pool.queue[WQ_TRACE0][i] = i;
 }
 __global__ void k_wf_debug_read(DScene sc, WfPool pool, int n, pb2_wf_hit *out) {
     int i = blockIdx.x * blockDim.x + threadIdx.x;
@@ -804,7 +808,7 @@
 
 enum { kMaxPipes = 4 };
 typedef void (*TraceKernel)(DScene, WfPool, int, WfChain);
-typedef void (*AdvanceKernel)(const DScene *, const DRenderParams *, WfPool, int, int, int, float4 *, unsigned long long *);
+typedef void (*AdvanceKernel)(const DScene *, const DRenderParams *, WfPool, int, int, int, int, float4 *, unsigned long long *);
 
 struct TraceLaunch {
     TraceKernel fn = nullptr;
@@ -825,10 +829,11 @@
 };
 template <int WIDTH, int T>
 static TraceKernelEntry wideTrace() {
+    const bool any = (T & TRACE_ANY) != 0;
     const char *name = WIDTH == 4              ? "k_wf_trace_w<4>"
-                       : (T & TRACE_ALPHA) ? "k_wf_trace_w<2,alpha>"
+                       : (T & TRACE_ALPHA) ? (any ? "k_wf_trace_w<2,alpha,any>" : "k_wf_trace_w<2,alpha>")
                        : (T & TRACE_CHAIN) ? "k_wf_trace_w<2,chain>"
-                                           : "k_wf_trace_w<2>";
+                                           : (any ? "k_wf_trace_w<2,any>" : "k_wf_trace_w<2>");
     return {WIDTH == 4 ? TK_WIDE4 : TK_WIDE2, T, k_wf_trace_w<WIDTH, T>, name, 0};
 }
 template <int T>
@@ -837,6 +842,7 @@
 struct TraceKey {
     TraceKernelForm form;
     int features;
+    bool split;
 };
 static TraceKey chooseTraceKernel(const pb2_scene *scene, int flags, bool render) {
     const bool instanced = scene->d.instances != nullptr;
@@ -844,56 +850,25 @@
     const bool linearFits = !instanced || scene->bvhDepth + 3 + scene->instDepth <= 64;
     int sceneBits = scene->d.spheres ? TRACE_SPHERES : 0;
     if (instanced) sceneBits |= TRACE_SPHERES | TRACE_INST;
-    if (flags & PB2_FLAG_COUNT_TRAVERSAL) return {TK_COUNT, 0};
-    if ((flags & PB2_FLAG_PLAIN_TRACE) || (!records && !linearFits)) return {TK_PLAIN, 0};
-    if (scene->d.hasAlpha) return records ? TraceKey{TK_WIDE2, sceneBits | TRACE_ALPHA} : TraceKey{TK_PLAIN, 0};
-    if (!records) return {TK_LINEAR, sceneBits | (sceneBits || scene->bvhDepth > 32 ? TRACE_DEEP : 0)};
-    if ((flags & PB2_FLAG_POOL) && !sceneBits) return {TK_POOL, 0};
+    if (flags & PB2_FLAG_COUNT_TRAVERSAL) return {TK_COUNT, 0, false};
+    if ((flags & PB2_FLAG_PLAIN_TRACE) || (!records && !linearFits)) return {TK_PLAIN, 0, false};
+    if (scene->d.hasAlpha) return records ? TraceKey{TK_WIDE2, sceneBits | TRACE_ALPHA, true} : TraceKey{TK_PLAIN, 0, false};
+    if (!records) return {TK_LINEAR, sceneBits | (sceneBits || scene->bvhDepth > 32 ? TRACE_DEEP : 0), false};
+    if ((flags & PB2_FLAG_POOL) && !sceneBits) return {TK_POOL, 0, false};
     const bool ld128 = (flags & PB2_FLAG_LD128) != 0;
     int features = sceneBits | (ld128 ? TRACE_LD128 : 0) | ((flags & PB2_FLAG_SMALL_STACK) ? TRACE_SMALL_STACK : 0);
-    if (flags & PB2_FLAG_WIDE4) return {TK_WIDE4, features};
+    if (flags & PB2_FLAG_WIDE4) return {TK_WIDE4, features, false};
     if (!ld128 && (flags & PB2_FLAG_LEAF_TMA) && !sceneBits) features = TRACE_LEAF_TMA;
     if (!ld128 && render && (flags & PB2_FLAG_CHAIN) && !(flags & (PB2_FLAG_SMALL_STACK | PB2_FLAG_LEAF_TMA))) features |= TRACE_CHAIN;
-    return {TK_WIDE2, features};
-}
-
-static int selectTraceKernel(pb2_scene *scene, int flags, TraceLaunch *out, bool render = false, const char *steps = "") {
-    static const TraceKernelEntry kernels[] = {
-        {TK_COUNT, 0, k_wf_trace_plain<true>, "k_wf_trace_plain<count>", 0},
-        {TK_PLAIN, 0, k_wf_trace_plain<false>, "k_wf_trace_plain", 0},
-        {TK_POOL, 0, k_wf_trace_pool, "k_wf_trace_pool", 4 * sizeof(PoolWarp)},
-        wideTrace<2, 0>(), wideTrace<2, TRACE_SMALL_STACK>(),
-        wideTrace<2, TRACE_LD128>(), wideTrace<2, TRACE_LD128 | TRACE_SMALL_STACK>(),
-        wideTrace<2, TRACE_SPHERES>(), wideTrace<2, TRACE_SPHERES | TRACE_SMALL_STACK>(),
-        wideTrace<2, TRACE_SPHERES | TRACE_LD128>(), wideTrace<2, TRACE_SPHERES | TRACE_LD128 | TRACE_SMALL_STACK>(),
-        wideTrace<2, TRACE_SPHERES | TRACE_INST>(), wideTrace<2, TRACE_SPHERES | TRACE_INST | TRACE_SMALL_STACK>(),
-        wideTrace<2, TRACE_SPHERES | TRACE_INST | TRACE_LD128>(), wideTrace<2, TRACE_SPHERES | TRACE_INST | TRACE_LD128 | TRACE_SMALL_STACK>(),
-        wideTrace<2, TRACE_LEAF_TMA>(),
-        wideTrace<2, TRACE_CHAIN>(), wideTrace<2, TRACE_SPHERES | TRACE_CHAIN>(), wideTrace<2, TRACE_SPHERES | TRACE_INST | TRACE_CHAIN>(),
-        wideTrace<2, TRACE_ALPHA>(), wideTrace<2, TRACE_SPHERES | TRACE_ALPHA>(), wideTrace<2, TRACE_SPHERES | TRACE_INST | TRACE_ALPHA>(),
-        wideTrace<4, 0>(), wideTrace<4, TRACE_SMALL_STACK>(),
-        wideTrace<4, TRACE_LD128>(), wideTrace<4, TRACE_LD128 | TRACE_SMALL_STACK>(),
-        wideTrace<4, TRACE_SPHERES>(), wideTrace<4, TRACE_SPHERES | TRACE_SMALL_STACK>(),
-        wideTrace<4, TRACE_SPHERES | TRACE_LD128>(), wideTrace<4, TRACE_SPHERES | TRACE_LD128 | TRACE_SMALL_STACK>(),
-        wideTrace<4, TRACE_SPHERES | TRACE_INST>(), wideTrace<4, TRACE_SPHERES | TRACE_INST | TRACE_SMALL_STACK>(),
-        wideTrace<4, TRACE_SPHERES | TRACE_INST | TRACE_LD128>(), wideTrace<4, TRACE_SPHERES | TRACE_INST | TRACE_LD128 | TRACE_SMALL_STACK>(),
-        linearTrace<0>(), linearTrace<TRACE_DEEP>(),
-        linearTrace<TRACE_SPHERES | TRACE_DEEP>(), linearTrace<TRACE_SPHERES | TRACE_INST | TRACE_DEEP>(),
-    };
-    const TraceKey want = chooseTraceKernel(scene, flags, render);
-    const TraceKernelEntry *k = nullptr;
-    for (const TraceKernelEntry &e : kernels)
-        if (e.form == want.form && e.features == want.features) k = &e;
-    if (!k)
-        return setError(PB2_ERR_CUDA, "no trace kernel of form " + std::to_string(want.form) + " is compiled for the trace features " +
-                                          std::to_string(want.features));
+    return {TK_WIDE2, features, features == sceneBits};
+}
+
+static int traceLaunchOf(const pb2_scene *scene, const TraceKernelEntry &k, const char *list, const char *steps, TraceLaunch *out) {
     TraceLaunch t;
-    t.fn = k->fn;
-    t.smem = k->smem;
-    t.chain = (k->features & TRACE_CHAIN) != 0;
-    t.name = k->name;
-    if (k->form == TK_POOL && !scene->wfSpill)
-        CUDA_TRY(cudaMalloc((void **)&scene->wfSpill, (size_t)kMaxPipes * g_numSMs * 8 * 4 * PL_R * PL_SPILL * sizeof(int2)));
+    t.fn = k.fn;
+    t.smem = k.smem;
+    t.chain = (k.features & TRACE_CHAIN) != 0;
+    t.name = k.name;
     if (t.smem) CUDA_TRY(cudaFuncSetAttribute(t.fn, cudaFuncAttributeMaxDynamicSharedMemorySize, (int)t.smem));
     int blocksPerSM = 1;
     CUDA_TRY(cudaOccupancyMaxActiveBlocksPerMultiprocessor(&blocksPerSM, t.fn, t.block, t.smem));
@@ -905,11 +880,61 @@
     CUDA_TRY(cudaFuncSetAttribute(t.fn, cudaFuncAttributePreferredSharedMemoryCarveout, pct));
     static const int verbose = envInt("PB2_VERBOSE", 0);
     if (verbose)
-        fprintf(stderr, "pb2: trace kernel %s: %d regs, %zu B smem, %d blocks/SM, carve-out %d %%, BVH depth %d%s\n", t.name, fa.numRegs,
-                fa.sharedSizeBytes + t.smem, blocksPerSM, pct, scene->bvhDepth, steps);
+        fprintf(stderr, "pb2: trace kernel %s: %d regs, %zu B smem, %d blocks/SM, carve-out %d %%, trace features %d, %s, BVH depth %d%s\n",
+                t.name, fa.numRegs, fa.sharedSizeBytes + t.smem, blocksPerSM, pct, k.features, list, scene->bvhDepth, steps);
     t.grid = g_numSMs * blocksPerSM;
     *out = t;
     return PB2_OK;
+}
+
+static int selectTraceKernel(pb2_scene *scene, int flags, TraceLaunch *trace, TraceLaunch *shadow, bool render = false, const char *steps = "") {
+    static const TraceKernelEntry kernels[] = {
+        {TK_COUNT, 0, k_wf_trace_plain<true>, "k_wf_trace_plain<count>", 0},
+        {TK_PLAIN, 0, k_wf_trace_plain<false>, "k_wf_trace_plain", 0},
+        {TK_POOL, 0, k_wf_trace_pool, "k_wf_trace_pool", 4 * sizeof(PoolWarp)},
+        wideTrace<2, TRACE_CLOSEST>(), wideTrace<2, TRACE_ANY>(),
+        wideTrace<2, TRACE_SPHERES | TRACE_CLOSEST>(), wideTrace<2, TRACE_SPHERES | TRACE_ANY>(),
+        wideTrace<2, TRACE_SPHERES | TRACE_INST | TRACE_CLOSEST>(), wideTrace<2, TRACE_SPHERES | TRACE_INST | TRACE_ANY>(),
+        wideTrace<2, TRACE_ALPHA | TRACE_CLOSEST>(), wideTrace<2, TRACE_ALPHA | TRACE_ANY>(),
+        wideTrace<2, TRACE_SPHERES | TRACE_ALPHA | TRACE_CLOSEST>(), wideTrace<2, TRACE_SPHERES | TRACE_ALPHA | TRACE_ANY>(),
+        wideTrace<2, TRACE_SPHERES | TRACE_INST | TRACE_ALPHA | TRACE_CLOSEST>(),
+        wideTrace<2, TRACE_SPHERES | TRACE_INST | TRACE_ALPHA | TRACE_ANY>(),
+        wideTrace<2, TRACE_SMALL_STACK>(),
+        wideTrace<2, TRACE_LD128>(), wideTrace<2, TRACE_LD128 | TRACE_SMALL_STACK>(),
+        wideTrace<2, TRACE_SPHERES | TRACE_SMALL_STACK>(),
+        wideTrace<2, TRACE_SPHERES | TRACE_LD128>(), wideTrace<2, TRACE_SPHERES | TRACE_LD128 | TRACE_SMALL_STACK>(),
+        wideTrace<2, TRACE_SPHERES | TRACE_INST | TRACE_SMALL_STACK>(),
+        wideTrace<2, TRACE_SPHERES | TRACE_INST | TRACE_LD128>(), wideTrace<2, TRACE_SPHERES | TRACE_INST | TRACE_LD128 | TRACE_SMALL_STACK>(),
+        wideTrace<2, TRACE_LEAF_TMA>(),
+        wideTrace<2, TRACE_CHAIN>(), wideTrace<2, TRACE_SPHERES | TRACE_CHAIN>(), wideTrace<2, TRACE_SPHERES | TRACE_INST | TRACE_CHAIN>(),
+        wideTrace<4, 0>(), wideTrace<4, TRACE_SMALL_STACK>(),
+        wideTrace<4, TRACE_LD128>(), wideTrace<4, TRACE_LD128 | TRACE_SMALL_STACK>(),
+        wideTrace<4, TRACE_SPHERES>(), wideTrace<4, TRACE_SPHERES | TRACE_SMALL_STACK>(),
+        wideTrace<4, TRACE_SPHERES | TRACE_LD128>(), wideTrace<4, TRACE_SPHERES | TRACE_LD128 | TRACE_SMALL_STACK>(),
+        wideTrace<4, TRACE_SPHERES | TRACE_INST>(), wideTrace<4, TRACE_SPHERES | TRACE_INST | TRACE_SMALL_STACK>(),
+        wideTrace<4, TRACE_SPHERES | TRACE_INST | TRACE_LD128>(), wideTrace<4, TRACE_SPHERES | TRACE_INST | TRACE_LD128 | TRACE_SMALL_STACK>(),
+        linearTrace<0>(), linearTrace<TRACE_DEEP>(),
+        linearTrace<TRACE_SPHERES | TRACE_DEEP>(), linearTrace<TRACE_SPHERES | TRACE_INST | TRACE_DEEP>(),
+    };
+    const TraceKey want = chooseTraceKernel(scene, flags, render);
+    auto find = [&](int features) -> const TraceKernelEntry * {
+        const TraceKernelEntry *k = nullptr;
+        for (const TraceKernelEntry &e : kernels)
+            if (e.form == want.form && e.features == features) k = &e;
+        if (!k)
+            setError(PB2_ERR_CUDA, "no trace kernel of form " + std::to_string(want.form) + " is compiled for the trace features " +
+                                       std::to_string(features));
+        return k;
+    };
+    const TraceKernelEntry *k = find(want.split ? want.features | TRACE_CLOSEST : want.features);
+    const TraceKernelEntry *ks = want.split ? find(want.features | TRACE_ANY) : nullptr;
+    if (!k || (want.split && !ks)) return PB2_ERR_CUDA;
+    if (k->form == TK_POOL && !scene->wfSpill)
+        CUDA_TRY(cudaMalloc((void **)&scene->wfSpill, (size_t)kMaxPipes * g_numSMs * 8 * 4 * PL_R * PL_SPILL * sizeof(int2)));
+    *shadow = TraceLaunch();
+    int rc = traceLaunchOf(scene, *k, want.split ? "path list" : "one list", steps, trace);
+    if (!rc && ks) rc = traceLaunchOf(scene, *ks, "shadow list", steps, shadow);
+    return rc;
 }
 
 static int ensurePool(pb2_scene *scene, int capacity) {
@@ -943,7 +968,7 @@
 constexpr int kShadeLambertAreaMinBlocks = 4;
 
 typedef void (*GenKernel)(const DRenderParams *, WfPool, int, int);
-typedef void (*FinishKernel)(const DScene *, const DRenderParams *, WfPool, int, unsigned, float4 *);
+typedef void (*FinishKernel)(const DScene *, const DRenderParams *, WfPool, int, int, unsigned, float4 *);
 
 template <typename K>
 struct StepKernel {
@@ -1012,8 +1037,9 @@
     char steps[96];
     snprintf(steps, sizeof(steps), "; shade features %d: gen %d, light %d, shade %d, tail %d", features, gen.features,
              advLight.features, advShade.features, finish.features);
-    TraceLaunch trace;
-    if ((rc = selectTraceKernel(scene, flags, &trace, true, steps))) return rc;
+    TraceLaunch trace, shadowTrace;
+    if ((rc = selectTraceKernel(scene, flags, &trace, &shadowTrace, true, steps))) return rc;
+    const bool split = shadowTrace.fn != nullptr;
     if (!scene->paramBuf) CUDA_TRY(cudaMalloc(&scene->paramBuf, sizeof(DScene) + sizeof(DRenderParams)));
     const DScene *dSc = reinterpret_cast<const DScene *>(scene->paramBuf);
     const DRenderParams *dRp = reinterpret_cast<const DRenderParams *>((char *)scene->paramBuf + sizeof(DScene));
@@ -1056,11 +1082,11 @@
     volatile unsigned *hc = scene->wfHostCounts;
     unsigned long long *hWork = reinterpret_cast<unsigned long long *>(scene->wfHostCounts + kMaxPipes * WQ_COUNT);
     for (long long round = 0;; ++round) {
-        int next = 1 - cur;
+        const WfRoundLists lists = wfRoundLists(cur, split);
         for (int p = 0; p < nPipes; ++p) {
             const WfPool &pool = pools[p];
             cudaStream_t st = streams[p];
-            gen.fn<<<blocks128, 128, 0, st>>>(dRp, pool, WQ_FREE0 + cur, WQ_TRACE0 + cur);
+            gen.fn<<<blocks128, 128, 0, st>>>(dRp, pool, lists.freeQ, lists.traceQ);
             if (timeTrace) {
                 if (scene->traceEvents.size() < nEvents + 2) {
                     cudaEvent_t e0, e1;
@@ -1071,25 +1097,28 @@
                 }
                 CUDA_TRY(cudaEventRecord(scene->traceEvents[nEvents], st));
             }
-            chain.freeQ = WQ_FREE0 + next;
-            trace.fn<<<trace.grid, trace.block, trace.smem, st>>>(scene->d, pool, WQ_TRACE0 + cur, chain);
+            chain.freeQ = lists.freeNext;
+            if (split) shadowTrace.fn<<<shadowTrace.grid, shadowTrace.block, shadowTrace.smem, st>>>(scene->d, pool, lists.shadowQ, chain);
+            trace.fn<<<trace.grid, trace.block, trace.smem, st>>>(scene->d, pool, lists.traceQ, chain);
             if (timeTrace) {
                 CUDA_TRY(cudaEventRecord(scene->traceEvents[nEvents + 1], st));
                 nEvents += 2;
             }
-            if (!trace.chain) advLight.fn<<<blocks128, 128, 0, st>>>(dSc, dRp, pool, WQ_LIGHT, WQ_TRACE0 + next, WQ_FREE0 + next, film, scene->counters);
+            if (!trace.chain)
+                advLight.fn<<<blocks128, 128, 0, st>>>(dSc, dRp, pool, WQ_LIGHT, lists.traceNext, lists.shadowNext, lists.freeNext, film, scene->counters);
             else --nLaunch;
-            advShade.fn<<<blocks128, 128, 0, st>>>(dSc, dRp, pool, WQ_SHADE, WQ_TRACE0 + next, WQ_FREE0 + next, film, scene->counters);
+            advShade.fn<<<blocks128, 128, 0, st>>>(dSc, dRp, pool, WQ_SHADE, lists.traceNext, lists.shadowNext, lists.freeNext, film, scene->counters);
             if (lazyLights) {
                 launchLightDistBuild(scene, st);
-                advShade.fn<<<blocks128, 128, 0, st>>>(dSc, dRp, pool, WQ_RETRY, WQ_TRACE0 + next, WQ_FREE0 + next, film, scene->counters);
+                advShade.fn<<<blocks128, 128, 0, st>>>(dSc, dRp, pool, WQ_RETRY, lists.traceNext, lists.shadowNext, lists.freeNext, film,
+                                                       scene->counters);
                 nLaunch += 3;
             }
-            if (finishThreshold) finish.fn<<<finishBlocks, 128, 0, st>>>(dSc, dRp, pool, WQ_TRACE0 + next, finishThreshold, film);
-            k_wf_reset<<<1, 32, 0, st>>>(pool, WQ_FREE0 + cur, WQ_TRACE0 + cur, WQ_TRACE0 + next, finishThreshold);
-            nLaunch += finishThreshold ? 6 : 5;
-        }
-        cur = next;
+            if (finishThreshold) finish.fn<<<finishBlocks, 128, 0, st>>>(dSc, dRp, pool, lists.traceNext, lists.shadowNext, finishThreshold, film);
+            k_wf_reset<<<1, 32, 0, st>>>(pool, lists, finishThreshold);
+            nLaunch += (finishThreshold ? 6 : 5) + (split ? 1 : 0);
+        }
+        cur = 1 - cur;
         if ((round + 1) % syncEvery != 0) continue;
         for (int p = 0; p < nPipes; ++p)
             CUDA_TRY(cudaMemcpyAsync((void *)(scene->wfHostCounts + p * WQ_COUNT), pools[p].counts, WQ_COUNT * sizeof(unsigned), cudaMemcpyDeviceToHost, streams[p]));
@@ -1102,7 +1131,8 @@
         const bool workLeft = (long long)*hWork < rp.nWorkItems;
         bool done = true;
         for (int p = 0; p < nPipes; ++p) {
-            const unsigned traceNext = hc[p * WQ_COUNT + WQ_TRACE0 + cur], freeNext = hc[p * WQ_COUNT + WQ_FREE0 + cur];
+            const WfRoundLists l = wfRoundLists(cur, split);
+            const unsigned traceNext = hc[p * WQ_COUNT + l.traceQ] + (split ? hc[p * WQ_COUNT + l.shadowQ] : 0u), freeNext = hc[p * WQ_COUNT + l.freeQ];
             if (!(traceNext == 0 && !(workLeft && freeNext > 0))) done = false;
         }
         if (done) break;
@@ -2205,8 +2235,9 @@
     if (n > (1 << 24)) return setError(PB2_ERR_INVALID, "at most 2^24 rays per call");
     const int N = (int)n;
     if ((rc = ensurePool(scene, (N + 255) / 256 * 256))) return rc;
-    TraceLaunch trace;
-    if ((rc = selectTraceKernel(scene, flags, &trace))) return rc;
+    TraceLaunch trace, shadowTrace;
+    if ((rc = selectTraceKernel(scene, flags, &trace, &shadowTrace))) return rc;
+    const WfRoundLists lists = wfRoundLists(0, shadowTrace.fn != nullptr);
     WfPool pool = poolOf(scene, scene->wfCapacity);
     pb2_ray *dRays = nullptr;
     uint8_t *dAny = nullptr;
@@ -2216,12 +2247,14 @@
     if (e == cudaSuccess && any_hit) e = cudaMalloc((void **)&dAny, n);
     if (e == cudaSuccess) e = cudaMemcpy(dRays, rays, n * sizeof(pb2_ray), cudaMemcpyHostToDevice);
     if (e == cudaSuccess && any_hit) e = cudaMemcpy(dAny, any_hit, n, cudaMemcpyHostToDevice);
+    if (e == cudaSuccess) e = cudaMemset(pool.counts, 0, WQ_COUNT * sizeof(unsigned));
     if (e == cudaSuccess) {
         const int blocks = (N + 127) / 128;
-        k_wf_debug_fill<<<blocks, 128>>>(pool, dRays, dAny, N);
+        k_wf_debug_fill<<<blocks, 128>>>(pool, dRays, dAny, N, lists.shadowQ);
         WfChain noChain;
         memset(&noChain, 0, sizeof(noChain));
-        trace.fn<<<trace.grid, trace.block, trace.smem>>>(scene->d, pool, WQ_TRACE0, noChain);
+        if (shadowTrace.fn) shadowTrace.fn<<<shadowTrace.grid, shadowTrace.block, shadowTrace.smem>>>(scene->d, pool, lists.shadowQ, noChain);
+        trace.fn<<<trace.grid, trace.block, trace.smem>>>(scene->d, pool, lists.traceQ, noChain);
         k_wf_debug_read<<<blocks, 128>>>(scene->d, pool, N, dOut);
         k_wf_debug_lists<<<std::min(blocks, g_numSMs * 8), 128>>>(pool, dOut);
         e = cudaGetLastError();
@@ -2231,6 +2264,18 @@
     cudaFree(dAny);
     cudaFree(dOut);
     if (e != cudaSuccess) return setError(PB2_ERR_CUDA, std::string("pb2_trace_wavefront: ") + cudaGetErrorString(e));
+    return PB2_OK;
+}
+
+int pb2_wavefront_round(int32_t cur, int32_t split, int32_t tail, uint32_t *counts, int32_t *lists_out, int32_t *n_counts) {
+    if (cur != 0 && cur != 1) return setError(PB2_ERR_INVALID, "round parity is 0 or 1");
+    if (n_counts) *n_counts = WQ_COUNT;
+    const WfRoundLists l = wfRoundLists(cur, split != 0);
+    if (lists_out) {
+        const int32_t v[6] = {l.freeQ, l.traceQ, l.shadowQ, l.freeNext, l.traceNext, l.shadowNext};
+        for (int i = 0; i < 6; ++i) lists_out[i] = v[i];
+    }
+    if (counts) wfResetCounts(counts, l, tail != 0);
     return PB2_OK;
 }
 
diff --git a/pbrt_v3_b200/csrc/pb2_wavefront.cuh b/pbrt_v3_b200/csrc/pb2_wavefront.cuh
--- a/pbrt_v3_b200/csrc/pb2_wavefront.cuh
+++ b/pbrt_v3_b200/csrc/pb2_wavefront.cuh
@@ -111,8 +111,42 @@
     __syncwarp();
 }
 
-enum { WQ_TRACE0 = 0, WQ_TRACE1 = 1, WQ_SHADE = 2, WQ_LIGHT = 3, WQ_FREE0 = 4, WQ_FREE1 = 5, WQ_CURSOR = 6, WQ_RETRY = 7, WQ_COUNT = 8 };
+enum {
+    WQ_TRACE0 = 0, WQ_TRACE1 = 1, WQ_SHADE = 2, WQ_LIGHT = 3, WQ_FREE0 = 4, WQ_FREE1 = 5, WQ_CURSOR = 6, WQ_RETRY = 7,
+    WQ_SHADOW0 = 8, WQ_SHADOW1 = 9, WQ_SHADOW_CURSOR = 10, WQ_COUNT = 11
+};
 enum { WQ_FINISH = WQ_RETRY, WF_FINISH_WAIT = 1, WF_FINISH_GO = 2 };
+
+struct WfRoundLists {
+    int freeQ, traceQ, shadowQ;
+    int freeNext, traceNext, shadowNext;
+};
+__host__ __device__ inline WfRoundLists wfRoundLists(int cur, bool split) {
+    const int next = 1 - cur;
+    WfRoundLists l;
+    l.freeQ = WQ_FREE0 + cur;
+    l.traceQ = WQ_TRACE0 + cur;
+    l.shadowQ = split ? WQ_SHADOW0 + cur : l.traceQ;
+    l.freeNext = WQ_FREE0 + next;
+    l.traceNext = WQ_TRACE0 + next;
+    l.shadowNext = split ? WQ_SHADOW0 + next : l.traceNext;
+    return l;
+}
+
+__host__ __device__ inline void wfResetCounts(unsigned *counts, const WfRoundLists &l, bool tail) {
+    if (tail && counts[WQ_FINISH] == WF_FINISH_GO) {
+        counts[l.traceNext] = 0;
+        counts[l.shadowNext] = 0;
+    }
+    counts[WQ_RETRY] = 0;
+    counts[WQ_CURSOR] = 0;
+    counts[WQ_SHADOW_CURSOR] = 0;
+    counts[WQ_SHADE] = 0;
+    counts[WQ_LIGHT] = 0;
+    counts[l.freeQ] = 0;
+    counts[l.traceQ] = 0;
+    counts[l.shadowQ] = 0;
+}
 
 struct WfPool {
     int capacity;
@@ -143,6 +177,16 @@
     if (lane == leader) base = atomicAdd(counter, (unsigned)__popc(mask));
     base = __shfl_sync(0xffffffffu, base, leader);
     if (participate) queue[base + __popc(mask & ((1u << lane) - 1u))] = value;
+}
+
+__device__ __forceinline__ void wfPushTrace(const WfPool &pool, int traceQ, int shadowQ, int c, int state, bool participate) {
+    if (shadowQ == traceQ) {
+        wfPush(wfQueue(pool, traceQ), &pool.counts[traceQ], c, participate);
+        return;
+    }
+    const bool shadow = state == LS_SHADOW;
+    wfPush(wfQueue(pool, traceQ), &pool.counts[traceQ], c, participate && !shadow);
+    wfPush(wfQueue(pool, shadowQ), &pool.counts[shadowQ], c, participate && shadow);
 }
 
 __device__ __forceinline__ void wfCountRays(unsigned long long *counters, unsigned regular, unsigned shadow) {
@@ -253,6 +297,8 @@
     TRACE_LEAF_TMA = 32,
     TRACE_CHAIN = 64,
     TRACE_DEEP = 128,
+    TRACE_CLOSEST = 256,
+    TRACE_ANY = 512,
 };
 
 template <bool COUNT>
@@ -536,7 +582,11 @@
     static_assert(WIDTH == 2 || WIDTH == 4, "two- or four-child records");
     static constexpr bool SPHERES = (T & TRACE_SPHERES) != 0, INST = (T & TRACE_INST) != 0, ALPHA = (T & TRACE_ALPHA) != 0;
     static constexpr bool LD128 = (T & TRACE_LD128) != 0, LEAFTMA = (T & TRACE_LEAF_TMA) != 0, CHAIN = (T & TRACE_CHAIN) != 0;
+    static constexpr bool CLOSEST = (T & TRACE_CLOSEST) != 0, ANYHIT = (T & TRACE_ANY) != 0;
     static_assert(!LEAFTMA || (!SPHERES && !INST), "the staging experiment covers triangle scenes");
+    static_assert(!(CLOSEST && ANYHIT) && (!(CLOSEST || ANYHIT) || (WIDTH == 2 && !CHAIN && !LEAFTMA)),
+                  "one class, in the two-child kernel without the chained light step or the staging experiment");
+    constexpr int CURSOR = ANYHIT ? WQ_SHADOW_CURSOR : WQ_CURSOR;
     static constexpr int LEAF_T = 1, FETCH_T = 8, NSUB = 4, SDEPTH = (T & TRACE_SMALL_STACK) ? 4 : 16;
     constexpr int STAGED = 4;
     __shared__ alignas(16) float4 sleaf[LEAFTMA ? 128 * 3 * STAGED : 1];
@@ -722,7 +772,7 @@
                     const int2 rest = stGet(sp), saved = stGet(sp + 1);
                     leafFirst = rest.x;
                     leafN = rest.y;
-                    if (!(flags & F_HITIN)) tMax = __int_as_float(saved.x);
+                    if (ANYHIT || !(flags & F_HITIN)) tMax = __int_as_float(saved.x);
                     const float4 *p = reinterpret_cast<const float4 *>(&pool.ctx[c]);
                     float4 ra = p[0], rb = p[1];
                     rs = setupRay(mk3(ra.y, ra.z, ra.w), mk3(rb.x, rb.y, rb.z));
@@ -730,7 +780,7 @@
                     instBase = 0;
                 }
                 bool finished = false, entered = false;
-                const bool any = (flags & F_ANY) != 0;
+                const bool any = ANYHIT || (!CLOSEST && (flags & F_ANY) != 0);
                 int staged = 0;
                 while (leafN > 0) {
                     const int idx = leafFirst;
@@ -827,11 +877,13 @@
             int state = LS_IDLE;
             if (flush) {
                 WfCtx &cx = pool.ctx[c];
-                state = (flags & F_ANY) ? LS_SHADOW : __ldcs(&cx.ln.state);
-                const int foundCode = (flags & F_FOUND) ? ((INST && !(flags & F_ANY) && hitInst >= 0) ? 2 + hitInst : 1) : 0;
-                __stcs(reinterpret_cast<float2 *>(&cx.tHit), make_float2(tMax, __int_as_float(foundCode)));
-            }
-            wfPush(pool.queue[WQ_SHADE], &pool.counts[WQ_SHADE], c, flush && state == LS_PATH);
+                const bool any = ANYHIT || (!CLOSEST && (flags & F_ANY) != 0);
+                state = any ? LS_SHADOW : __ldcs(&cx.ln.state);
+                const int foundCode = (flags & F_FOUND) ? ((INST && !any && hitInst >= 0) ? 2 + hitInst : 1) : 0;
+                if (ANYHIT) __stcs(&cx.found, foundCode);
+                else __stcs(reinterpret_cast<float2 *>(&cx.tHit), make_float2(tMax, __int_as_float(foundCode)));
+            }
+            if (!ANYHIT) wfPush(pool.queue[WQ_SHADE], &pool.counts[WQ_SHADE], c, flush && state == LS_PATH);
             bool again = false;
             if (CHAIN) {
                 int next = LS_PATH;
@@ -868,7 +920,7 @@
             if (wantMask) {
                 int leader = __ffs(wantMask) - 1;
                 unsigned base = 0;
-                if (lane == leader) base = atomicAdd(&pool.counts[WQ_CURSOR], (unsigned)__popc(wantMask));
+                if (lane == leader) base = atomicAdd(&pool.counts[CURSOR], (unsigned)__popc(wantMask));
                 base = __shfl_sync(FULL, base, leader);
                 if (want) {
                     unsigned i = base + __popc(wantMask & ((1u << lane) - 1u));
@@ -878,7 +930,7 @@
                         c = pool.queue[traceQ][i];
                         const float4 *p = reinterpret_cast<const float4 *>(&pool.ctx[c]);
                         float4 ra = __ldcs(p), rb = __ldcs(p + 1);
-                        flags = (__float_as_int(ra.x) == LS_SHADOW) ? F_ANY : 0;
+                        flags = (!CLOSEST && !ANYHIT && __float_as_int(ra.x) == LS_SHADOW) ? F_ANY : 0;
                         rs = setupRay(mk3(ra.y, ra.z, ra.w), mk3(rb.x, rb.y, rb.z));
                         tMax = rb.w;
                         cur = 0;
@@ -1113,7 +1165,8 @@
 
 template <bool SHADE, int MINB, int F>
 __global__ void __launch_bounds__(128, MINB) k_wf_advance(const DScene *__restrict__ scp, const DRenderParams *__restrict__ rpp, WfPool pool,
-                                                          int srcQ, int traceQ, int freeQ, float4 *film, unsigned long long *counters) {
+                                                          int srcQ, int traceQ, int shadowQ, int freeQ, float4 *film,
+                                                          unsigned long long *counters) {
     __shared__ WfSlot stage[128];
     __shared__ float sampleRows[SHADE ? 128 * (kSampleBatch + 1) : 1];
     WfSlot &slot = stage[threadIdx.x];
@@ -1122,7 +1175,7 @@
     const DScene &sc = *scp;
     const DRenderParams &rp = *rpp;
     const int *srcList = wfQueue(pool, srcQ);
-    int *traceList = wfQueue(pool, traceQ), *freeList = wfQueue(pool, freeQ);
+    int *freeList = wfQueue(pool, freeQ);
     unsigned n = pool.counts[srcQ];
     unsigned stride = gridDim.x * blockDim.x;
     unsigned regular = 0, shadow = 0;
@@ -1131,6 +1184,7 @@
         bool have = i < n;
         int c = have ? srcList[i] : 0;
         bool ended = false, deferred = false;
+        int next = LS_IDLE;
         wfStageIn<SHADE ? WF_IN_SHADE : WF_IN_ALL>(pool.ctx, warpSlots, have ? c : -1);
         if (have) {
             DLane &ln = slot.ln;
@@ -1155,6 +1209,7 @@
                 ln.state = LS_PATH;
                 deferred = true;
             } else {
+                next = ln.state;
                 ended = ln.state == LS_IDLE;
                 if (ended) addSample(rp, film, slot.pFilm, guardRadiance(ln.L));
                 else if (ln.state == LS_SHADOW) shadow++;
@@ -1163,35 +1218,38 @@
         }
         wfStageOut<SHADE ? WF_OUT_SHADE : WF_OUT_LIGHT>(pool.ctx, warpSlots, have && !ended ? c : -1);
         if (SHADE && (F & SHADE_LAZY)) wfPush(pool.queue[WQ_RETRY], &pool.counts[WQ_RETRY], c, deferred);
-        wfPush(traceList, &pool.counts[traceQ], c, have && !ended && !deferred);
+        wfPushTrace(pool, traceQ, shadowQ, c, next, have && !ended && !deferred);
         wfPush(freeList, &pool.counts[freeQ], c, have && ended);
     }
     wfCountRays(counters, regular, shadow);
 }
 
-__device__ __forceinline__ bool wfFinishNow(const DRenderParams &rp, const WfPool &pool, int traceQ, unsigned threshold) {
-    const unsigned n = pool.counts[traceQ];
+__device__ __forceinline__ unsigned wfInFlight(const WfPool &pool, int traceQ, int shadowQ) {
+    return pool.counts[traceQ] + (shadowQ != traceQ ? pool.counts[shadowQ] : 0u);
+}
+__device__ __forceinline__ bool wfFinishNow(const DRenderParams &rp, const WfPool &pool, int traceQ, int shadowQ, unsigned threshold) {
+    const unsigned n = wfInFlight(pool, traceQ, shadowQ);
     return n > 0 && n <= threshold && (long long)pool.ctr[CTR_WORK] >= rp.nWorkItems;
 }
 
 template <int F>
 __global__ void __launch_bounds__(128) k_wf_finish(const DScene *__restrict__ scp, const DRenderParams *__restrict__ rpp, WfPool pool, int traceQ,
-                                                   unsigned threshold, float4 *film) {
+                                                   int shadowQ, unsigned threshold, float4 *film) {
     const DScene &sc = *scp;
     const DRenderParams &rp = *rpp;
     __shared__ bool sGo;
     if (threadIdx.x == 0) {
-        const unsigned mine = wfFinishNow(rp, pool, traceQ, threshold) ? WF_FINISH_GO : WF_FINISH_WAIT;
+        const unsigned mine = wfFinishNow(rp, pool, traceQ, shadowQ, threshold) ? WF_FINISH_GO : WF_FINISH_WAIT;
         const unsigned first = atomicCAS(&pool.counts[WQ_FINISH], 0u, mine);
         sGo = (first ? first : mine) == WF_FINISH_GO;
     }
     __syncthreads();
     if (!sGo) return;
-    const unsigned n = pool.counts[traceQ];
-    const int *traceList = wfQueue(pool, traceQ);
+    const unsigned nPath = pool.counts[traceQ], n = wfInFlight(pool, traceQ, shadowQ);
+    const int *traceList = wfQueue(pool, traceQ), *shadowList = wfQueue(pool, shadowQ);
     unsigned regular = 0, shadow = 0;
     for (unsigned i = blockIdx.x * blockDim.x + threadIdx.x; i < n; i += gridDim.x * blockDim.x) {
-        WfCtx &cx = pool.ctx[traceList[i]];
+        WfCtx &cx = pool.ctx[i < nPath ? traceList[i] : shadowList[i - nPath]];
         DLane &ln = cx.ln;
         while (ln.state != LS_IDLE) {
             DHit hit;
@@ -1248,16 +1306,8 @@
     if (i < WQ_COUNT) pool.counts[i] = (i == WQ_FREE0) ? (unsigned)pool.capacity : 0u;
 }
 
-__global__ void k_wf_reset(WfPool pool, int a, int b, int traceNext, unsigned threshold) {
-    if (threadIdx.x == 0) {
-        if (threshold && pool.counts[WQ_FINISH] == WF_FINISH_GO) pool.counts[traceNext] = 0;
-        pool.counts[WQ_RETRY] = 0;
-        pool.counts[WQ_CURSOR] = 0;
-        pool.counts[WQ_SHADE] = 0;
-        pool.counts[WQ_LIGHT] = 0;
-        pool.counts[a] = 0;
-        pool.counts[b] = 0;
-    }
+__global__ void k_wf_reset(WfPool pool, WfRoundLists lists, unsigned threshold) {
+    if (threadIdx.x == 0) wfResetCounts(pool.counts, lists, threshold != 0);
 }
 
 #endif
```

New measurement: 215.2 (median of 6 runs). -3.4%, worse.
